# burchim/AVEC

Measured on AMD Instinct MI355X. Metric: AV utterances/sec fwd+bwd (audio T=400, video 100x88x88), higher is better.
Workload: dtype bf16

## Files before the change

avec_amd/csrc/conv3x3.hip:

```cpp
#include "wave_prims.h"
#include "vec.h"
#include "avec_hip.h"

#define C3_WPITCH 1280
#define C3_WBYTES (64 * C3_WPITCH)
#define C3_MAXPIX 576
#define C3_SBYTES (C3_MAXPIX * 128)

struct C3Args { const bf16* x; const bf16* w; bf16* y; const bf16* res; float* stats; int N, H, W, flip; const unsigned char* rmask; };

__device__ __forceinline__ int c3_wslot(int n, int c) { return (c & ~15) | ((c & 15) ^ (n & 15)); }
__device__ __forceinline__ int c3_saddr(int pix, int c) { const int pr = pix >> 1; return pr * 256 + (((((pix & 1) << 3) | c) ^ (pr & 7)) << 4); }
__device__ __forceinline__ int c3_lane_pixel(int l) { return l < 4 ? l : l < 12 ? l + 12 : l < 16 ? l - 8 : l < 20 ? l + 8 : l < 28 ? l - 12 : l; }

#ifndef C3S_ABL
#define C3S_ABL 0
#endif
template <bool STATS, bool RES>
__global__ __launch_bounds__(512) void conv3x3_c64_kernel(C3Args a) {
  extern __shared__ __attribute__((aligned(16))) char smem[];
  char* Ws = smem; char* Sl = smem + C3_WBYTES;
  const int tid = threadIdx.x, lane = tid & 63, wave = tid >> 6;
  const int H = a.H, W = a.W, PW = W + 1, HW = H * W, NPIX = (H + 2) * PW + 1;

  for (int q = tid; q < 64 * 72; q += 512) {
    const int n = q / 72, c = q - n * 72;
    *(chunk16*)(Ws + n * C3_WPITCH + c3_wslot(n, c) * 16) = ldg16(a.w + (long long)n * 576 + c * 8);
  }
  int soff[9];
#pragma unroll
  for (int i = 0; i < 9; ++i) {
    const int S = (wave + 8 * i) * 64 + lane, pr = S >> 4, c2 = (S & 15) ^ (pr & 7);
    const int pix = pr * 2 + (c2 >> 3), ch = c2 & 7;
    const int py = (pix - 1) / PW, px = (pix - 1) - py * PW;
    const bool in = pix >= 1 && pix < NPIX && py >= 1 && py <= H && px < W;
    soff[i] = in ? ((py - 1) * W + px) * 64 + ch * 8 : -1;
  }
  const int kh2 = lane >> 5;
  int p0[2]; bool pvalid[2]; int pm[2];
#pragma unroll
  for (int i = 0; i < 2; ++i) {
    int m = wave * 64 + i * 32 + c3_lane_pixel(lane & 31);
    pvalid[i] = m < HW; if (m >= HW) m = HW - 1;
    pm[i] = m;
    const int oy = m / W;
    p0[i] = oy * PW + (m - oy * W);
  }
  const int wrow[2] = {(lane & 31) * C3_WPITCH, (32 + (lane & 31)) * C3_WPITCH};
  const int wkey = lane & 15;

  float ssum[STATS ? 2 : 1][16], ssq[STATS ? 2 : 1][16];
  if (STATS) {
#pragma unroll
    for (int j = 0; j < 2; ++j)
#pragma unroll
      for (int r = 0; r < 16; ++r) { ssum[j][r] = 0.f; ssq[j][r] = 0.f; }
  }

  f32x16 acc[2][2];
  u32x4 outp[2][2][2], resp[RES ? 2 : 1][2][2];
  long long prev = -1;
  auto swap_pair = [&](uint2& x, uint2& y) {
    auto r0 = __builtin_amdgcn_permlane32_swap(x.x, y.x, false, false); x.x = r0[0]; y.x = r0[1];
    auto r1 = __builtin_amdgcn_permlane32_swap(x.y, y.y, false, false); x.y = r1[0]; y.y = r1[1];
  };
  const int chq = kh2 * 8;
  unsigned ldoff[9], zmask = 0u;
#pragma unroll
  for (int i = 0; i < 9; ++i) { ldoff[i] = soff[i] < 0 ? 0u : (unsigned)soff[i] * 2u; if (soff[i] < 0) zmask |= 1u << i; }
  const unsigned stoff[2] = {(unsigned)pm[0] * 128u + (unsigned)chq * 2u, (unsigned)pm[1] * 128u + (unsigned)chq * 2u};
#define C3_GLOAD(dst, voff, sbase, OFF) asm volatile("s_nop 4\n\tglobal_load_dwordx4 %0, %1, %2 offset:%3" : "+v"(dst) : "v"(voff), "s"(sbase), "n"(OFF))
#define C3_GSTORE(voff, data, sbase, OFF) asm volatile("s_nop 4\n\tglobal_store_dwordx4 %0, %1, %2 offset:%3\n\ts_nop 1" :: "v"(voff), "v"(data), "s"(sbase), "n"(OFF))
  auto issue_stores = [&]() {
    if (prev < 0 || (C3S_ABL & (8 | 16))) return;
    bf16* yo = a.y + prev * HW * 64;
#pragma unroll
    for (int i = 0; i < 2; ++i) {
      if (!pvalid[i]) continue;
#pragma unroll
      for (int j = 0; j < 2; ++j)
#pragma unroll
        for (int k = 0; k < 2; ++k) *(u32x4*)(yo + (long long)pm[i] * 64 + j * 32 + k * 16 + chq) = outp[j][i][k];
    }
  };

  u32x4 pf[9];
#pragma unroll
  for (int i = 0; i < 9; ++i) pf[i] = u32x4{0u, 0u, 0u, 0u};
  if (RES) {
#pragma unroll
    for (int i = 0; i < 2; ++i)
#pragma unroll
      for (int j = 0; j < 2; ++j)
#pragma unroll
        for (int k = 0; k < 2; ++k) resp[RES ? j : 0][i][k] = u32x4{0u, 0u, 0u, 0u};
  }
  if ((long long)blockIdx.x < a.N && !(C3S_ABL & 2)) {
    const bf16* x0 = a.x + (long long)blockIdx.x * HW * 64;
#pragma unroll
    for (int i = 0; i < 9; ++i) C3_GLOAD(pf[i], ldoff[i], x0, 0);
    asm volatile("s_waitcnt vmcnt(0)");
#pragma unroll
    for (int i = 0; i < 9; ++i) asm volatile("" : "+v"(pf[i]));
  }
#ifdef C3S_TRACE
  int tr_k = 0;
  float* const trbuf = STATS ? a.stats + 8192 : (float*)(a.y + (long long)a.N * HW * 64);
#define C3S_STAMP(slot) do { if (blockIdx.x == C3S_TRACE_WG && tid == 0 && tr_k < 16) { trbuf[8 * tr_k + (slot)] = (float)(clock64() & 0xffffff); if ((slot) == 0) trbuf[8 * tr_k + 6] = (float)(wall_clock64() & 0xffffff); } } while (0)
#else
#define C3S_STAMP(slot) do {} while (0)
#endif
  for (long long n = blockIdx.x; n < a.N; n += gridDim.x) {
    C3S_STAMP(0);
    asm volatile("s_waitcnt vmcnt(0)");
#pragma unroll
    for (int i = 0; i < 9; ++i) asm volatile("" : "+v"(pf[i]));
    __syncthreads();
#pragma unroll
    for (int i = 0; i < 9; ++i) {
      if (C3S_ABL & 2) break;
      u32x4 v = pf[i];
      if (zmask & (1u << i)) v = u32x4{0u, 0u, 0u, 0u};
      *(u32x4*)(Sl + ((wave + 8 * i) * 64 + lane) * 16) = v;
    }
    __syncthreads();
    C3S_STAMP(1);
#pragma unroll
    for (int j = 0; j < 2; ++j)
#pragma unroll
      for (int i = 0; i < 2; ++i)
#pragma unroll
        for (int r = 0; r < 16; ++r) acc[j][i][r] = 0.f;
    int p0o[2] = {p0[0], p0[1]}, wkeyo = wkey;
    asm volatile("" : "+v"(p0o[0]), "+v"(p0o[1]), "+v"(wkeyo));
    auto tap_addr = [&](int tap, int& ax0, int& ax1, int& aw0, int& aw1, bool& z0, bool& z1) {
      const int th = tap / 3, tw = tap - th * 3;
      const int dh = (a.flip & 1) ? 2 - th : th, dw = (a.flip & 1) ? 2 - tw : tw;
      const int d = dh * PW + dw;
      ax0 = c3_saddr(p0o[0] + d, kh2); ax1 = c3_saddr(p0o[1] + d, kh2);
      const int wt = (((tap >> 1) << 4) | ((((tap & 1) << 3) | kh2) ^ wkeyo)) << 4;
      aw0 = wrow[0] + wt; aw1 = wrow[1] + wt;
      z0 = z1 = false;
    };
    auto load4 = [&](int ax0, int ax1, int aw0, int aw1, bool z0, bool z1, int q, chunk16& fx0, chunk16& fx1, chunk16& fw0, chunk16& fw1) {
      if (C3S_ABL & 4) { fx0.w[0] = fx0.w[1] = fx0.w[2] = fx0.w[3] = ax0 + q; fx1 = fx0; fw0 = fx0; fw1 = fx0; return; }
      fx0 = *(const chunk16*)(Sl + (ax0 ^ (q << 5)));
      fx1 = *(const chunk16*)(Sl + (ax1 ^ (q << 5)));
      fw0 = *(const chunk16*)(Ws + (aw0 ^ (q << 5)));
      fw1 = *(const chunk16*)(Ws + (aw1 ^ (q << 5)));
    };
    const bool has_prev = prev >= 0 && !(C3S_ABL & (8 | 16)), has_next = n + gridDim.x < a.N;
    const bf16* const yprev = a.y + (has_prev ? prev : 0) * HW * 64;
    const bf16* const xnext = a.x + (has_next ? n + gridDim.x : n) * HW * 64;
    const bf16* const rcur = RES ? a.res + n * HW * 64 : a.x;
    auto one_tap = [&](int tap) {
      int ax0, ax1, aw0, aw1; bool z0, z1;
      tap_addr(tap, ax0, ax1, aw0, aw1, z0, z1);
#pragma unroll
      for (int q = 0; q < 4; ++q) {
        chunk16 cx0, cx1, cw0, cw1;
        load4(ax0, ax1, aw0, aw1, z0, z1, q, cx0, cx1, cw0, cw1);
        if (C3S_ABL & 1) { asm volatile("" :: "v"(cx0.w[0]), "v"(cx0.w[3]), "v"(cx1.w[0]), "v"(cx1.w[3]), "v"(cw0.w[0]), "v"(cw0.w[3]), "v"(cw1.w[0]), "v"(cw1.w[3])); continue; }
        acc[0][0] = __builtin_amdgcn_mfma_f32_32x32x16_bf16(__builtin_bit_cast(bf16x8_t, cw0), __builtin_bit_cast(bf16x8_t, cx0), acc[0][0], 0, 0, 0);
        acc[0][1] = __builtin_amdgcn_mfma_f32_32x32x16_bf16(__builtin_bit_cast(bf16x8_t, cw0), __builtin_bit_cast(bf16x8_t, cx1), acc[0][1], 0, 0, 0);
        acc[1][0] = __builtin_amdgcn_mfma_f32_32x32x16_bf16(__builtin_bit_cast(bf16x8_t, cw1), __builtin_bit_cast(bf16x8_t, cx0), acc[1][0], 0, 0, 0);
        acc[1][1] = __builtin_amdgcn_mfma_f32_32x32x16_bf16(__builtin_bit_cast(bf16x8_t, cw1), __builtin_bit_cast(bf16x8_t, cx1), acc[1][1], 0, 0, 0);
      }
    };
#define C3_RS(I, J, K) do { if (RES) C3_GLOAD(resp[RES ? (J) : 0][I][K], stoff[I], rcur, (J) * 64 + (K) * 32); } while (0)
#define C3_ST(I, J, K) do { if (has_prev) C3_GSTORE(stoff[I], outp[J][I][K], yprev, (J) * 64 + (K) * 32); } while (0)
#define C3_LD1(I) do { if (!(C3S_ABL & 2)) C3_GLOAD(pf[I], ldoff[I], xnext, 0); } while (0)
#pragma unroll
    for (int tap = 0; tap < 9; ++tap) {
      switch (tap) {
        case 0: C3_LD1(0); C3_ST(0, 0, 0); break;
        case 1: C3_LD1(1); C3_ST(0, 0, 1); break;
        case 2: C3_LD1(2); C3_ST(0, 1, 0); break;
        case 3: C3_LD1(3); C3_ST(0, 1, 1); break;
        case 4: C3_LD1(4); C3_ST(1, 0, 0); break;
        case 5: C3_RS(0, 0, 0); C3_RS(0, 0, 1); C3_RS(0, 1, 0); C3_RS(0, 1, 1); C3_RS(1, 0, 0); C3_RS(1, 0, 1); C3_RS(1, 1, 0); C3_RS(1, 1, 1); C3_LD1(5); C3_ST(1, 0, 1); break;
        case 6: C3_LD1(6); C3_ST(1, 1, 0); break;
        case 7: C3_LD1(7); C3_ST(1, 1, 1); break;
        default: C3_LD1(8); break;
      }
      one_tap(tap);
      if (tap == 4) C3S_STAMP(2);
    }
#undef C3_LD1
#undef C3_RS
#undef C3_ST
    if (RES) { if (C3S_ABL & 2) asm volatile("s_waitcnt vmcnt(0)"); else if (has_prev) asm volatile("s_waitcnt vmcnt(7)"); else asm volatile("s_waitcnt vmcnt(4)"); }
    if (RES) {
#pragma unroll
      for (int i = 0; i < 2; ++i)
#pragma unroll
        for (int j = 0; j < 2; ++j)
#pragma unroll
          for (int k = 0; k < 2; ++k) asm volatile("" : "+v"(resp[RES ? j : 0][i][k]));
    }
    C3S_STAMP(3);
    if (C3S_ABL & 8) {
      float t = 0.f;
      for (int i = 0; i < 2; ++i) for (int j = 0; j < 2; ++j) for (int r = 0; r < 16; ++r) t += acc[j][i][r];
      if (t == 1234.5f) outp[0][0][0][0] = 1u;
      asm volatile("" :: "v"(t));
      prev = n; continue;
    }
#pragma unroll
    for (int i = 0; i < 2; ++i)
#pragma unroll
      for (int j = 0; j < 2; ++j)
#pragma unroll
        for (int k = 0; k < 2; ++k) {
          uint2 rx = make_uint2(0u, 0u), ry = make_uint2(0u, 0u);
          if (RES) { const u32x4 rr = resp[RES ? j : 0][i][k]; rx = make_uint2(rr[0], rr[1]); ry = make_uint2(rr[2], rr[3]); swap_pair(rx, ry); }
          uint2 o[2];
#pragma unroll
          for (int e = 0; e < 2; ++e) {
            const int g = 2 * k + e;
            float v[4] = {acc[j][i][g * 4 + 0], acc[j][i][g * 4 + 1], acc[j][i][g * 4 + 2], acc[j][i][g * 4 + 3]};
            if (STATS && pvalid[i]) {
#pragma unroll
              for (int t = 0; t < 4; ++t) { ssum[j][g * 4 + t] += v[t]; ssq[j][g * 4 + t] += v[t] * v[t]; }
            }
            if (RES) {
              const uint2 r = e ? ry : rx;
              v[0] += __uint_as_float(r.x << 16); v[1] += __uint_as_float(r.x & 0xffff0000u); v[2] += __uint_as_float(r.y << 16); v[3] += __uint_as_float(r.y & 0xffff0000u);
            }
            o[e] = make_uint2(f32x2_to_bf16x2(v[0], v[1]), f32x2_to_bf16x2(v[2], v[3]));
          }
          swap_pair(o[0], o[1]);
          outp[j][i][k] = u32x4{o[0].x, o[0].y, o[1].x, o[1].y};
        }
    prev = n;
    C3S_STAMP(4);
#ifdef C3S_TRACE
    ++tr_k;
#endif
  }
  issue_stores();
  if (STATS) {
    __syncthreads();
    float* red = (float*)Sl;
#pragma unroll
    for (int j = 0; j < 2; ++j)
#pragma unroll
      for (int r = 0; r < 16; ++r) {
        float s = ssum[j][r], q = ssq[j][r];
#pragma unroll
        for (int o = 1; o < 32; o <<= 1) { s += __shfl_xor(s, o, 64); q += __shfl_xor(q, o, 64); }
        if ((lane & 31) == 0) {
          const int ch = j * 32 + (r >> 2) * 8 + kh2 * 4 + (r & 3);
          red[(wave * 2 + 0) * 64 + ch] = s; red[(wave * 2 + 1) * 64 + ch] = q;
        }
      }
    __syncthreads();
    if (tid < 128) {
      float t = 0.f;
      for (int w = 0; w < 8; ++w) t += red[w * 128 + tid];
      float* rep = a.stats + (long long)(blockIdx.x % AVEC_STAT_REPLICAS) * 128;
      atomicAdd(rep + tid, t);
    }
  }
}

__device__ __forceinline__ unsigned c3_mask2(unsigned b, int d) {
  return ((0u - ((b >> (2 * d)) & 1u)) & 0xffffu) | ((0u - ((b >> (2 * d + 1)) & 1u)) & 0xffff0000u);
}
__global__ __launch_bounds__(512) void conv3x3_c64_res_kernel(C3Args a) {
  extern __shared__ __attribute__((aligned(16))) char smem[];
  char* Ws = smem; char* Sl = smem + C3_WBYTES;
  const int tid = threadIdx.x, lane = tid & 63, wave = tid >> 6;
  const int H = a.H, W = a.W, PW = W + 1, HW = H * W, NPIX = (H + 2) * PW + 1;

  for (int q = tid; q < 64 * 72; q += 512) {
    const int n = q / 72, c = q - n * 72;
    *(chunk16*)(Ws + n * C3_WPITCH + c3_wslot(n, c) * 16) = ldg16(a.w + (long long)n * 576 + c * 8);
  }
  int soff[9];
#pragma unroll
  for (int i = 0; i < 9; ++i) {
    const int S = (wave + 8 * i) * 64 + lane, pr = S >> 4, c2 = (S & 15) ^ (pr & 7);
    const int pix = pr * 2 + (c2 >> 3), ch = c2 & 7;
    const int py = (pix - 1) / PW, px = (pix - 1) - py * PW;
    const bool in = pix >= 1 && pix < NPIX && py >= 1 && py <= H && px < W;
    soff[i] = in ? ((py - 1) * W + px) * 64 + ch * 8 : -1;
  }
  const int kh2 = lane >> 5;
  int p0[2]; bool pvalid[2]; int pm[2];
#pragma unroll
  for (int i = 0; i < 2; ++i) {
    int m = wave * 64 + i * 32 + c3_lane_pixel(lane & 31);
    pvalid[i] = m < HW; if (m >= HW) m = HW - 1;
    pm[i] = m;
    const int oy = m / W;
    p0[i] = oy * PW + (m - oy * W);
  }
  const int wrow[2] = {(lane & 31) * C3_WPITCH, (32 + (lane & 31)) * C3_WPITCH};
  const int wkey = lane & 15;


  f32x16 acc[2][2];
  uint4 outp[2][2][2], resp[2][2][2];
  long long prev = -1;
  auto swap_pair = [&](uint2& x, uint2& y) {
    auto r0 = __builtin_amdgcn_permlane32_swap(x.x, y.x, false, false); x.x = r0[0]; y.x = r0[1];
    auto r1 = __builtin_amdgcn_permlane32_swap(x.y, y.y, false, false); x.y = r1[0]; y.y = r1[1];
  };
  const int chq = kh2 * 8;
  auto issue_stores = [&]() {
    if (prev < 0) return;
    bf16* yo = a.y + prev * HW * 64;
#pragma unroll
    for (int i = 0; i < 2; ++i) {
      if (!pvalid[i]) continue;
#pragma unroll
      for (int j = 0; j < 2; ++j)
#pragma unroll
        for (int k = 0; k < 2; ++k) *(uint4*)(yo + (long long)pm[i] * 64 + j * 32 + k * 16 + chq) = outp[j][i][k];
    }
  };

  chunk16 pf[9];
  if ((long long)blockIdx.x < a.N) {
    const bf16* x0 = a.x + (long long)blockIdx.x * HW * 64;
#pragma unroll
    for (int i = 0; i < 9; ++i) pf[i] = ldg16(x0 + (soff[i] < 0 ? 0 : soff[i]));
  }
  for (long long n = blockIdx.x; n < a.N; n += gridDim.x) {
    __syncthreads();
#pragma unroll
    for (int i = 0; i < 9; ++i) {
      chunk16 v = pf[i];
      if (soff[i] < 0) v.w[0] = v.w[1] = v.w[2] = v.w[3] = 0u;
      *(chunk16*)(Sl + ((wave + 8 * i) * 64 + lane) * 16) = v;
    }
    __syncthreads();
    if (n + gridDim.x < a.N) {
      const bf16* xn = a.x + (n + gridDim.x) * HW * 64;
#pragma unroll
      for (int i = 0; i < 9; ++i) pf[i] = ldg16(xn + (soff[i] < 0 ? 0 : soff[i]));
    }
#pragma unroll
    for (int j = 0; j < 2; ++j)
#pragma unroll
      for (int i = 0; i < 2; ++i)
#pragma unroll
        for (int r = 0; r < 16; ++r) acc[j][i][r] = 0.f;
    auto tap_addr = [&](int tap, int& ax0, int& ax1, int& aw0, int& aw1, bool& z0, bool& z1) {
      const int th = tap / 3, tw = tap - th * 3;
      const int dh = (a.flip & 1) ? 2 - th : th, dw = (a.flip & 1) ? 2 - tw : tw;
      const int d = dh * PW + dw;
      ax0 = c3_saddr(p0[0] + d, kh2); ax1 = c3_saddr(p0[1] + d, kh2);
      const int wt = (((tap >> 1) << 4) | ((((tap & 1) << 3) | kh2) ^ wkey)) << 4;
      aw0 = wrow[0] + wt; aw1 = wrow[1] + wt;
      z0 = z1 = false;
    };
    auto load4 = [&](int ax0, int ax1, int aw0, int aw1, bool z0, bool z1, int q, chunk16& fx0, chunk16& fx1, chunk16& fw0, chunk16& fw1) {
      fx0 = *(const chunk16*)(Sl + (ax0 ^ (q << 5)));
      fx1 = *(const chunk16*)(Sl + (ax1 ^ (q << 5)));
      fw0 = *(const chunk16*)(Ws + (aw0 ^ (q << 5)));
      fw1 = *(const chunk16*)(Ws + (aw1 ^ (q << 5)));
    };
    bf16* yprev = prev >= 0 ? a.y + prev * HW * 64 : nullptr;
    auto one_tap = [&](int tap) {
      int ax0, ax1, aw0, aw1; bool z0, z1;
      tap_addr(tap, ax0, ax1, aw0, aw1, z0, z1);
#pragma unroll
      for (int q = 0; q < 4; ++q) {
        chunk16 cx0, cx1, cw0, cw1;
        load4(ax0, ax1, aw0, aw1, z0, z1, q, cx0, cx1, cw0, cw1);
        acc[0][0] = mma16(cw0, cx0, acc[0][0]);
        acc[0][1] = mma16(cw0, cx1, acc[0][1]);
        acc[1][0] = mma16(cw1, cx0, acc[1][0]);
        acc[1][1] = mma16(cw1, cx1, acc[1][1]);
      }
    };
#define C3_ST(I, J, K) if (pvalid[I]) *(uint4*)(yprev + (long long)pm[I] * 64 + J * 32 + K * 16 + chq) = outp[J][I][K]
#pragma unroll 1
    for (int tap = 0; tap < 5; ++tap) {
      if (yprev) {
        switch (tap) {
          case 1: C3_ST(0, 0, 0); C3_ST(0, 0, 1); break;
          case 2: C3_ST(0, 1, 0); C3_ST(0, 1, 1); break;
          case 3: C3_ST(1, 0, 0); C3_ST(1, 0, 1); break;
          case 4: C3_ST(1, 1, 0); C3_ST(1, 1, 1); break;
          default: break;
        }
      }
      one_tap(tap);
    }
#undef C3_ST
    if (a.res) {
      const bf16* ro = a.res + n * HW * 64;
#pragma unroll
      for (int i = 0; i < 2; ++i)
#pragma unroll
        for (int j = 0; j < 2; ++j)
#pragma unroll
          for (int k = 0; k < 2; ++k) resp[j][i][k] = *(const uint4*)(ro + (long long)pm[i] * 64 + j * 32 + k * 16 + chq);
      if (a.rmask) {
        const unsigned char* mo = a.rmask + n * HW * 8;
        unsigned mb[2][2][2];
#pragma unroll
        for (int i = 0; i < 2; ++i)
#pragma unroll
          for (int j = 0; j < 2; ++j)
#pragma unroll
            for (int k = 0; k < 2; ++k) mb[j][i][k] = mo[((long long)pm[i] * 64 + j * 32 + k * 16 + chq) >> 3];
#pragma unroll
        for (int i = 0; i < 2; ++i)
#pragma unroll
          for (int j = 0; j < 2; ++j)
#pragma unroll
            for (int k = 0; k < 2; ++k) {
              const unsigned b = mb[j][i][k];
              resp[j][i][k].x &= c3_mask2(b, 0); resp[j][i][k].y &= c3_mask2(b, 1); resp[j][i][k].z &= c3_mask2(b, 2); resp[j][i][k].w &= c3_mask2(b, 3);
            }
      }
    }
#pragma unroll 1
    for (int tap = 5; tap < 9; ++tap) one_tap(tap);
#pragma unroll
    for (int i = 0; i < 2; ++i)
#pragma unroll
      for (int j = 0; j < 2; ++j)
#pragma unroll
        for (int k = 0; k < 2; ++k) {
          uint2 rx = make_uint2(0u, 0u), ry = make_uint2(0u, 0u);
          if (a.res) { rx = make_uint2(resp[j][i][k].x, resp[j][i][k].y); ry = make_uint2(resp[j][i][k].z, resp[j][i][k].w); swap_pair(rx, ry); }
          uint2 o[2];
#pragma unroll
          for (int e = 0; e < 2; ++e) {
            const int g = 2 * k + e;
            float v[4] = {acc[j][i][g * 4 + 0], acc[j][i][g * 4 + 1], acc[j][i][g * 4 + 2], acc[j][i][g * 4 + 3]};
            if (a.res) {
              const uint2 r = e ? ry : rx;
              v[0] += __uint_as_float(r.x << 16); v[1] += __uint_as_float(r.x & 0xffff0000u); v[2] += __uint_as_float(r.y << 16); v[3] += __uint_as_float(r.y & 0xffff0000u);
            }
            o[e] = make_uint2(f32x2_to_bf16x2(v[0], v[1]), f32x2_to_bf16x2(v[2], v[3]));
          }
          swap_pair(o[0], o[1]);
          outp[j][i][k] = make_uint4(o[0].x, o[0].y, o[1].x, o[1].y);
        }
    prev = n;
  }
  issue_stores();
}

__device__ __forceinline__ uint2 c3_lds_tr(unsigned lds_addr) { uint2 v; asm volatile("ds_read_b64_tr_b16 %0, %1" : "=v"(v) : "v"(lds_addr) : "memory"); return v; }
#ifndef C3W_ABL
#define C3W_ABL 0
#endif
#define C3W_KROWS 512
#define C3W_DBYTES (C3W_KROWS * 128)

struct C3WArgs { const bf16* x; const bf16* dy; float* dw; int N, H, W; };
#if C3W_ABL & 64
__device__ float c3w_dbg[128];
extern "C" int avec_c3w_debug(float* out) { return (int)hipMemcpyFromSymbol(out, HIP_SYMBOL(c3w_dbg), sizeof(float) * 128); }
#endif

template <int V> struct C3I { static constexpr int value = V; };
__device__ __forceinline__ void c3w_roll_body(const C3WArgs& a, const int bid, const int nwg) {
  extern __shared__ __attribute__((aligned(16))) char smem[];
  char* Xs = smem; char* Ds = smem + C3_SBYTES;
  const int tid = threadIdx.x, lane = tid & 63, wave = __builtin_amdgcn_readfirstlane(tid >> 6);
  const int H = a.H, W = a.W, PW = W + 1, HW = H * W, NPIX = (H + 2) * PW + 1;
  int xoff[9], doff[8];
#pragma unroll
  for (int i = 0; i < 9; ++i) {
    const int S = (wave + 8 * i) * 64 + lane, row = S >> 3, c = (S & 7) ^ (4 * ((row >> 1) & 1));
    const int py = (row - 1) / PW, px = (row - 1) - py * PW;
    const bool in = row >= 1 && row < NPIX && py >= 1 && py <= H && px < W;
    xoff[i] = in ? ((py - 1) * W + px) * 64 + c * 8 : -1;
  }
#pragma unroll
  for (int i = 0; i < 8; ++i) {
    const int S = (wave + 8 * i) * 64 + lane, row = S >> 3, c = (S & 7) ^ (4 * ((row >> 1) & 1));
    const int oy = row / PW, ox = row - oy * PW;
    doff[i] = (oy < H && ox < W) ? (oy * W + ox) * 64 + c * 8 : -1;
  }
  const int cohalf = (wave >> 1) & 1, cihalf = wave & 1, tap0 = wave >> 2;
  const bool five = wave < 4;
  const int g4 = lane >> 4, t = lane & 15;
  int offa[2], offb[5][2];
#pragma unroll
  for (int h = 0; h < 2; ++h) {
    const int krow = 8 * (g4 >> 1) + 4 * h + (t >> 2);
    const int cbA = cohalf * 32 + 16 * (g4 & 1), cbB = cihalf * 32 + 16 * (g4 & 1);
    offa[h] = krow * 128 + ((((cbA >> 3) + ((t & 3) >> 1)) ^ (4 * ((krow >> 1) & 1))) << 4) + (t & 1) * 8;
#pragma unroll
    for (int j = 0; j < 5; ++j) {
      const int tap = j < 4 ? tap0 + 2 * j : 8;
      const int rowd = krow + (tap / 3) * PW + (tap % 3);
      offb[j][h] = rowd * 128 + ((((cbB >> 3) + ((t & 3) >> 1)) ^ (4 * ((rowd >> 1) & 1))) << 4) + (t & 1) * 8;
    }
  }
  f32x16 acc[5];
#pragma unroll
  for (int j = 0; j < 5; ++j)
#pragma unroll
    for (int r = 0; r < 16; ++r) acc[j][r] = 0.f;

  const unsigned xs0 = (unsigned)(uintptr_t)(lptr_t)Xs, ds0 = (unsigned)(uintptr_t)(lptr_t)Ds;
  auto batch = [&](auto gc, const long long n) {
    constexpr int G = decltype(gc)::value;
    const bf16* xi = a.x + n * HW * 64; const bf16* di = a.dy + n * HW * 64;
#pragma unroll
    for (int i = 2 * G; i < (G == 3 ? 9 : 2 * G + 2); ++i) glds16(xoff[i] >= 0 ? (const void*)(xi + xoff[i]) : (const void*)avec_zero16, xs0 + (wave + 8 * i) * 1024);
#pragma unroll
    for (int i = 2 * G; i < 2 * G + 2; ++i) glds16(doff[i] >= 0 ? (const void*)(di + doff[i]) : (const void*)avec_zero16, ds0 + (wave + 8 * i) * 1024);
  };
  auto group = [&](auto gc) {
    constexpr int G = decltype(gc)::value;
#pragma unroll 2
    for (int s = 8 * G; s < 8 * G + 8; ++s) {
      const int so = s * 2048;
      const chunk16 fa = lds_tr8(Ds + offa[0] + so, Ds + offa[1] + so);
      chunk16 fb[5];
#pragma unroll
      for (int j = 0; j < 4; ++j) fb[j] = lds_tr8(Xs + offb[j][0] + so, Xs + offb[j][1] + so);
      if (five) fb[4] = lds_tr8(Xs + offb[4][0] + so, Xs + offb[4][1] + so);
#pragma unroll
      for (int j = 0; j < 4; ++j)
        acc[j] = mma16(fa, fb[j], acc[j]);
      if (five) acc[4] = mma16(fa, fb[4], acc[4]);
    }
// ... 202 lines not shown
  int KP, RS, IT;
  AVEC_CHECK_ARG(wgrad3x3_pairs_supported(H, W, C) || c3_wide_geometry(H, W, C, KP, RS, IT), "wgrad3x3_c128: %d channels, %dx%d images do not fit the slabs", C, H, W);
  avec_wgrad3x3_item_t it; it.x = x; it.dy = dy; it.dw = dw; it.images = images; it.C = C; it.H = H; it.W = W; it.reserved = 0;
  return avec_wgrad3x3_c128_grouped(&it, 1, st);
}

extern "C" int avec_wgrad3x3_c64_grouped(const avec_wgrad3x3_item_t* items, int n, hipStream_t st) {
  AVEC_CHECK_ARG(items && n > 0 && n <= AVEC_WGRAD_GROUP_MAX, "wgrad3x3_c64_grouped: 1..%d items", AVEC_WGRAD_GROUP_MAX);
  C3WGroup g; g.n = n;
  long long total_images = 0;
  for (int i = 0; i < n; ++i) {
    const avec_wgrad3x3_item_t& t = items[i];
    AVEC_CHECK_ARG(t.x && t.dy && t.dw && t.images > 0 && t.C == 64, "wgrad3x3_c64_grouped: bad item %d", i);
    AVEC_CHECK_ARG(avec_conv3x3_c64_supported(t.H, t.W, 64, 64, 3, 3, 1) && t.H * (t.W + 1) <= C3W_KROWS, "wgrad3x3_c64_grouped: item %d: %dx%d images do not fit the slab", i, t.H, t.W);
    C3WArgs& a = g.it[i]; a.x = (const bf16*)t.x; a.dy = (const bf16*)t.dy; a.dw = t.dw; a.N = (int)t.images; a.H = t.H; a.W = t.W;
    total_images += t.images;
  }
  int used = 0; g.first[0] = 0;
  for (int i = 0; i < n; ++i) {
    long long w = (256 * items[i].images + total_images / 2) / total_images; if (w < 1) w = 1; if (w > items[i].images) w = items[i].images;
    if (used + w > 256 + n) w = 1;
    used += (int)w; g.first[i + 1] = used;
  }
  const size_t lds = C3_SBYTES + C3W_DBYTES;
  if (int r = avec_lds_optin(wgrad3x3_c64_grouped_kernel, lds)) return r;
  avec_note_kernel("wgrad3x3_c64_grouped_kernel");
  hipLaunchKernelGGL(wgrad3x3_c64_grouped_kernel, dim3((unsigned)used), dim3(512), lds, st, g);
  AVEC_LAUNCH_CHECK();
  return 0;
}

extern "C" int avec_wgrad3x3_c128_grouped(const avec_wgrad3x3_item_t* items, int n, hipStream_t st) {
  AVEC_CHECK_ARG(items && n > 0 && n <= AVEC_WGRAD_GROUP_MAX, "wgrad3x3_c128_grouped: 1..%d items", AVEC_WGRAD_GROUP_MAX);
  {
    avec_wgrad3x3_item_t fast[AVEC_WGRAD_GROUP_MAX], slow[AVEC_WGRAD_GROUP_MAX]; int nf = 0, ns = 0;
    for (int i = 0; i < n; ++i) {
      AVEC_CHECK_ARG(items[i].x && items[i].dy && items[i].dw && items[i].images > 0, "wgrad3x3_c128_grouped: null buffer in item %d", i);
      if (wgrad3x3_pairs_supported(items[i].H, items[i].W, items[i].C)) fast[nf++] = items[i]; else slow[ns++] = items[i];
    }
    if (nf) {
      if (int r = wgrad3x3_pairs_grouped(fast, nf, st)) return r;
      if (!ns) return 0;
      return avec_wgrad3x3_c128_grouped(slow, ns, st);
    }
  }
  C3WWGroup g; g.n = n;
  long long cost[AVEC_WGRAD_GROUP_MAX]; int kinds[AVEC_WGRAD_GROUP_MAX], nwg[AVEC_WGRAD_GROUP_MAX], total = 0;
  for (int i = 0; i < n; ++i) {
    const avec_wgrad3x3_item_t& t = items[i];
    AVEC_CHECK_ARG(t.x && t.dy && t.dw && t.images > 0, "wgrad3x3_c128_grouped: null buffer in item %d", i);
    C3WWArgs& a = g.it[i]; a.x = (const bf16*)t.x; a.dy = (const bf16*)t.dy; a.dw = t.dw; a.N = (int)t.images; a.H = t.H; a.W = t.W; a.C = t.C;
    AVEC_CHECK_ARG(c3_wide_geometry(t.H, t.W, t.C, a.KP, a.RS, a.IT), "wgrad3x3_c128_grouped: item %d: %d channels, %dx%d images do not fit the slabs", i, t.C, t.H, t.W);
    kinds[i] = (t.C / 64) * (t.C / 128);
    const long long halves = (t.images + a.IT - 1) / a.IT;
    cost[i] = halves * (long long)(a.IT * (a.KP >> 4) + 2);
    nwg[i] = kinds[i]; total += kinds[i];
  }
  AVEC_CHECK_ARG(total <= 4096, "wgrad3x3_c128_grouped: too many tiles");
  const int budget = 256;
  for (;;) {
    int best = -1; double worst = 0.0;
    for (int i = 0; i < n; ++i) {
      const long long halves = (g.it[i].N + g.it[i].IT - 1) / g.it[i].IT;
      if (total + kinds[i] > budget || nwg[i] / kinds[i] >= halves) continue;
      const double load = (double)cost[i] / (double)(nwg[i] / kinds[i]);
      if (load > worst) { worst = load; best = i; }
    }
    if (best < 0) break;
    nwg[best] += kinds[best]; total += kinds[best];
  }
  g.first[0] = 0; for (int i = 0; i < n; ++i) g.first[i + 1] = g.first[i] + nwg[i];
  const size_t lds = (size_t)C3X_ROWS * 256 + C3X_KROWS * 128;
  if (int r = avec_lds_optin(wgrad3x3_wide_grouped_kernel, lds)) return r;
  avec_note_kernel("wgrad3x3_wide_grouped_kernel");
  hipLaunchKernelGGL(wgrad3x3_wide_grouped_kernel, dim3((unsigned)total), dim3(512), lds, st, g);
  AVEC_LAUNCH_CHECK();
  return 0;
}

extern "C" int avec_conv3x3_c64_supported(int H, int W, int Cin, int Cout, int KH, int KW, int stride) {
  return Cin == 64 && Cout == 64 && KH == 3 && KW == 3 && stride == 1 && H * W <= 512 && (H + 2) * (W + 1) + 1 <= C3_MAXPIX && H >= 1 && W >= 2;
}

static int conv3x3_c64_impl(const void* x, const void* w, void* y, const void* res, const unsigned char* rmask, float* stats, long long images, int H, int W, int flip, hipStream_t st);
extern "C" int avec_conv3x3_c64(const void* x, const void* w, void* y, const void* res, float* stats, long long images, int H, int W, int flip, hipStream_t st) {
  return conv3x3_c64_impl(x, w, y, res, nullptr, stats, images, H, W, flip, st);
}
extern "C" int avec_conv3x3_c64_res_masked(const void* x, const void* w, void* y, const void* res, const unsigned char* res_mask, long long images, int H, int W, int flip, hipStream_t st) {
  AVEC_CHECK_ARG(res && res_mask, "conv3x3_c64_res_masked: null residual / mask");
  return conv3x3_c64_impl(x, w, y, res, res_mask, nullptr, images, H, W, flip, st);
}
static int conv3x3_c64_impl(const void* x, const void* w, void* y, const void* res, const unsigned char* rmask, float* stats, long long images, int H, int W, int flip, hipStream_t st) {
  AVEC_CHECK_ARG(x && w && y && images > 0, "conv3x3_c64: null buffer");
  AVEC_CHECK_ARG(avec_conv3x3_c64_supported(H, W, 64, 64, 3, 3, 1), "conv3x3_c64: %dx%d images do not fit the slab", H, W);
  AVEC_CHECK_ARG(!(stats && res), "conv3x3_c64: statistics and a residual in the same launch are not supported");
  const size_t lds = C3_WBYTES + C3_SBYTES;
  const void* kern = !stats && !res ? (const void*)conv3x3_c64_kernel<false, false> : stats ? (const void*)conv3x3_c64_kernel<true, false> : (const void*)conv3x3_c64_res_kernel;
  if (int r = avec_lds_optin(kern, lds)) return r;
  C3Args a; a.x = (const bf16*)x; a.w = (const bf16*)w; a.y = (bf16*)y; a.res = (const bf16*)res; a.stats = stats; a.N = (int)images; a.H = H; a.W = W; a.flip = flip; a.rmask = rmask;
  const int grid = (int)(images < 256 ? images : 256);
  avec_note_kernel(stats ? "conv3x3_c64_kernel<true,false>" : res ? "conv3x3_c64_res_kernel" : "conv3x3_c64_kernel<false,false>");
  if (stats) hipLaunchKernelGGL((conv3x3_c64_kernel<true, false>), dim3(grid), dim3(512), lds, st, a);
  else if (res) hipLaunchKernelGGL(conv3x3_c64_res_kernel, dim3(grid), dim3(512), lds, st, a);
  else hipLaunchKernelGGL((conv3x3_c64_kernel<false, false>), dim3(grid), dim3(512), lds, st, a);
  AVEC_LAUNCH_CHECK();
  return 0;
}

extern "C" int avec_wgrad3x3_c64(const void* x, const void* dy, float* dw, long long images, int H, int W, hipStream_t st) {
  AVEC_CHECK_ARG(x && dy && dw && images > 0, "wgrad3x3_c64: null buffer");
  AVEC_CHECK_ARG(avec_conv3x3_c64_supported(H, W, 64, 64, 3, 3, 1) && H * (W + 1) <= C3W_KROWS, "wgrad3x3_c64: %dx%d images do not fit the slab", H, W);
  avec_wgrad3x3_item_t it; it.x = x; it.dy = dy; it.dw = dw; it.images = images; it.C = 64; it.H = H; it.W = W; it.reserved = 0;
  return avec_wgrad3x3_c64_grouped(&it, 1, st);
}
```

avec_amd/csrc/norm.hip:

```cpp
#include "common.h"
#include "avec_hip.h"

#include "vec.h"
#include <type_traits>

__global__ __launch_bounds__(256) void col_finalize_kernel(ColFin f) {
  __shared__ float red[16][17];
  const int cw = threadIdx.x & 15, sl = threadIdx.x >> 4;
  const int ncols = f.NV * f.W;
  const int o = blockIdx.x * 16 + cw;
  const unsigned cb = blockIdx.y;
  const int s0 = blockIdx.z * 128;
  float s = 0.f;
  if (o < ncols) {
    const float* p = f.partial + ((size_t)cb * f.nslots) * ncols + o;
#pragma unroll
    for (int k = 0; k < 8; ++k) {
      const int si = s0 + sl + 16 * k; const int sc = si < f.nslots ? si : f.nslots - 1;
      const float v = p[(size_t)sc * ncols];
      s += si < f.nslots ? v : 0.f;
    }
  }
  red[sl][cw] = s;
  __syncthreads();
// ... 588 lines not shown
  ld8<float>(ss + 2 * C + c, k.mu); ld8<float>(ss + 3 * C + c, k.rs);
  if (recompute) { ld8<float>(ss + c, k.sc); ld8<float>(ss + C + c, k.sh); }
}
__device__ __forceinline__ void bn8_dy_coeffs(Bn8Dy& q, const Bn8Bwd& k, const float* __restrict__ gamma, const float* __restrict__ dstats, float inv_n, int C, int c) {
  float g[8], s1[8], s2[8]; ld8<float>(gamma + c, g); ld8<float>(dstats + c, s1); ld8<float>(dstats + C + c, s2);
#pragma unroll
  for (int e = 0; e < 8; ++e) { q.A[e] = g[e] * k.rs[e]; q.m1[e] = s1[e] * inv_n; q.m2[e] = s2[e] * inv_n; }
}
template <typename T>
__device__ __forceinline__ void bn8_bwd_d(const Raw8<T>& rd, const Raw8<T>& rv, const Raw8<T>& ro, const unsigned& mb, int src, int act, const Bn8Bwd& k, float (&d)[8], float (&v)[8]) {
  rd.get(d); rv.get(v);
  if (src == BN_SRC_BITS) {
#pragma unroll
    for (int e = 0; e < 8; ++e) d[e] = (mb >> e) & 1u ? d[e] : 0.f;
  } else if (src == BN_SRC_OUT) { float o[8]; ro.get(o);
#pragma unroll
    for (int e = 0; e < 8; ++e) d[e] = o[e] > 0.f ? d[e] : 0.f;
  } else if (act == 2) {
#pragma unroll
    for (int e = 0; e < 8; ++e) d[e] = __builtin_fmaf(v[e], k.sc[e], k.sh[e]) > 0.f ? d[e] : 0.f;
  } else if (act == 1) {
#pragma unroll
    for (int e = 0; e < 8; ++e) { const float x = __builtin_fmaf(v[e], k.sc[e], k.sh[e]), sg = sigmoidf_(x); d[e] *= sg * __builtin_fmaf(x, 1.f - sg, 1.f); }
  }
}
__device__ __forceinline__ void bn8_bwd_acc(float (&part)[2][8], const float (&d)[8], const float (&v)[8], const Bn8Bwd& k) {
#pragma unroll
  for (int e = 0; e < 8; ++e) { part[0][e] += d[e]; part[1][e] += d[e] * (v[e] - k.mu[e]) * k.rs[e]; }
}
__device__ __forceinline__ void bn8_dy(const float (&d)[8], const float (&v)[8], const Bn8Bwd& k, const Bn8Dy& q, float (&o)[8]) {
#pragma unroll
  for (int e = 0; e < 8; ++e) o[e] = q.A[e] * __builtin_fmaf(-((v[e] - k.mu[e]) * k.rs[e]), q.m2[e], d[e] - q.m1[e]);
}

constexpr int BNS_P = 4;
constexpr unsigned BNS_SLICE_FWD = 1024, BNS_SLICE_BWD = 1536;
constexpr unsigned BNS_GRID_RED = 2048, BNS_RED_MIN_UNITS = 4;
constexpr long long BNS_MIN_CHUNKS = 1ll << 20;
static int& bns_mode() { static int mode = getenv("AVEC_BN_SLICE") ? atoi(getenv("AVEC_BN_SLICE")) : 1; return mode; }
static inline bool bns_ok(int dtype, long long M, int C) {
  const int mode = bns_mode();
  if (mode == 0 || dtype != AVEC_BF16 || C % 8 != 0 || 256 % (C / 8) != 0) return false;
  const long long n8 = M * C / 8;
  return n8 < (1ll << 31) && (mode == 2 || n8 >= BNS_MIN_CHUNKS);
}
template <bool NT> __device__ __forceinline__ void bns_ld(Raw8<bf16>& r, const bf16* p) {
  if (NT) { typedef unsigned v4u __attribute__((ext_vector_type(4))); const v4u t = __builtin_nontemporal_load((const v4u*)p); r.t = make_uint4(t.x, t.y, t.z, t.w); }
  else r.load(p);
}
static inline unsigned bns_slice(long long n8, unsigned grid) { return (unsigned)(((n8 + grid - 1) / grid + 255) / 256 * 256); }
static inline unsigned bns_grid(long long n8, unsigned slice) { return (unsigned)((n8 + slice - 1) / slice); }
static inline unsigned bns_red_grid(long long n8) {
  long long g = n8 / (256ll * BNS_P * BNS_RED_MIN_UNITS) / 256 * 256; if (g > BNS_GRID_RED) g = BNS_GRID_RED; if (g < 256) g = 256;
  return (unsigned)g;
}
struct BnsPlan { unsigned grid, slice; ColPlan col; };
static BnsPlan bns_plan(int pass, long long n8, int C, hipStream_t st) {
  if (pass == 1) { const ColPlan col = ColPlan::flat<2>(bns_red_grid(n8), C, st).cap_without_ws(256); return BnsPlan{col.nslots, bns_slice(n8, col.nslots), col}; }
  const unsigned slice = pass == 0 ? BNS_SLICE_FWD : BNS_SLICE_BWD;
  return BnsPlan{bns_grid(n8, slice), slice, ColPlan{}};
}
template <int P, typename Set, typename Load, typename Use>
__device__ __forceinline__ void bns_walk(unsigned begin, unsigned end, Load load, Use use) {
  constexpr unsigned UNIT = 256 * P;
  constexpr std::true_type full{}; constexpr std::false_type ragged{};
  if (begin >= end) return;
  Set a, b;
  unsigned base = begin;
  load(a, base, ragged);
  while (end - base >= 3 * UNIT) {
    load(b, base + UNIT, full); use(a, base, full);
    load(a, base + 2 * UNIT, full); use(b, base + UNIT, full);
    base += 2 * UNIT;
  }
  if (end - base > UNIT) {
    load(b, base + UNIT, ragged); use(a, base, full);
    if (end - base > 2 * UNIT) { load(a, base + 2 * UNIT, ragged); use(b, base + UNIT, full); use(a, base + 2 * UNIT, ragged); }
    else use(b, base + UNIT, ragged);
  } else use(a, base, ragged);
}
template <bool FULL> __device__ __forceinline__ unsigned bns_chunk(unsigned base, int p, unsigned end) {
  const unsigned j = base + threadIdx.x + p * 256; return FULL || j < end ? j : end - 1;
}
__device__ __forceinline__ void bns_range(unsigned slice, unsigned n8, unsigned& begin, unsigned& end) {
  const unsigned long long b = (unsigned long long)blockIdx.x * slice;
  begin = b < n8 ? (unsigned)b : n8; end = n8 - begin > slice ? begin + slice : n8;
}

template <int P, bool RES> struct BnsFwdSet { Raw8<bf16> y[P], r[RES ? P : 1]; };
template <int P, bool RES, bool MASK>
__global__ __launch_bounds__(256) void bn_apply8s_kernel(const bf16* __restrict__ y, const float* __restrict__ ss, const bf16* __restrict__ res, int act,
                                                         bf16* __restrict__ out, unsigned n8, int C, unsigned slice, unsigned char* __restrict__ mask,
                                                         const float* __restrict__ res_ss) {
  unsigned begin, end; bns_range(slice, n8, begin, end);
  const int c = (int)(threadIdx.x % ((unsigned)C >> 3)) * 8;
  Bn8Fwd k; bn8_fwd_coeffs(k, ss, RES ? res_ss : nullptr, C, c);
  typedef BnsFwdSet<P, RES> Set;
  auto load = [&](Set& s, unsigned base, auto full) {
#pragma unroll
    for (int p = 0; p < P; ++p) { const long long off = (long long)bns_chunk<decltype(full)::value>(base, p, end) * 8; bns_ld<true>(s.y[p], y + off); if (RES) bns_ld<true>(s.r[p], res + off); }
  };
  auto use = [&](Set& s, unsigned base, auto full) {
#pragma unroll
    for (int p = 0; p < P; ++p) {
      const unsigned j = base + threadIdx.x + p * 256; if (!decltype(full)::value && j >= end) break;
      const Bn8Out o = bn8_fwd<bf16>(s.y[p], s.r[RES ? p : 0], RES, res_ss != nullptr, k, act, MASK ? mask : nullptr, j);
      st8<bf16>(out + (long long)j * 8, o.v);
    }
  };
  bns_walk<P, Set>(begin, end, load, use);
}

template <int P, int SRC> struct BnsBwdSet { Raw8<bf16> d[P], v[P], o[SRC == BN_SRC_OUT ? P : 1]; unsigned mb[SRC == BN_SRC_BITS ? P : 1]; };
template <bool FULL, bool NT, int P, int SRC>
__device__ __forceinline__ void bns_bwd_load(BnsBwdSet<P, SRC>& s, unsigned base, unsigned end, const bf16* __restrict__ dout, const bf16* __restrict__ y,
                                             const bf16* __restrict__ out, const unsigned char* __restrict__ mask) {
#pragma unroll
  for (int p = 0; p < P; ++p) { const unsigned j = bns_chunk<FULL>(base, p, end); const long long off = (long long)j * 8; bns_ld<NT>(s.d[p], dout + off); bns_ld<NT>(s.v[p], y + off);
    if (SRC == BN_SRC_BITS) s.mb[p] = mask[j]; else if (SRC == BN_SRC_OUT) bns_ld<NT>(s.o[p], out + off); }
}
template <int P, int SRC>
__device__ __forceinline__ void bns_bwd_d(const BnsBwdSet<P, SRC>& s, int p, int act, const Bn8Bwd& k, float (&d)[8], float (&v)[8]) {
  bn8_bwd_d<bf16>(s.d[p], s.v[p], s.o[SRC == BN_SRC_OUT ? p : 0], s.mb[SRC == BN_SRC_BITS ? p : 0], SRC, act, k, d, v);
}
template <int P, int SRC>
__global__ __launch_bounds__(256) void bn_bwd_reduce8s_kernel(const bf16* __restrict__ dout, const bf16* __restrict__ y, const bf16* __restrict__ out, const float* __restrict__ ss,
                                                              int act, float* dstats, unsigned n8, int C, unsigned slice, ColWs ws, const unsigned char* __restrict__ mask) {
  unsigned begin, end; bns_range(slice, n8, begin, end);
  const Col8 m = col8_map(C);
  const int c = m.l * 8;
  float part[2][8];
#pragma unroll
  for (int e = 0; e < 8; ++e) part[0][e] = part[1][e] = 0.f;
  Bn8Bwd k; bn8_bwd_coeffs(k, ss, SRC == BN_SRC_NONE && act != 0, C, c);
  typedef BnsBwdSet<P, SRC> Set;
  auto load = [&](Set& s, unsigned base, auto full) { bns_bwd_load<decltype(full)::value, false, P, SRC>(s, base, end, dout, y, out, mask); };
  auto use = [&](Set& s, unsigned base, auto full) {
#pragma unroll
    for (int p = 0; p < P; ++p) {
      if (!decltype(full)::value && base + threadIdx.x + p * 256 >= end) break;
      float d[8], v[8]; bns_bwd_d<P, SRC>(s, p, act, k, d, v);
      bn8_bwd_acc(part, d, v, k);
    }
  };
  bns_walk<P, Set>(begin, end, load, use);
  float* const dst[2] = {dstats, dstats + C};
  colreduce8_atomic<2>(part, dst, m, ws);
}
template <int P, int SRC>
__global__ __launch_bounds__(256) void bn_bwd_apply8s_kernel(const bf16* __restrict__ dout, const bf16* __restrict__ y, const bf16* __restrict__ out, const float* __restrict__ ss,
                                                             const float* __restrict__ gamma, const float* __restrict__ dstats, const float* count_ptr, float count, int act,
                                                             bf16* __restrict__ dy, bf16* __restrict__ dres, float* dgamma, float* dbeta, unsigned n8, int C, unsigned slice,
                                                             const unsigned char* __restrict__ mask) {
  const float inv_n = 1.f / (count_ptr ? *count_ptr : count);
  if (blockIdx.x == 0 && dgamma) for (int cc = threadIdx.x; cc < C; cc += 256) { atomicAdd(dgamma + cc, dstats[C + cc]); atomicAdd(dbeta + cc, dstats[cc]); }
  unsigned begin, end; bns_range(slice, n8, begin, end);
  const int c = (int)(threadIdx.x % ((unsigned)C >> 3)) * 8;
  Bn8Bwd k; bn8_bwd_coeffs(k, ss, SRC == BN_SRC_NONE && act != 0, C, c);
  Bn8Dy q; bn8_dy_coeffs(q, k, gamma, dstats, inv_n, C, c);
  typedef BnsBwdSet<P, SRC> Set;
  auto load = [&](Set& s, unsigned base, auto full) { bns_bwd_load<decltype(full)::value, true, P, SRC>(s, base, end, dout, y, out, mask); };
  auto use = [&](Set& s, unsigned base, auto full) {
#pragma unroll
    for (int p = 0; p < P; ++p) {
      const unsigned j = base + threadIdx.x + p * 256; if (!decltype(full)::value && j >= end) break;
      const long long off = (long long)j * 8;
      float d[8], v[8], o[8]; bns_bwd_d<P, SRC>(s, p, act, k, d, v);
      bn8_dy(d, v, k, q, o);
      st8<bf16>(dy + off, o);
      if (dres) st8<bf16>(dres + off, d);
    }
  };
  bns_walk<P, Set>(begin, end, load, use);
}

template <typename T>
__global__ __launch_bounds__(256) void bn_apply8_kernel(const T* __restrict__ y, const float* __restrict__ ss, const T* __restrict__ res, int act,
                                                        T* __restrict__ out, unsigned n8, int C, unsigned char* __restrict__ mask, const float* __restrict__ res_ss) {
  const unsigned C8 = (unsigned)C >> 3, stride = gridDim.x * 256, i0 = blockIdx.x * 256 + threadIdx.x;
  const int c = (int)(i0 % C8) * 8;
  Bn8Fwd k; bn8_fwd_coeffs(k, ss, res_ss, C, c);
  for (unsigned i = i0; i < n8; i += stride * BN8_U) {
    Raw8<T> ry[BN8_U], rr[BN8_U];
#pragma unroll
    for (int u = 0; u < BN8_U; ++u) { const unsigned j = i + u * stride; if (j < n8) { ry[u].load(y + (long long)j * 8); if (res) rr[u].load(res + (long long)j * 8); } }
#pragma unroll
    for (int u = 0; u < BN8_U; ++u) {
      const unsigned j = i + u * stride; if (j >= n8) break;
      const Bn8Out o = bn8_fwd<T>(ry[u], rr[u], res != nullptr, res_ss != nullptr, k, act, mask, j);
      st8<T>(out + (long long)j * 8, o.v);
    }
  }
}
static int bn_apply_fwd_impl(int dtype, const void* y, const float* ss, const void* res, const float* res_ss, int act, void* out, unsigned char* mask, long long M, int C,
                             hipStream_t st) {
  const long long n8 = M * C / 8;
  if (bns_ok(dtype, M, C)) {
    const BnsPlan p = bns_plan(0, n8, C, st);
#define BNS_FWD(RES, MASK) hipLaunchKernelGGL((bn_apply8s_kernel<BNS_P, RES, MASK>), dim3(p.grid), dim3(256), 0, st, (const bf16*)y, ss, (const bf16*)res, act, (bf16*)out, (unsigned)n8, C, p.slice, mask, res_ss)
    if (res) { if (mask) BNS_FWD(true, true); else BNS_FWD(true, false); } else { if (mask) BNS_FWD(false, true); else BNS_FWD(false, false); }
#undef BNS_FWD
  } else if (C % 8 == 0 && n8 < (1ll << 31)) {
    DISPATCH_T(dtype, hipLaunchKernelGGL(bn_apply8_kernel<T>, dim3(bn8_blocks(n8, C, BN8_CAP_FWD)), dim3(256), 0, st, (const T*)y, ss, (const T*)res, act, (T*)out, (unsigned)n8, C, mask, res_ss));
  } else {
    long long n4 = M * C / 4; long long nb = (n4 + 255) / 256; if (nb > 4096) nb = 4096;
    DISPATCH_T(dtype, hipLaunchKernelGGL(bn_apply_kernel<T>, dim3((unsigned)nb), dim3(256), 0, st, (const T*)y, ss, (const T*)res, act, (T*)out, n4, C));
  }
  AVEC_LAUNCH_CHECK(); return 0;
}
extern "C" int avec_bn_apply_fwd_mask(int dtype, const void* y, const float* ss, const void* residual, const float* residual_ss, void* out, unsigned char* mask, long long M, int C,
                                      hipStream_t st) {
  AVEC_CHECK_ARG(y && ss && out && mask && M > 0 && C > 0 && C % 8 == 0 && M * C / 8 < (1ll << 31) && (residual || !residual_ss), "bn_apply_fwd_mask: bad arguments (C %% 8 == 0, M*C < 2^34)");
  return bn_apply_fwd_impl(dtype, y, ss, residual, residual_ss, 2, out, mask, M, C, st);
}
extern "C" int avec_bn_apply_fwd(int dtype, const void* y, const float* ss, const void* residual, int act, void* out, long long M, int C, hipStream_t st) {
  AVEC_CHECK_ARG(y && ss && out && M > 0 && C > 0 && C % 4 == 0, "bn_apply_fwd: bad arguments");
  return bn_apply_fwd_impl(dtype, y, ss, residual, nullptr, act, out, nullptr, M, C, st);
}

template <typename T>
__device__ __forceinline__ void bn_dr(const T* dout, const T* y, const T* out, const float* ss, int act, long long off, int c, int C, float dr[4], float yh[4]) {
  float d[4], v[4], mu[4], rs[4]; ld4<T>(dout + off, d); ld4<T>(y + off, v); ld4<float>(ss + 2 * C + c, mu); ld4<float>(ss + 3 * C + c, rs);
  for (int e = 0; e < 4; ++e) yh[e] = (v[e] - mu[e]) * rs[e];
  if (act == 2) {
    if (out) { float o[4]; ld4<T>(out + off, o); for (int e = 0; e < 4; ++e) dr[e] = o[e] > 0.f ? d[e] : 0.f; }
    else { float sc[4], sh[4]; ld4<float>(ss + c, sc); ld4<float>(ss + C + c, sh); for (int e = 0; e < 4; ++e) dr[e] = (v[e] * sc[e] + sh[e]) > 0.f ? d[e] : 0.f; }
  }
  else if (act == 1) { float sc[4], sh[4]; ld4<float>(ss + c, sc); ld4<float>(ss + C + c, sh); for (int e = 0; e < 4; ++e) dr[e] = d[e] * dswishf_(v[e] * sc[e] + sh[e]); }
  else { for (int e = 0; e < 4; ++e) dr[e] = d[e]; }
}
template <typename T>
__global__ __launch_bounds__(256) void bn_bwd_reduce_kernel(const T* __restrict__ dout, const T* __restrict__ y, const T* __restrict__ out, const float* __restrict__ ss,
                                                            int act, float* dstats, long long M, int C, ColWs ws) {
  const int tx = threadIdx.x & 31, ty = threadIdx.x >> 5; const int col = (blockIdx.x * 32 + tx) * 4;
  float part[2][4] = {{0.f, 0.f, 0.f, 0.f}, {0.f, 0.f, 0.f, 0.f}};
  if (col < C) for (long long row = (long long)blockIdx.y * 8 + ty; row < M; row += (long long)gridDim.y * 8) {
    float dr[4], yh[4]; bn_dr<T>(dout, y, out, ss, act, row * C + col, col, C, dr, yh);
    for (int e = 0; e < 4; ++e) { part[0][e] += dr[e]; part[1][e] += dr[e] * yh[e]; }
  }
  float* const dst[2] = {dstats, dstats + C};
  colreduce_atomic<2>(part, dst, col, C, ws);
}
template <typename T>
__global__ __launch_bounds__(256) void bn_bwd_reduce8_kernel(const T* __restrict__ dout, const T* __restrict__ y, const T* __restrict__ out, const float* __restrict__ ss,
                                                             int act, float* dstats, long long M, int C, ColWs ws, const unsigned char* __restrict__ mask) {
  const Col8 m = col8_map(C);
  float part[2][8];
#pragma unroll
  for (int e = 0; e < 8; ++e) part[0][e] = part[1][e] = 0.f;
  if (m.active) {
    const int c = m.l * 8, src = bn8_src(act, out, mask);
    Bn8Bwd k; bn8_bwd_coeffs(k, ss, src == BN_SRC_NONE && act != 0, C, c);
    const long long rstride = (long long)gridDim.x * m.R;
    for (long long row = (long long)blockIdx.x * m.R + m.r; row < M; row += rstride * BN8_UR) {
      Raw8<T> rd[BN8_UR], rv[BN8_UR], ro[BN8_UR]; unsigned mb[BN8_UR];
#pragma unroll
      for (int u = 0; u < BN8_UR; ++u) { const long long r = row + u * rstride; if (r < M) { const long long off = r * C + c; rd[u].load(dout + off); rv[u].load(y + off);
        if (src == BN_SRC_BITS) mb[u] = mask[off >> 3]; else if (src == BN_SRC_OUT) ro[u].load(out + off); } }
#pragma unroll
      for (int u = 0; u < BN8_UR; ++u) {
        if (row + u * rstride >= M) break;
        float d[8], v[8]; bn8_bwd_d<T>(rd[u], rv[u], ro[u], mb[u], src, act, k, d, v);
        bn8_bwd_acc(part, d, v, k);
      }
    }
  }
  float* const dst[2] = {dstats, dstats + C};
  colreduce8_atomic<2>(part, dst, m, ws);
}
static int bn_bwd_reduce_impl(int dtype, const void* dout, const void* y, const void* out, const unsigned char* mask, const float* ss, int act, float* dstats, long long M, int C,
                              hipStream_t st) {
  ColPlan plan;
  if (mask && bns_ok(dtype, M, C)) {
    const long long n8 = M * C / 8; const BnsPlan p = bns_plan(1, n8, C, st); plan = p.col;
    hipLaunchKernelGGL((bn_bwd_reduce8s_kernel<BNS_P, BN_SRC_BITS>), dim3(p.grid), dim3(256), 0, st, (const bf16*)dout, (const bf16*)y, (const bf16*)out, ss, act, dstats, (unsigned)n8, C, p.slice, plan.ws, mask);
  } else if (col8_ok(C)) {
    plan = ColPlan::flat8<2>(M, C, st);
    DISPATCH_T(dtype, hipLaunchKernelGGL(bn_bwd_reduce8_kernel<T>, dim3(plan.nslots), dim3(256), 0, st, (const T*)dout, (const T*)y, (const T*)out, ss, act, dstats, M, C, plan.ws, mask));
  } else {
    const dim3 grid = col_grid(M, C); plan = ColPlan::grid<2>(grid, C, st);
    DISPATCH_T(dtype, hipLaunchKernelGGL(bn_bwd_reduce_kernel<T>, grid, dim3(256), 0, st, (const T*)dout, (const T*)y, (const T*)out, ss, act, dstats, M, C, plan.ws));
  }
  AVEC_LAUNCH_CHECK();
  return plan.finish({dstats, dstats + C}, C, st);
}
extern "C" int avec_bn_bwd_reduce_mask(int dtype, const void* dout, const void* y, const unsigned char* mask, const float* ss, float* dstats, long long M, int C, hipStream_t st) {
  AVEC_CHECK_ARG(dout && y && mask && ss && dstats && M > 0 && col8_ok(C), "bn_bwd_reduce_mask: bad arguments");
  return bn_bwd_reduce_impl(dtype, dout, y, nullptr, mask, ss, 2, dstats, M, C, st);
}
extern "C" int avec_bn_bwd_reduce(int dtype, const void* dout, const void* y, const void* out, const float* ss, int act, float* dstats, long long M, int C, hipStream_t st) {
  AVEC_CHECK_ARG(dout && y && ss && dstats && M > 0 && C % 4 == 0, "bn_bwd_reduce: bad arguments");
  return bn_bwd_reduce_impl(dtype, dout, y, out, nullptr, ss, act, dstats, M, C, st);
}
template <typename T>
__global__ __launch_bounds__(256) void bn_bwd_apply_kernel(const T* __restrict__ dout, const T* __restrict__ y, const T* __restrict__ out, const float* __restrict__ ss,
                                                           const float* __restrict__ gamma, const float* __restrict__ dstats, const float* count_ptr, float count, int act,
                                                           T* __restrict__ dy, T* __restrict__ dres, float* dgamma, float* dbeta, long long n4, int C) {
  const float inv_n = 1.f / (count_ptr ? *count_ptr : count);
  if (blockIdx.x == 0 && dgamma) for (int c = threadIdx.x; c < C; c += 256) { atomicAdd(dgamma + c, dstats[C + c]); atomicAdd(dbeta + c, dstats[c]); }
  for (long long i = (long long)blockIdx.x * 256 + threadIdx.x; i < n4; i += (long long)gridDim.x * 256) {
    const long long off = i * 4; const int c = (int)(off % C);
    float dr[4], yh[4], g[4], rs[4], s1[4], s2[4], o[4];
    bn_dr<T>(dout, y, out, ss, act, off, c, C, dr, yh);
    ld4<float>(gamma + c, g); ld4<float>(ss + 3 * C + c, rs); ld4<float>(dstats + c, s1); ld4<float>(dstats + C + c, s2);
    for (int e = 0; e < 4; ++e) o[e] = g[e] * rs[e] * (dr[e] - s1[e] * inv_n - yh[e] * s2[e] * inv_n);
    st4<T>(dy + off, o);
    if (dres) st4<T>(dres + off, dr);
  }
}
template <typename T>
__global__ __launch_bounds__(256) void bn_bwd_apply8_kernel(const T* __restrict__ dout, const T* __restrict__ y, const T* __restrict__ out, const float* __restrict__ ss,
                                                            const float* __restrict__ gamma, const float* __restrict__ dstats, const float* count_ptr, float count, int act,
                                                            T* __restrict__ dy, T* __restrict__ dres, float* dgamma, float* dbeta, unsigned n8, int C,
                                                            const unsigned char* __restrict__ mask) {
  const float inv_n = 1.f / (count_ptr ? *count_ptr : count);
  if (blockIdx.x == 0 && dgamma) for (int c = threadIdx.x; c < C; c += 256) { atomicAdd(dgamma + c, dstats[C + c]); atomicAdd(dbeta + c, dstats[c]); }
  const unsigned C8 = (unsigned)C >> 3, stride = gridDim.x * 256, i0 = blockIdx.x * 256 + threadIdx.x;
  const int c = (int)(i0 % C8) * 8, src = bn8_src(act, out, mask);
  Bn8Bwd k; bn8_bwd_coeffs(k, ss, src == BN_SRC_NONE && act != 0, C, c);
  Bn8Dy q; bn8_dy_coeffs(q, k, gamma, dstats, inv_n, C, c);
  for (unsigned i = i0; i < n8; i += stride * BN8_U) {
    Raw8<T> rd[BN8_U], rv[BN8_U], ro[BN8_U]; unsigned mb[BN8_U];
#pragma unroll
    for (int u = 0; u < BN8_U; ++u) { const unsigned j = i + u * stride; if (j < n8) { const long long off = (long long)j * 8; rd[u].load(dout + off); rv[u].load(y + off);
      if (src == BN_SRC_BITS) mb[u] = mask[j]; else if (src == BN_SRC_OUT) ro[u].load(out + off); } }
#pragma unroll
    for (int u = 0; u < BN8_U; ++u) {
      const unsigned j = i + u * stride; if (j >= n8) break;
      const long long off = (long long)j * 8;
      float d[8], v[8], o[8]; bn8_bwd_d<T>(rd[u], rv[u], ro[u], mb[u], src, act, k, d, v);
      bn8_dy(d, v, k, q, o);
      st8<T>(dy + off, o);
      if (dres) st8<T>(dres + off, d);
    }
  }
}
static int bn_bwd_apply_impl(int dtype, const void* dout, const void* y, const void* out, const unsigned char* mask, const float* ss, const float* gamma, const float* dstats,
                             const float* count_ptr, float count, int act, void* dy, void* dres, float* dgamma, float* dbeta, long long M, int C, hipStream_t st) {
  const long long n8 = M * C / 8;
  if (bns_ok(dtype, M, C)) {
    const BnsPlan p = bns_plan(2, n8, C, st);
#define BNS_BWD(SRC) hipLaunchKernelGGL((bn_bwd_apply8s_kernel<BNS_P, SRC>), dim3(p.grid), dim3(256), 0, st, (const bf16*)dout, (const bf16*)y, (const bf16*)out, ss, gamma, dstats, \
                                        count_ptr, count, act, (bf16*)dy, (bf16*)dres, dgamma, dbeta, (unsigned)n8, C, p.slice, mask)
    if (mask) BNS_BWD(BN_SRC_BITS); else if (act == 2 && out) BNS_BWD(BN_SRC_OUT); else BNS_BWD(BN_SRC_NONE);
#undef BNS_BWD
  } else if (C % 8 == 0 && n8 < (1ll << 31)) {
    DISPATCH_T(dtype, hipLaunchKernelGGL(bn_bwd_apply8_kernel<T>, dim3(bn8_blocks(n8, C, BN8_CAP_BWD)), dim3(256), 0, st, (const T*)dout, (const T*)y, (const T*)out, ss, gamma, dstats,
                                         count_ptr, count, act, (T*)dy, (T*)dres, dgamma, dbeta, (unsigned)n8, C, mask));
  } else {
    long long n4 = M * C / 4; long long nb = (n4 + 255) / 256; if (nb > 4096) nb = 4096;
    DISPATCH_T(dtype, hipLaunchKernelGGL(bn_bwd_apply_kernel<T>, dim3((unsigned)nb), dim3(256), 0, st, (const T*)dout, (const T*)y, (const T*)out, ss, gamma, dstats,
                                         count_ptr, count, act, (T*)dy, (T*)dres, dgamma, dbeta, n4, C));
  }
  AVEC_LAUNCH_CHECK(); return 0;
}
extern "C" int avec_bn_bwd_apply_mask(int dtype, const void* dout, const void* y, const unsigned char* mask, const float* ss, const float* gamma, const float* dstats,
                                      const float* count_ptr, float count, void* dy, void* dres, float* dgamma, float* dbeta, long long M, int C, hipStream_t st) {
  AVEC_CHECK_ARG(dout && y && mask && ss && gamma && dstats && dy && M > 0 && C % 8 == 0 && M * C / 8 < (1ll << 31), "bn_bwd_apply_mask: bad arguments");
  return bn_bwd_apply_impl(dtype, dout, y, nullptr, mask, ss, gamma, dstats, count_ptr, count, 2, dy, dres, dgamma, dbeta, M, C, st);
}
extern "C" int avec_bn_bwd_apply(int dtype, const void* dout, const void* y, const void* out, const float* ss, const float* gamma, const float* dstats,
                                 const float* count_ptr, float count, int act, void* dy, void* dres, float* dgamma, float* dbeta, long long M, int C, hipStream_t st) {
  AVEC_CHECK_ARG(dout && y && ss && gamma && dstats && dy && M > 0 && C % 4 == 0, "bn_bwd_apply: bad arguments");
  return bn_bwd_apply_impl(dtype, dout, y, out, nullptr, ss, gamma, dstats, count_ptr, count, act, dy, dres, dgamma, dbeta, M, C, st);
}
extern "C" int avec_bn_slice_mode(int mode) { const int old = bns_mode(); if (mode >= 0 && mode <= 2) bns_mode() = mode; return old; }
extern "C" int avec_bn_slice_plan(int pass, long long M, int C, int* P, unsigned* grid, unsigned* slice, hipStream_t st) {
  if (P) *P = BNS_P;
  if (M <= 0 || C <= 0 || C % 8 != 0 || pass < 0 || pass > 2 || !bns_ok(AVEC_BF16, M, C)) return 0;
  const BnsPlan p = bns_plan(pass, M * C / 8, C, st);
  if (grid) *grid = p.grid;
  if (slice) *slice = p.slice;
  return 1;
}

template <typename T>
__global__ __launch_bounds__(256) void softmax_fwd_kernel(const float* __restrict__ x, T* __restrict__ p, long long M, int V) {
  const int lane = threadIdx.x & 63; const long long row = (long long)blockIdx.x * 4 + (threadIdx.x >> 6);
  if (row >= M) return;
  float mx = -INFINITY;
  for (int c = lane; c < V; c += 64) mx = fmaxf(mx, x[row * V + c]);
  mx = wave_max(mx);
  float s = 0.f;
  for (int c = lane; c < V; c += 64) s += __expf(x[row * V + c] - mx);
  s = 1.f / wave_sum(s);
  for (int c = lane; c < V; c += 64) stf(p + row * V + c, __expf(x[row * V + c] - mx) * s);
}
template <typename T>
__global__ __launch_bounds__(256) void softmax_bwd_kernel(const T* __restrict__ dp, const float* __restrict__ x, float* dx, const float* dadd, long long M, int V) {
  const int lane = threadIdx.x & 63; const long long row = (long long)blockIdx.x * 4 + (threadIdx.x >> 6);
  if (row >= M) return;
  float mx = -INFINITY;
  for (int c = lane; c < V; c += 64) mx = fmaxf(mx, x[row * V + c]);
  mx = wave_max(mx);
  float s = 0.f, dot = 0.f;
  for (int c = lane; c < V; c += 64) { float e = __expf(x[row * V + c] - mx); s += e; dot += e * ldf(dp + row * V + c); }
  s = wave_sum(s); dot = wave_sum(dot) / s;
  for (int c = lane; c < V; c += 64) {
    float pr = __expf(x[row * V + c] - mx) / s; float g = pr * (ldf(dp + row * V + c) - dot);
    dx[row * V + c] = dadd ? dadd[row * V + c] + g : g;
  }
}
extern "C" int avec_softmax_fwd(int dtype, const float* logits, void* probs, long long M, int V, hipStream_t st) {
  AVEC_CHECK_ARG(logits && probs && M > 0 && V > 0, "softmax_fwd: bad arguments");
  DISPATCH_T(dtype, hipLaunchKernelGGL(softmax_fwd_kernel<T>, dim3((unsigned)((M + 3) / 4)), dim3(256), 0, st, logits, (T*)probs, M, V));
  AVEC_LAUNCH_CHECK(); return 0;
}
extern "C" int avec_softmax_bwd(int dtype, const void* dprobs, const float* logits, float* dlogits, const float* dadd, long long M, int V, hipStream_t st) {
  AVEC_CHECK_ARG(dprobs && logits && dlogits && M > 0 && V > 0, "softmax_bwd: bad arguments");
  DISPATCH_T(dtype, hipLaunchKernelGGL(softmax_bwd_kernel<T>, dim3((unsigned)((M + 3) / 4)), dim3(256), 0, st, (const T*)dprobs, logits, dlogits, dadd, M, V));
  AVEC_LAUNCH_CHECK(); return 0;
}

template <typename T>
__global__ __launch_bounds__(256) void cast_rows_kernel(const float* __restrict__ src, long long lds_, T* __restrict__ dst, long long ldd, long long M, int N) {
  const long long n4 = M * (N / 4);
  for (long long i = (long long)blockIdx.x * 256 + threadIdx.x; i < n4; i += (long long)gridDim.x * 256) {
    const long long row = i / (N / 4); const int c = (int)(i % (N / 4)) * 4;
    float v[4]; ld4<float>(src + row * lds_ + c, v); st4<T>(dst + row * ldd + c, v);
  }
}
extern "C" int avec_cast_rows(int dtype, const float* src, long long ld_src, void* dst, long long ld_dst, long long M, int N, hipStream_t st) {
  AVEC_CHECK_ARG(src && dst && M > 0 && N > 0 && N % 4 == 0 && ld_src % 4 == 0 && ld_dst % 4 == 0, "cast_rows: bad arguments");
  long long nb = (M * (N / 4) + 255) / 256; if (nb > 4096) nb = 4096;
  DISPATCH_T(dtype, hipLaunchKernelGGL(cast_rows_kernel<T>, dim3((unsigned)nb), dim3(256), 0, st, src, ld_src, (T*)dst, ld_dst, M, N));
  AVEC_LAUNCH_CHECK(); return 0;
}
template <typename T>
__global__ __launch_bounds__(256) void to_f32_rows_kernel(const T* __restrict__ src, long long lds_, float* __restrict__ dst, long long ldd, long long M, int N, int accum) {
  const long long n4 = M * (N / 4);
  for (long long i = (long long)blockIdx.x * 256 + threadIdx.x; i < n4; i += (long long)gridDim.x * 256) {
    const long long row = i / (N / 4); const int c = (int)(i % (N / 4)) * 4;
    float v[4]; ld4<T>(src + row * lds_ + c, v);
    if (accum) { float o[4]; ld4<float>(dst + row * ldd + c, o); for (int e = 0; e < 4; ++e) v[e] += o[e]; }
    st4<float>(dst + row * ldd + c, v);
  }
}
extern "C" int avec_to_f32_rows(int dtype, const void* src, long long ld_src, float* dst, long long ld_dst, long long M, int N, int accum, hipStream_t st) {
  AVEC_CHECK_ARG(src && dst && M > 0 && N > 0 && N % 4 == 0 && ld_src % 4 == 0 && ld_dst % 4 == 0, "to_f32_rows: bad arguments");
  long long nb = (M * (N / 4) + 255) / 256; if (nb > 4096) nb = 4096;
  DISPATCH_T(dtype, hipLaunchKernelGGL(to_f32_rows_kernel<T>, dim3((unsigned)nb), dim3(256), 0, st, (const T*)src, ld_src, dst, ld_dst, M, N, accum));
  AVEC_LAUNCH_CHECK(); return 0;
}

__global__ __launch_bounds__(256) void dropout_f32_kernel(const float* __restrict__ x, float* __restrict__ y, float p, const unsigned long long* rng, unsigned stream, long long n) {
  const DropKey dk = drop_key(rng, stream, p);
  for (long long i = (long long)blockIdx.x * 256 + threadIdx.x; i < n; i += (long long)gridDim.x * 256) y[i] = x[i] * drop_one(dk, (unsigned long long)i);
// ... 146 lines not shown
```

avec_amd/csrc/vec.h:

```cpp
#pragma once
#include "common.h"
#include <cstdlib>
#include <initializer_list>

template <typename T> __device__ __forceinline__ void ld4(const T* p, float v[4]);
template <> __device__ __forceinline__ void ld4<float>(const float* p, float v[4]) { float4 t = *(const float4*)p; v[0] = t.x; v[1] = t.y; v[2] = t.z; v[3] = t.w; }
template <> __device__ __forceinline__ void ld4<bf16>(const bf16* p, float v[4]) {
  uint2 t = *(const uint2*)p;
  v[0] = __uint_as_float(t.x << 16); v[1] = __uint_as_float(t.x & 0xffff0000u);
  v[2] = __uint_as_float(t.y << 16); v[3] = __uint_as_float(t.y & 0xffff0000u);
}
template <typename T> __device__ __forceinline__ void st4(T* p, const float v[4]);
template <> __device__ __forceinline__ void st4<float>(float* p, const float v[4]) { *(float4*)p = make_float4(v[0], v[1], v[2], v[3]); }
template <> __device__ __forceinline__ void st4<bf16>(bf16* p, const float v[4]) {
  uint2 t; t.x = f32x2_to_bf16x2(v[0], v[1]);
  t.y = f32x2_to_bf16x2(v[2], v[3]);
  *(uint2*)p = t;
}

template <typename T> __device__ __forceinline__ void ld8(const T* p, float v[8]);
template <> __device__ __forceinline__ void ld8<float>(const float* p, float v[8]) { ld4<float>(p, v); ld4<float>(p + 4, v + 4); }
template <> __device__ __forceinline__ void ld8<bf16>(const bf16* p, float v[8]) {
  uint4 t = *(const uint4*)p; const uint32_t w[4] = {t.x, t.y, t.z, t.w};
#pragma unroll
  for (int k = 0; k < 4; ++k) { v[2 * k] = __uint_as_float(w[k] << 16); v[2 * k + 1] = __uint_as_float(w[k] & 0xffff0000u); }
}
template <typename T> __device__ __forceinline__ void st8(T* p, const float v[8]);
template <> __device__ __forceinline__ void st8<float>(float* p, const float v[8]) { st4<float>(p, v); st4<float>(p + 4, v + 4); }
template <> __device__ __forceinline__ void st8<bf16>(bf16* p, const float v[8]) {
  uint4 t;
  t.x = f32x2_to_bf16x2(v[0], v[1]); t.y = f32x2_to_bf16x2(v[2], v[3]);
  t.z = f32x2_to_bf16x2(v[4], v[5]); t.w = f32x2_to_bf16x2(v[6], v[7]);
  *(uint4*)p = t;
}

__device__ __forceinline__ void bf8_to_f32(const uint4& t, float v[8]) {
  const uint32_t w[4] = {t.x, t.y, t.z, t.w};
#pragma unroll
  for (int k = 0; k < 4; ++k) { v[2 * k] = __uint_as_float(w[k] << 16); v[2 * k + 1] = __uint_as_float(w[k] & 0xffff0000u); }
}
template <typename T> struct Raw8;
template <> struct Raw8<bf16> { uint4 t; __device__ __forceinline__ void load(const bf16* p) { t = *(const uint4*)p; } __device__ __forceinline__ void get(float v[8]) const { bf8_to_f32(t, v); } };
template <> struct Raw8<float> { float4 a, b; __device__ __forceinline__ void load(const float* p) { a = *(const float4*)p; b = *(const float4*)(p + 4); }
  __device__ __forceinline__ void get(float v[8]) const { v[0] = a.x; v[1] = a.y; v[2] = a.z; v[3] = a.w; v[4] = b.x; v[5] = b.y; v[6] = b.z; v[7] = b.w; } };
#define DISPATCH_T(dtype, ...) do { if ((dtype) == AVEC_BF16) { typedef bf16 T; __VA_ARGS__; } else { typedef float T; __VA_ARGS__; } } while (0)


struct ColWs { float* partial; };
ColWs avec_reduce_ws(size_t partial_floats, hipStream_t st);

__device__ __forceinline__ float* ws_slot(const ColWs& ws, unsigned colblock, unsigned slot, unsigned nslots, int ncols) {
  return ws.partial + ((size_t)colblock * nslots + slot) * ncols;
}
static constexpr int FIN_MAXNV = 20;
struct ColFin { const float* partial; float* dst[FIN_MAXNV]; int NV, W, C, nslots, dstride; };
__global__ __launch_bounds__(256) void col_finalize_kernel(ColFin f);
int colsum_launch(int dtype, const void* x, long long ld, float* out, long long M, int N, bool use_ws, hipStream_t st);
int col_finalize(const ColWs& ws, unsigned colblocks, unsigned nslots, int NV, int W, float* const* dst, int C, hipStream_t st, int dstride = 1);

template <int NV>
__device__ __forceinline__ void colreduce_atomic(float (&part)[NV][4], float* const (&dst)[NV], int col, int C, const ColWs& ws = ColWs{nullptr}) {
  __shared__ float red[8][32][4];
  const int tx = threadIdx.x & 31, ty = threadIdx.x >> 5;
  float* mine = ws.partial ? ws_slot(ws, blockIdx.x, blockIdx.y, gridDim.y, NV * 128) : nullptr;
#pragma unroll
  for (int n = 0; n < NV; ++n) {
    for (int e = 0; e < 4; ++e) red[ty][tx][e] = part[n][e];
    __syncthreads();
    if (ty == 0) {
      for (int e = 0; e < 4; ++e) {
        float s = 0.f;
        for (int y = 0; y < 8; ++y) s += red[y][tx][e];
        if (mine) mine[n * 128 + tx * 4 + e] = s;
        else if (col + e < C && dst[n]) atomicAdd(dst[n] + col + e, s);
      }
    }
    __syncthreads();
  }
}
static inline long long col_ws_min_atomics() { return 16384; }

static inline dim3 col_grid(long long M, int C) {
  unsigned gx = (unsigned)((C / 4 + 31) / 32);
  long long gy = (M + 63) / 64; long long cap = 2048 / gx; if (cap < 1) cap = 1; if (gy > cap) gy = cap; if (gy < 1) gy = 1;
  return dim3(gx, (unsigned)gy);
}

struct Col8 { int L, R, r, l; bool active; };
__device__ __forceinline__ Col8 col8_map(int C) {
  Col8 m; m.L = C >> 3; m.R = 256 / m.L; m.r = threadIdx.x / m.L; m.l = threadIdx.x - m.r * m.L; m.active = m.r < m.R; return m;
}
template <int NV>
__device__ __forceinline__ void colreduce8_atomic(float (&part)[NV][8], float* const (&dst)[NV], const Col8& m, const ColWs& ws = ColWs{nullptr}) {
  __shared__ float red8[NV * 8][256];
#pragma unroll
  for (int n = 0; n < NV; ++n)
#pragma unroll
    for (int e = 0; e < 8; ++e) red8[n * 8 + e][threadIdx.x] = m.active ? part[n][e] : 0.f;
  __syncthreads();
  const int C = m.L * 8;
  float* mine = ws.partial ? ws_slot(ws, 0, blockIdx.x, gridDim.x, NV * C) : nullptr;
  for (int o = threadIdx.x; o < NV * 8 * m.L; o += 256) {
    const int q = o / m.L, l = o - q * m.L; float s = 0.f;
    for (int rr = 0; rr < m.R; ++rr) s += red8[q][rr * m.L + l];
    if (mine) mine[(q >> 3) * C + l * 8 + (q & 7)] = s;
    else {
      float* d = nullptr;
#pragma unroll
      for (int n = 0; n < NV; ++n) if ((q >> 3) == n) d = dst[n];
      if (d) atomicAdd(d + l * 8 + (q & 7), s);
    }
  }
}
static inline bool col8_ok(int C) { return C % 8 == 0 && C <= 2048; }
#ifndef AVEC_COL8_CAP
#define AVEC_COL8_CAP 1024
#endif
static inline long long col8_cap() { return AVEC_COL8_CAP; }
static inline unsigned col8_blocks(long long M, int C) { const int R = 256 / (C / 8); long long nb = (M + R - 1) / R; if (nb > col8_cap()) nb = col8_cap(); return (unsigned)nb; }

struct __attribute__((visibility("hidden"))) ColPlan {
  ColWs ws; unsigned colblocks, nslots; int NV, W;
  template <int NV_> static ColPlan grid(dim3 g, int C, hipStream_t st, bool want_ws = true) {
    static_assert(NV_ <= FIN_MAXNV, "col_finalize_kernel carries FIN_MAXNV destinations");
    const bool two = want_ws && (long long)g.y * NV_ * C > col_ws_min_atomics();
    return ColPlan{two ? avec_reduce_ws((size_t)g.x * g.y * NV_ * 128, st) : ColWs{nullptr}, g.x, g.y, NV_, 128};
  }
  template <int NV_> static ColPlan flat(unsigned nb, int W, hipStream_t st, bool want_ws = true) {
    static_assert(NV_ <= FIN_MAXNV, "col_finalize_kernel carries FIN_MAXNV destinations");
    return ColPlan{want_ws ? avec_reduce_ws((size_t)nb * NV_ * W, st) : ColWs{nullptr}, 1, nb, NV_, W};
  }
  template <int NV_> static ColPlan flat8(long long M, int C, hipStream_t st) {
    const unsigned nb = col8_blocks(M, C);
    if ((long long)nb * NV_ * C <= col_ws_min_atomics()) return flat<NV_>(nb, C, st, false);
    return flat<NV_>(nb, C, st).cap_without_ws(256);
  }
  ColPlan cap_without_ws(unsigned cap) const { ColPlan p = *this; if (!p.ws.partial && p.nslots > cap) p.nslots = cap; return p; }
  int finish(float* const* dst, int C, hipStream_t st, int dstride = 1) const {
    return ws.partial ? col_finalize(ws, colblocks, nslots, NV, W, dst, C, st, dstride) : 0;
  }
  int finish(std::initializer_list<float*> dst, int C, hipStream_t st, int dstride = 1) const {
    AVEC_CHECK_ARG((int)dst.size() == NV, "column reduction: %d destinations for %d quantities", (int)dst.size(), NV);
    return finish(dst.begin(), C, st, dstride);
  }
};
```

avec_amd/nnet/networks.py:

```python
import os

import torch
import torch.nn as nn

from .. import ops
from .. import runtime as rt
from . import attentions, blocks, layers, modules, preprocessing, transforms
from .streaming import AudioFrontStreamSession, AudioStreamSession, AudioVisualStreamSession, ConformerLookaheadStreamSession, ConformerStreamSession, VisualFrontStreamSession, VisualStreamSession


class ResNet(nn.Module):

    def __init__(self, dim_input=3, dim_output=1000, model="ResNet50", include_stem=True, include_head=True):
        super().__init__()
        assert model in ("ResNet18", "ResNet34") and not include_stem, "hot path: basic-block ResNet fed by the Conv3d stem (nnet/networks.py:472)"
        dim_stem, dim_blocks = 64, [64, 128, 256, 512]
        num_blocks = [2, 2, 2, 2] if model == "ResNet18" else [3, 4, 6, 3]
        self.stem = nn.Identity()
        self.blocks = nn.ModuleList()
        for stage in range(4):
            for b in range(num_blocks[stage]):
                first = b == 0
                cin = (dim_stem if stage == 0 else dim_blocks[stage - 1]) if first else dim_blocks[stage]
                stride = (2, 2) if (first and stage > 0) else (1, 1)
                self.blocks.append(blocks.ResNetBlock(in_features=cin, out_features=dim_blocks[stage], kernel_size=(3, 3), stride=stride,
                                                      act_fun="ReLU", joined_post_act=True))
        self.head = nn.Sequential(layers.GlobalAvgPool2d(),
                                  layers.Linear(dim_blocks[-1], dim_output, weight_init="he_normal", bias_init="zeros")) if include_head else nn.Identity()

    def forward_nhwc(self, x):
        for i, blk in enumerate(self.blocks):
            x = blk.forward_nhwc(x, chain=i + 1 < len(self.blocks))
        if isinstance(self.head, nn.Identity):
            return x
        x = ops.AvgPoolFn.apply(x)
        lin = self.head[1]
        return ops.linear(x, lin.weight, lin.bias)

    def forward(self, x):
        return self.forward_nhwc(x.permute(0, 2, 3, 1).to(rt.act_dtype()).contiguous())


class Transformer(nn.Module):

    def __init__(self, dim_model, num_blocks, att_params={"class": "MultiHeadAttention", "params": {"num_heads": 4, "weight_init": "normal_02", "bias_init": "zeros"}},
                 ff_ratio=4, emb_drop_rate=0.1, drop_rate=0.1, act_fun="GELU", pos_embedding=None, mask=None, inner_dropout=False, weight_init="normal_02",
                 bias_init="zeros", post_norm=False):
        super().__init__()
        assert not post_norm, "post-norm Transformers are not on this path"
        if not (isinstance(mask, attentions.Mask) and mask.right_context == 0 and mask.left_context is None and not mask.mask_start):
            raise NotImplementedError("networks.Transformer on the HIP path is the causal LM stack: mask=attentions.Mask(right_context=0)")
        self.pos_embedding = pos_embedding
        self.dropout = nn.Dropout(p=emb_drop_rate)
        self.mask = mask
        self.blocks = nn.ModuleList([blocks.TransformerBlock(dim_model=dim_model, ff_ratio=ff_ratio, att_params=att_params, drop_rate=drop_rate, inner_dropout=inner_dropout,
                                                             act_fun=act_fun, weight_init=weight_init, bias_init=bias_init, post_norm=post_norm) for _ in range(num_blocks)])
        self.layernorm = nn.LayerNorm(normalized_shape=dim_model)

    def forward_rows(self, x, lengths=None, embedded=False):
        if self.training:
            raise RuntimeError("networks.Transformer is an inference path: call .eval() first (training the LM is out of scope)")
        ops._inference_only("networks.Transformer", x)
        if self.pos_embedding is not None and not embedded:
            x = self.pos_embedding(x)
        B, T, D = x.shape
        mask = attentions.CausalMask(lengths)
        for block in self.blocks:
            x = block(x, mask=mask)
        ln = self.layernorm
        return ops.layernorm_fwd(x.reshape(B * T, D), ln.weight, ln.bias, B * T, D, False, ln.eps)[0]

    def forward(self, x, lengths=None):
        B, T, D = x.shape
        return self.forward_rows(x, lengths).float().view(B, T, D)


class ConformerInterCTC(nn.Module):

    def __init__(self, dim_model, num_blocks, interctc_blocks, vocab_size, loss_prefix="ctc", att_params={"class": "MultiHeadAttention", "num_heads": 4},
                 conv_params={"class": "Conv1d", "params": {"padding": "same", "kernel_size": 31}}, ff_ratio=4, drop_rate=0.1, pos_embedding=None,
                 mask=None, conv_stride=1, batch_norm=True):
        super().__init__()
        assert pos_embedding is None
        self.interctc_blocks, self.loss_prefix = interctc_blocks, loss_prefix
        dim_model = [dim_model] if isinstance(dim_model, int) else dim_model
        num_blocks = [num_blocks] if isinstance(num_blocks, int) else num_blocks
        self.pos_embedding = None
        self.dropout = layers.Dropout(p=drop_rate)
        self.mask = mask
        self.conformer_blocks = nn.ModuleList()
        self.interctc_modules = nn.ModuleList()
        i = 1
        for stage, nb in enumerate(num_blocks):
            for b in range(nb):
                down = (b == nb - 1) and (stage < len(num_blocks) - 1)
                d_out = dim_model[stage + 1] if down else dim_model[stage]
                stride = (conv_stride[stage] if isinstance(conv_stride, list) else conv_stride) if down else 1
                self.conformer_blocks.append(blocks.ConformerBlock(
                    dim_model=dim_model[stage], dim_expand=d_out, ff_ratio=ff_ratio, drop_rate=drop_rate,
                    att_params=att_params[stage] if isinstance(att_params, list) else att_params, conv_stride=stride,
                    conv_params=conv_params[stage] if isinstance(conv_params, list) else conv_params, batch_norm=batch_norm))
                if i in interctc_blocks:
                    self.interctc_modules.append(modules.InterCTCResModule(dim_model=d_out, vocab_size=vocab_size))
                i += 1

        for i in range(len(self.conformer_blocks) - 1):
            b0, b1 = self.conformer_blocks[i], self.conformer_blocks[i + 1]
            if (i + 1) not in interctc_blocks and isinstance(b0.norm, nn.LayerNorm) and b0.norm.normalized_shape == b1.ff_module1.layers[0].normalized_shape:
                object.__setattr__(b0, "_next_ln", b1.ff_module1.layers[0])
        i0 = 0
        for nb in num_blocks:
            atts = [getattr(b.self_att_module, "attention", None) for b in self.conformer_blocks[i0:i0 + nb]]
            i0 += nb
# ... 212 lines not shown
```

avec_amd/ops.py:

```python
import collections
import ctypes
import os

import torch

from . import fp8
from . import runtime as rt
from .lib import (ACT_GELU, ACT_NONE, ACT_RELU, ACT_SWISH, BF16, LN_GROUP_MAX, ROWS_CONV_BWD, ROWS_CONV_FWD, ROWS_PLAIN, ROWS_STEM3D, TN_GROUP_MAX, WGRAD_GROUP_MAX, Attn, Epilogue, LnItem, Rows, TnBatched, TnItem,
                  WgradItem, lib)

_byref = ctypes.byref


class KernelTimer:
    NAMES = {(0, ROWS_CONV_FWD): "gemm_nt<conv_fwd>", (0, ROWS_CONV_BWD): "gemm_nt<conv_bwd_data>", (0, ROWS_STEM3D): "gemm_nt<stem3d>",
             (0, ROWS_PLAIN): "gemm_nt<plain>", (1, ROWS_CONV_FWD): "gemm_tn<conv_wgrad>", (1, ROWS_STEM3D): "gemm_tn<stem3d_wgrad>",
             (1, ROWS_PLAIN): "gemm_tn<plain>", (2, 0): "conv3x3_slab<fwd>", (2, 1): "conv3x3_slab<bwd_data>", (2, 2): "conv3x3_slab<wgrad>"}

    def __init__(self):
        self.enabled = False
        self.records = []

    def reset(self, enabled):
        self.enabled, self.records = enabled, []
# ... 162 lines not shown
    if drop_p > 0.0:
        ep.drop_p, ep.rng, ep.rng_stream = drop_p, _rng(out.device, drop_p), sid
    if res is not None:
        ep.res, ep.ldres, ep.res_act, ep.res_cls0 = res.data_ptr(), (N if ldres is None else ldres), int(res_act), int(res_cls0)
        if res_mask is not None:
            ep.res_mask = res_mask.data_ptr()
    ep.alpha = alpha
    if dact_z is not None:
        ep.dact_z, ep.ldz, ep.dact = dact_z.data_ptr(), N, dact
    ep.colsum, ep.stats = _p(colsum), _p(stats)
    if bnb is not None:
        ep.bnb_y, ep.ldby, ep.stats = bnb.y.data_ptr(), N, bnb.stats.data_ptr()
        if bnb.mask_z is not None:
            ep.dact_z, ep.ldz, ep.dact, ep.bnb_mask = bnb.mask_z.data_ptr(), N, 2, 0
        else:
            ep.bnb_ss, ep.bnb_mask = bnb.ss.data_ptr(), 1
    if rows is None:
        rows = rows_plain(K)
    ev = KERNEL_TIMER.start()
    lib.gemm_nt(rt.dt() if dtype is None else dtype, A.data_ptr(), _byref(rows), mode, int(a_f32), W.data_ptr(),
                K if ldw is None else ldw, M, N, K, _byref(ep), rt.stream())
    esz = A.element_size()
    KERNEL_TIMER.stop(ev, (0, mode), 2.0 * M * N * K if flops is None else flops,
                      ((M * K + N * K) * esz + M * N * (4 if out_f32 else esz)) if abytes is None else abytes)
    return out


DEFER_WGRAD = os.environ.get("AVEC_DEFER_WGRAD", "1") != "0"


_QueueKind = collections.namedtuple("_QueueKind", "item group_max launcher dtype timer_key abytes flush_when_full")


def _wgrad3x3_bytes(it):
    return 2.0 * 2 * it.images * it.H * it.W * it.C + 4.0 * 9 * it.C * it.C


_QUEUE_KINDS = {
    "tn": _QueueKind(TnItem, TN_GROUP_MAX, "gemm_tn_grouped", lambda: BF16, (1, ROWS_PLAIN), lambda it: 2.0 * it.M * (it.I + it.J) + 4.0 * it.I * it.J, True),
    "ln": _QueueKind(LnItem, LN_GROUP_MAX, "layernorm_param_grads_grouped", rt.dt, None, None, True),
    "cw": _QueueKind(WgradItem, WGRAD_GROUP_MAX, "wgrad3x3_c128_grouped", None, (2, 2), _wgrad3x3_bytes, False),
    "cw64": _QueueKind(WgradItem, WGRAD_GROUP_MAX, "wgrad3x3_c64_grouped", None, (2, 2), _wgrad3x3_bytes, False),
}


class _PendingGrads:
    __slots__ = ("stream", "items", "flops", "keep")

    def __init__(self, stream):
        self.stream = stream
        self.clear()

    def clear(self):
        self.items, self.flops, self.keep = {k: [] for k in _QUEUE_KINDS}, dict.fromkeys(_QUEUE_KINDS, 0.0), []

    def push(self, kind, item, keep, flops=0.0):
        self.items[kind].append(item)
        self.keep += keep
        self.flops[kind] += flops
        if _QUEUE_KINDS[kind].flush_when_full and len(self.items[kind]) >= _QUEUE_KINDS[kind].group_max:
            self.flush((kind,))

    def flush(self, kinds=None):
        cur = torch.cuda.current_stream()
        if cur.cuda_stream != self.stream.cuda_stream:
            for t in self.keep:
                t.record_stream(cur)
        for kind in (_QUEUE_KINDS if kinds is None else kinds):
            k, items = _QUEUE_KINDS[kind], self.items[kind]
            if not items:
                continue
            ev = KERNEL_TIMER.start() if k.timer_key is not None else None
            for i in range(0, len(items), k.group_max):
                chunk = items[i:i + k.group_max]
                getattr(lib, k.launcher)(*(() if k.dtype is None else (k.dtype(),)), (k.item * len(chunk))(*chunk), len(chunk), rt.stream())
            if ev is not None:
                KERNEL_TIMER.stop(ev, k.timer_key, self.flops[kind], sum(k.abytes(it) for it in items))
            self.items[kind], self.flops[kind] = [], 0.0
        if not any(self.items.values()):
            self.keep = []


class _BackwardPass:
    __slots__ = ("task", "queues", "prep", "ln2", "pos", "bn_ready")

    def __init__(self, task):
        self.task = task
        self.queues = {}
        self.prep = {}
        self.ln2 = {}
        self.pos = {}
        self.bn_ready = {}

    def pending(self):
        st = torch.cuda.current_stream()
        q = self.queues.get(st.cuda_stream)
        if q is None:
            q = self.queues[st.cuda_stream] = _PendingGrads(st)
        return q


_PASS = None


def _pass():
    global _PASS
    task = torch._C._current_graph_task_id()
    if task == -1:
        return None
    if _PASS is None or _PASS.task != task:
        _PASS = _BackwardPass(task)
        torch.autograd.Variable._execution_engine.queue_callback(_flush_at_end)
    return _PASS


def _in_backward():
    return DEFER_WGRAD and torch._C._current_graph_task_id() != -1


def reset_backward_state():
    global _PASS
    _PASS = None


def flush_param_grads(all_streams=False):
    if _PASS is None:
        return
    if all_streams:
        for q in list(_PASS.queues.values()):
            q.flush()
        return
    q = _PASS.queues.get(torch.cuda.current_stream().cuda_stream)
    if q is not None:
        q.flush()


def _flush_at_end():
    global _PASS
    flush_param_grads(all_streams=True)
    _PASS = None


def gemm_tn(P, Q, O, M, I, J, *, ldp=None, q_rows=None, q_mode=ROWS_PLAIN, q_f32=False, ldo=None, dtype=None, p_colsum=None, side=False):
    if q_rows is None:
        q_rows = rows_plain(J)
    if side and q_mode == ROWS_PLAIN and q_f32 and dtype is None and rt.compute_dtype() == "bf16" and _in_backward() and Q.dim() == 2 and Q.dtype == torch.float32:
        Qb = empty((Q.shape[0], J), rt.act_dtype(), Q)
        lib.cast_rows(rt.dt(), Q.data_ptr(), q_rows.ld, Qb.data_ptr(), J, Q.shape[0], J, rt.stream())
        Q, q_f32, q_rows = Qb, False, rows_plain(J, q_rows.rows_out, q_rows.rows_in, q_rows.step)
    if side and q_mode == ROWS_PLAIN and not q_f32 and dtype is None and rt.compute_dtype() == "bf16" and _in_backward():
        it = TnItem()
        it.P, it.Q, it.O, it.p_colsum = P.data_ptr(), Q.data_ptr(), O.data_ptr(), _p(p_colsum)
        it.ldp, it.ldq, it.ldo, it.M, it.I, it.J = (I if ldp is None else ldp), q_rows.ld, (J if ldo is None else ldo), M, I, J
        it.q_rows_out, it.q_rows_in, it.q_step = q_rows.rows_out, q_rows.rows_in, q_rows.step
        if lib.raw("avec_gemm_tn_grouped_ok")(BF16, _byref(it)) and _chunk_readable(P, it.ldp, I, M) and _chunk_readable(Q, it.ldq, J, M):
            _pass().pending().push("tn", it, [P, Q], 2.0 * M * I * J)
            return
    ev = KERNEL_TIMER.start()
    st = rt.stream()
    if side and not KERNEL_TIMER.enabled:
        sd = rt.wgrad_fork(P, Q)
        st = st if sd is None else sd.cuda_stream
    lib.gemm_tn_bias(rt.dt() if dtype is None else dtype, P.data_ptr(), I if ldp is None else ldp, Q.data_ptr(), _byref(q_rows), q_mode,
                     int(q_f32), O.data_ptr(), J if ldo is None else ldo, _p(p_colsum), M, I, J, st)
    KERNEL_TIMER.stop(ev, (1, q_mode), 2.0 * M * I * J, (M * I + M * J) * 2.0 + I * J * 4.0)


def layernorm_fwd(x, w, b, M, D, out_f32, eps):
    y = empty((M, D), torch.float32 if out_f32 else rt.act_dtype(), x)
    mean = empty((M,), torch.float32, x)
    rstd = empty((M,), torch.float32, x)
    lib.layernorm_fwd(rt.dt(), x.data_ptr(), w.data_ptr(), b.data_ptr(), y.data_ptr(), int(out_f32), mean.data_ptr(), rstd.data_ptr(), M, D, eps,
                      rt.stream())
    return y, mean, rstd


def _tag_prep(out, alpha, drop_p, sid):
    out._avec_prep = (float(alpha), float(drop_p), int(sid))
    return out


def _prep_request(x):
    return getattr(x, "_avec_prep", None)


def _take_prep(dy, M, N, alpha, drop_p, sid):
    p = _pass()
    r = None if p is None else p.prep.pop(dy.data_ptr(), None)
    if r is not None and r[1:] == (M, N, float(alpha), float(drop_p), int(sid)) and r[0].dtype == rt.act_dtype():
        return r[0]
    return None


def layernorm_bwd(dy, dy_f32, x, mean, rstd, w, b, M, D, dres=None, prep=None):
    dx = empty((M, D), torch.float32, x)
    gw, gb = grad_of(w), grad_of(b)
# ... 513 lines not shown
        lib.relpos_attention_fwd(rt.dt(), _byref(a), rt.stream())
        ctx.saved = (qkv, e, o, lse, lens, len_div, mask, B, H, T, d, scale)
        return o

    @staticmethod
    def backward(ctx, do):
        qkv, e, o, lse, lens, len_div, mask, B, H, T, d, scale = ctx.saved
        D, adt = H * d, rt.act_dtype()
        do = do.to(adt).contiguous()
        dqkv = empty((B * T, 3 * D), adt, do)
        de = torch.zeros((2 * T - 1, D), dtype=torch.float32, device=do.device)
        a = _attn_args(qkv, e, lens, len_div, mask, o, lse, B, H, T, d, D, scale=scale)
        dsrel = torch.zeros((H, B * T, _pad8(2 * T - 1)), dtype=adt, device=do.device)
        _attn_backward(a, do, dqkv, dsrel, de, products=True)
        return dqkv, de.to(adt), None, None, None, None, None, None, None, None


def relpos_core_infer(q, k, v, e, lens, mask, B, H, T, Tk, d, scale, want_probs=False):
    rt.require_gpu(q)
    D, adt = H * d, rt.act_dtype()
    for t in (q, k, v, e):
        assert t.dtype == adt and t.is_contiguous()
    assert q.shape == (B * T, D) and k.shape == (B * Tk, D) and v.shape == (B * Tk, D) and e.shape == (Tk + T - 1, D)
    if mask is not None:
        mask = mask.reshape(mask.shape[0], T, Tk).float().contiguous()
    o = empty((B * T, D), adt, q)
    lse = empty((B * H, T, 2), torch.float32, q)
    a = _attn_args(q, e, lens, 1, mask, o, lse, B, H, T, d, D, kv=(k, v, D), Tk=Tk, scale=scale)
    lib.relpos_attention_fwd(rt.dt(), _byref(a), rt.stream())
    if not want_probs:
        return o, None
    dq = empty((B * T, D), adt, q)
    zero = torch.zeros((B * T, D), dtype=adt, device=q.device)
    dsrel = torch.zeros((H, B * T, _pad8(Tk + T - 1)), dtype=adt, device=q.device)
    scratch = _attn_backward(a, zero, dq, dsrel)
    return o, scratch[0].view(B, H, T, -1)[..., :Tk].float()


def _pool_mask(mask, T, P):
    pad = (P - T % P) % P
    m = torch.nn.functional.pad(mask.reshape(mask.shape[0], 1, T, T).float(), (0, pad, 0, pad), value=0.0)
    Tp = (T + pad) // P
    return m.reshape(m.shape[0], Tp, P, Tp, P).amin(dim=(2, 4))


class BNState:

    NREP = 64

    def __init__(self, C, ref):
        self.stats = rt.zeros_scratch(self.NREP * 2 * C, ref.device)
        self.red = None
        self.ss = torch.empty(4 * C, dtype=torch.float32, device=ref.device)
        self.C = C


RELU_BITMASK = True
def bn_finalize(bn, st, count, training):
    C = st.C
    cptr = None
    sptr, nrep = st.stats.data_ptr(), st.NREP
    if training and rt.sync_batchnorm():
        st.red = rt.sync_bn_stats(st.stats, st.NREP, C, count, key=(id(bn), "f"))
        sptr, nrep, cptr = st.red.data_ptr(), 1, st.red.data_ptr() + 2 * C * 4
    lib.bn_finalize(sptr, nrep, cptr, float(count), bn.weight.data_ptr(), bn.bias.data_ptr(), *_bn_running(bn, training), bn.eps, st.ss.data_ptr(), C, int(training),
                    rt.stream())
    return cptr


def _bn_running(bn, training):
    track = bn.track_running_stats and bn.running_mean is not None
    return (bn.running_mean.data_ptr() if track else None, bn.running_var.data_ptr() if track else None,
            bn.num_batches_tracked.data_ptr() if (track and training) else None, bn.momentum if bn.momentum is not None else 0.1)


def bn_backward(bn, st, cptr, count, dout, y, out, act, M, want_dres=False, pre=None, mask=None):
    C = st.C
    adt = rt.act_dtype()
    dstats = rt.zeros_scratch(2 * C, dout.device)
    if pre is not None:
        lib.bn_bwd_finalize(pre.stats.data_ptr(), BNState.NREP, st.ss.data_ptr(), dstats.data_ptr(), C, rt.stream())
        act, out, want_dres, mask = ACT_NONE, None, False, None
    elif mask is not None:
        lib.bn_bwd_reduce_mask(rt.dt(), dout.data_ptr(), y.data_ptr(), mask.data_ptr(), st.ss.data_ptr(), dstats.data_ptr(), M, C, rt.stream())
    else:
        lib.bn_bwd_reduce(rt.dt(), dout.data_ptr(), y.data_ptr(), _p(out), st.ss.data_ptr(), act, dstats.data_ptr(), M, C, rt.stream())
    dstats, gw, gb = _bn_sync_grads(bn, dstats, C)
    dy = empty((M, C), adt, dout)
    dres = empty((M, C), adt, dout) if want_dres else None
    if mask is not None:
        lib.bn_bwd_apply_mask(rt.dt(), dout.data_ptr(), y.data_ptr(), mask.data_ptr(), st.ss.data_ptr(), bn.weight.data_ptr(), dstats.data_ptr(), cptr, float(count),
                              dy.data_ptr(), _p(dres), _p(gw), _p(gb), M, C, rt.stream())
    else:
        lib.bn_bwd_apply(rt.dt(), dout.data_ptr(), y.data_ptr(), _p(out), st.ss.data_ptr(), bn.weight.data_ptr(), dstats.data_ptr(), cptr, float(count), act,
                         dy.data_ptr(), _p(dres), _p(gw), _p(gb), M, C, rt.stream())
    return dy, (dout if pre is not None else dres)


def _add_local_affine_grads(dstats, gw, gb, C, key):
    if not rt.sync_batchnorm():
        return dstats, False
    from . import peer
    px = peer.active()
    if px is not None and dstats.is_cuda and dstats.is_contiguous() :
        return px.all_reduce_sum_fused(dstats, 1, 2 * C, None, key, dgamma=gw, dbeta=gb, C=C), True
    lib.bn_affine_grads(dstats.data_ptr(), gw.data_ptr(), gb.data_ptr(), C, rt.stream())
    return rt.all_reduce_small(dstats, key), True


def _bn_sync_grads(bn, dstats, C):
    gw, gb = grad_of(bn.weight), grad_of(bn.bias)
    dstats, synced = _add_local_affine_grads(dstats, gw, gb, C, (id(bn), "b"))
    return (dstats, None, None) if synced else (dstats, gw, gb)


def dw_pad_left(conv):
    K = conv.kernel_size[0]
    kind = getattr(conv, "padding_type", "same")
    if kind == "causal":
        return K - 1
    assert kind == "same", "the fused convolution module supports 'same' and 'causal' padding, got %r" % (kind,)
    return K // 2

CONVMOD_BN_FUSE = True


class ConvModuleFn(torch.autograd.Function):
    @staticmethod
    def forward(ctx, x, _anchor, mod, res_conv, drop_p, sid, training):
        rt.require_gpu(x)
        B, T, D = x.shape
        ln, pw1, dw, bn, pw2 = mod.layers[0], mod.layers[1], mod.layers[3], mod.layers[4], mod.layers[6]
        Dp, K, stride = dw.weight.shape[0], dw.weight.shape[2], dw.stride[0]
        To = (T - 1) // stride + 1
        M, Mo, adt = B * T, B * To, rt.act_dtype()
        x2 = _f32c(x.reshape(M, D))
        h, mean, rstd = layernorm_fwd(x2, ln.weight, ln.bias, M, D, False, ln.eps)
        u = linear_fwd(h, pw1.weight, pw1.bias, M, in_f32=False, out_f32=False)
        c = empty((Mo, Dp), adt, x2)
        st = BNState(Dp, x2)
        use_batch = training and not getattr(bn, "frozen", False)
        if use_batch and not rt.sync_batchnorm() and CONVMOD_BN_FUSE:
            lib.glu_dwconv_fwd_bn(rt.dt(), u.data_ptr(), dw.weight.data_ptr(), _p(dw.bias), c.data_ptr(), st.stats.data_ptr(), B, T, Dp, K, stride, dw_pad_left(dw),
                                  bn.weight.data_ptr(), bn.bias.data_ptr(), *_bn_running(bn, use_batch), bn.eps, st.ss.data_ptr(), rt.stream())
            cptr = None
        else:
            lib.glu_dwconv_fwd(rt.dt(), u.data_ptr(), dw.weight.data_ptr(), _p(dw.bias), c.data_ptr(), st.stats.data_ptr() if use_batch else None,
                               B, T, Dp, K, stride, dw_pad_left(dw), rt.stream())
            cptr = bn_finalize(bn, st, Mo, use_batch)
        a = empty((Mo, Dp), adt, x2)
        lib.bn_apply_fwd(rt.dt(), c.data_ptr(), st.ss.data_ptr(), None, ACT_SWISH, a.data_ptr(), Mo, Dp, rt.stream())
        if res_conv is not None:
            rs = res_conv.stride[0]
            R = linear_fwd(x2, res_conv.weight, res_conv.bias, Mo, in_f32=(adt != torch.float32), out_f32=True,
                           rows=rows_plain(D, To, T, rs) if rs > 1 else None)
        else:
            R = x2
        y = linear_fwd(a, pw2.weight, pw2.bias, Mo, in_f32=False, out_f32=True, drop_p=drop_p, sid=sid, res=R, alpha=1.0)
        ctx.saved = (x2, mean, rstd, h, u, c, a, st, cptr, use_batch, mod, res_conv, drop_p, sid, B, T, To, D, Dp, K, stride)
        ctx.prep_req = _prep_request(x)
        return _tag_prep(y.view(B, To, Dp), 1.0, drop_p, sid)

    @staticmethod
    def backward(ctx, dy):
        x2, mean, rstd, h, u, c, a, st, cptr, use_batch, mod, res_conv, drop_p, sid, B, T, To, D, Dp, K, stride = ctx.saved
        ln, pw1, dw, bn, pw2 = mod.layers[0], mod.layers[1], mod.layers[3], mod.layers[4], mod.layers[6]
        M, Mo, adt = B * T, B * To, rt.act_dtype()
        dy = _f32c(dy.reshape(Mo, Dp))
        dacc = _take_prep(dy, Mo, Dp, 1.0, drop_p, sid)
        if dacc is None:
            dacc = grad_prep(dy, Mo, Dp, drop_p=drop_p, sid=sid)
        linear_bwd_weight(dacc, a, pw2.weight, Mo, bias=pw2.bias)
        da = linear_bwd_input(dacc, pw2.weight, Mo, out_f32=False)
        du = empty((M, 2 * Dp), adt, dy)
        if use_batch and CONVMOD_BN_FUSE and stride == 1 and not rt.sync_batchnorm():
            dstats = rt.zeros_scratch(2 * Dp, da.device)
            lib.bn_bwd_reduce(rt.dt(), da.data_ptr(), c.data_ptr(), None, st.ss.data_ptr(), ACT_SWISH, dstats.data_ptr(), Mo, Dp, rt.stream())
            lib.dwconv_glu_bwd_bn(rt.dt(), da.data_ptr(), c.data_ptr(), st.ss.data_ptr(), bn.weight.data_ptr(), dstats.data_ptr(), float(Mo), u.data_ptr(), dw.weight.data_ptr(),
# ... 162 lines not shown
        ctx.mark_non_differentiable(*outs)
        return (total,) + outs

    @staticmethod
    def backward(ctx, dtotal, *_unused):
        grads, B, n, weights = ctx.saved
        out = [None, None, None, None, None]
        if dtotal is None:
            return tuple(out + [None, None] * n)
        dt = dtotal.float().contiguous()
        live = [i for i in range(n) if grads[i] is not None]
        outs = {i: torch.empty_like(grads[i]) for i in live}
        if live:
            k = len(live)
            lib.scale_by_scalar_multi(k, (ctypes.c_void_p * k)(*[grads[i].data_ptr() for i in live]), (ctypes.c_void_p * k)(*[outs[i].data_ptr() for i in live]),
                                      (ctypes.c_longlong * k)(*[grads[i].numel() for i in live]), (ctypes.c_float * k)(*[weights[i] / B for i in live]), dt.data_ptr(), rt.stream())
        for i in range(n):
            out += [outs.get(i), None]
        return tuple(out)


_WCACHE = {}


def ctc_multi_fits(T, V, Lmax):
    return bool(lib.raw("avec_ctc_loss_multi_fits")(int(T), int(V), int(Lmax)))


class TimeMeanFn(torch.autograd.Function):

    @staticmethod
    def forward(ctx, x):
        from .lib import F32
        rt.require_gpu(x)
        B, T, V = x.shape
        x = _f32c(x)
        y = empty((B, V), torch.float32, x)
        lib.avgpool_fwd(F32, x.data_ptr(), y.data_ptr(), B, T, V, rt.stream())
        ctx.saved = (B, T, V)
        return y

    @staticmethod
    def backward(ctx, dy):
        from .lib import F32
        B, T, V = ctx.saved
        dy = _f32c(dy)
        dx = empty((B, T, V), torch.float32, dy)
        lib.avgpool_bwd(F32, dy.data_ptr(), dx.data_ptr(), B, T, V, rt.stream())
        return dx


class SoftmaxCEFn(torch.autograd.Function):

    @staticmethod
    def forward(ctx, logits, targets, ignore_index):
        rt.require_gpu(logits)
        M, V = logits.shape
        lg = _f32c(logits)
        tg = targets.to(device=lg.device, dtype=torch.int64).contiguous()
        loss = empty((M,), torch.float32, lg)
        mean = torch.zeros((), dtype=torch.float32, device=lg.device)
        grad = empty((M, V), torch.float32, lg) if ctx.needs_input_grad[0] else None
        lib.softmax_ce(lg.data_ptr(), tg.data_ptr(), int(ignore_index), loss.data_ptr(), mean.data_ptr(), _p(grad), M, V, rt.stream())
        ctx.saved = (grad, M)
        return mean

    @staticmethod
    def backward(ctx, dloss):
        grad, M = ctx.saved
        out = torch.empty_like(grad)
        lib.scale_by_scalar(grad.data_ptr(), dloss.float().contiguous().data_ptr(), 1.0 / M, out.data_ptr(), grad.numel(), rt.stream())
        return out, None, None


def conv2d_fwd(x, weight, N, H, W, Cin, stride, stats=None):
    Cout, KH, KW = weight.shape[0], weight.shape[2], weight.shape[3]
    pad = (KH - 1) // 2
    OH, OW = (H - 1) // stride + 1, (W - 1) // stride + 1
    M = N * OH * OW
    sh = rt.shadow(weight)
    y = empty((M, Cout), rt.act_dtype(), x)
    if _slab_conv(H, W, Cin, Cout, KH, KW, stride):
        ev = KERNEL_TIMER.start()
        lib.conv3x3_c64(x.data_ptr(), sh.fwd.data_ptr(), y.data_ptr(), None, _p(stats), N, H, W, 0, rt.stream())
        KERNEL_TIMER.stop(ev, (2, 0), 2.0 * M * Cout * KH * KW * Cin, 2.0 * (N * H * W * Cin + Cout * KH * KW * Cin + M * Cout))
        return y, OH, OW
    gemm_nt(x, sh.fwd, y, M, Cout, KH * KW * Cin, rows=rows_conv(H, W, Cin, KH, KW, stride, pad, OH, OW), mode=ROWS_CONV_FWD, stats=stats,
            abytes=2.0 * (N * H * W * Cin + Cout * KH * KW * Cin + M * Cout))
    return y, OH, OW


SHORTCUT_SUBGRID = True
GROUP_WGRAD128 = True


def _slab_conv(H, W, Cin, Cout, KH, KW, stride):
    return rt.act_dtype() == torch.bfloat16 and bool(lib.raw("avec_conv3x3_c64_supported")(H, W, Cin, Cout, KH, KW, stride))


class BnbFuse:
    __slots__ = ("y", "ss", "mask_z", "stats", "done")

    def __init__(self, y, ss, mask_z, C):
        self.y, self.ss, self.mask_z, self.done = y, ss, mask_z, False
        self.stats = rt.zeros_scratch(BNState.NREP * 2 * C, y.device)


BNB_FUSE = False


def conv2d_bwd(dy, x, weight, N, H, W, Cin, stride, OH, OW, need_dx=True, dx_res=None, bnb=None, dx_res_cls0=False, dx_res_mask=None):
    Cout, KH, KW = weight.shape[0], weight.shape[2], weight.shape[3]
    pad = (KH - 1) // 2
    M = N * OH * OW
    sh = rt.shadow(weight)
    slab64 = _slab_conv(H, W, Cin, Cout, KH, KW, stride) and H * (W + 1) <= 512
    wide = not slab64 and rt.act_dtype() == torch.bfloat16 and bool(lib.raw("avec_wgrad3x3_c128_supported")(H, W, Cin, Cout, KH, KW, stride))
    if slab64 or wide:
        if GROUP_WGRAD128 and _in_backward():
            it = WgradItem()
            it.x, it.dy, it.dw, it.images, it.C, it.H, it.W = x.data_ptr(), dy.data_ptr(), grad_of(weight).data_ptr(), N, Cin, H, W
            _pass().pending().push("cw64" if slab64 else "cw", it, [x, dy], 2.0 * M * Cout * KH * KW * Cin)
        else:
            ev = KERNEL_TIMER.start()
            if slab64:
                lib.wgrad3x3_c64(x.data_ptr(), dy.data_ptr(), grad_of(weight).data_ptr(), N, H, W, rt.stream())
            else:
                lib.wgrad3x3_c128(x.data_ptr(), dy.data_ptr(), grad_of(weight).data_ptr(), N, Cin, H, W, rt.stream())
            KERNEL_TIMER.stop(ev, (2, 2), 2.0 * M * Cout * KH * KW * Cin)
    else:
        gemm_tn(dy, x, grad_of(weight), M, Cout, KH * KW * Cin, q_rows=rows_conv(H, W, Cin, KH, KW, stride, pad, OH, OW), q_mode=ROWS_CONV_FWD, side=True)
    if not need_dx:
        return None
    dx = empty((N * H * W, Cin), rt.act_dtype(), dy)
    if _slab_conv(H, W, Cin, Cout, KH, KW, stride):
        ev = KERNEL_TIMER.start()
        if dx_res_mask is not None:
            lib.conv3x3_c64_res_masked(dy.data_ptr(), sh.bwd.data_ptr(), dx.data_ptr(), dx_res.data_ptr(), dx_res_mask.data_ptr(), N, H, W, 1, rt.stream())
        else:
            lib.conv3x3_c64(dy.data_ptr(), sh.bwd.data_ptr(), dx.data_ptr(), _p(dx_res), None, N, H, W, 1, rt.stream())
        KERNEL_TIMER.stop(ev, (2, 1), 2.0 * N * H * W * Cin * KH * KW * Cout, 2.0 * (2 * N * H * W * Cin + Cout * KH * KW * Cin + M * Cout))
        return dx
    fuse = bnb if (bnb is not None and BNB_FUSE and rt.act_dtype() == torch.bfloat16 and Cin % 4 == 0) else None
    gemm_nt(dy, sh.bwd, dx, N * H * W, Cin, KH * KW * Cout, rows=rows_conv(H, W, Cout, KH, KW, stride, pad, OH, OW), mode=ROWS_CONV_BWD,
            res=dx_res, res_act=True, flops=2.0 * N * OH * OW * Cout * KH * KW * Cin, bnb=fuse, res_cls0=dx_res_cls0, res_mask=dx_res_mask,
            abytes=2.0 * (N * H * W * Cin * (2 if dx_res is not None else 1) + Cout * KH * KW * Cin + M * Cout))
    if fuse is not None:
        fuse.done = True
    return dx


def res_mask_ok(H, W, Cin, Cout, stride):
    if rt.act_dtype() != torch.bfloat16 or stride != 1 or Cin != Cout:
        return False
    return _slab_conv(H, W, Cin, Cout, 3, 3, 1) or (Cin >= 128 and Cin % 32 == 0 and W <= 31)


class ResNetBlockFn(torch.autograd.Function):

    _CHAIN = {}

    @staticmethod
    def forward(ctx, x, _anchor, blk, training, chain=False):
        rt.require_gpu(x)
        N, H, W, Cin = x.shape
        conv1, bn1, conv2, bn2 = blk.layers[0], blk.layers[1], blk.layers[3], blk.layers[4]
        stride = conv1.stride[0]
        Cout = conv1.weight.shape[0]
        adt = rt.act_dtype()
        x = x.contiguous()
        st1, st2 = BNState(Cout, x), BNState(Cout, x)
        y1, OH, OW = conv2d_fwd(x, conv1.weight, N, H, W, Cin, stride, stats=st1.stats if training else None)
        Mo = N * OH * OW
        c1 = bn_finalize(bn1, st1, Mo, training)
        a1 = empty((Mo, Cout), adt, x)
        lib.bn_apply_fwd(rt.dt(), y1.data_ptr(), st1.ss.data_ptr(), None, ACT_RELU, a1.data_ptr(), Mo, Cout, rt.stream())
        y2, _, _ = conv2d_fwd(a1, conv2.weight, N, OH, OW, Cout, 1, stats=st2.stats if training else None)
        c2 = bn_finalize(bn2, st2, Mo, training)
        has_proj = not isinstance(blk.residual, torch.nn.Identity)
        yr = str_ = cr = None
        if has_proj:
            convr, bnr = blk.residual[0], blk.residual[1]
            str_ = BNState(Cout, x)
            yr, _, _ = conv2d_fwd(x, convr.weight, N, H, W, Cin, stride, stats=str_.stats if training else None)
            cr = bn_finalize(bnr, str_, Mo, training)
        use_mask = RELU_BITMASK and training and Cout % 8 == 0 and Cout <= 2048 and Mo * Cout // 8 < (1 << 31)
        if has_proj and not use_mask:
            r = empty((Mo, Cout), adt, x)
            lib.bn_apply_fwd(rt.dt(), yr.data_ptr(), str_.ss.data_ptr(), None, ACT_NONE, r.data_ptr(), Mo, Cout, rt.stream())
        elif not has_proj:
            r = x
        out = empty((Mo, Cout), adt, x)
        ctx.relu_mask = None
        if use_mask:
            ctx.relu_mask = torch.empty(Mo * Cout // 8, dtype=torch.uint8, device=x.device)
            lib.bn_apply_fwd_mask(rt.dt(), y2.data_ptr(), st2.ss.data_ptr(), (yr if has_proj else r).data_ptr(), str_.ss.data_ptr() if has_proj else None, out.data_ptr(),
                                  ctx.relu_mask.data_ptr(), Mo, Cout, rt.stream())
        else:
            lib.bn_apply_fwd(rt.dt(), y2.data_ptr(), st2.ss.data_ptr(), r.data_ptr(), ACT_RELU, out.data_ptr(), Mo, Cout, rt.stream())
        ctx.saved = (x, y1, a1, y2, yr, out, st1, st2, str_, c1, c2, cr, blk, training, N, H, W, Cin, Cout, OH, OW, stride, has_proj)
        ctx.chain = bool(chain and training and BNB_FUSE and rt.act_dtype() == torch.bfloat16)
        if ctx.chain:
            if len(ResNetBlockFn._CHAIN) > 64:
                ResNetBlockFn._CHAIN.clear()
            ResNetBlockFn._CHAIN[out.data_ptr()] = (y2, out, st2, Cout)
        return out.view(N, OH, OW, Cout)

    @staticmethod
    def backward(ctx, dout):
        x, y1, a1, y2, yr, out, st1, st2, str_, c1, c2, cr, blk, training, N, H, W, Cin, Cout, OH, OW, stride, has_proj = ctx.saved
        conv1, bn1, conv2, bn2 = blk.layers[0], blk.layers[1], blk.layers[3], blk.layers[4]
        Mo = N * OH * OW
        dout = dout.reshape(Mo, Cout).to(rt.act_dtype()).contiguous()
        assert training, "ResNetBlock backward is implemented for training-mode BatchNorm"
        ResNetBlockFn._CHAIN.pop(out.data_ptr(), None)
        pre2 = _pass().bn_ready.pop(dout.data_ptr(), None) if ctx.chain else None
        if pre2 is not None and pre2.y is not y2:
            raise RuntimeError("ResNetBlock backward: a fused BatchNorm-backward request does not belong to this block (the block output has another consumer?)")
        lazy_dres = (not BNB_FUSE and ctx.relu_mask is not None and pre2 is None and
                     (has_proj or (conv1.weight.shape[2] == 3 and res_mask_ok(H, W, Cin, Cout, stride) and not KERNEL_TIMER.enabled)))
        dy2, dres = bn_backward(bn2, st2, c2, Mo, dout, y2, out, ACT_RELU, Mo, want_dres=not lazy_dres, pre=pre2, mask=ctx.relu_mask)
        f1 = BnbFuse(y1, st1.ss, None, Cout)
        da1 = conv2d_bwd(dy2, a1, conv2.weight, N, OH, OW, Cout, 1, OH, OW, bnb=f1)
        dy1, _ = bn_backward(bn1, st1, c1, Mo, da1, y1, None, ACT_RELU, Mo, pre=f1 if f1.done else None)
        need_dx = ctx.needs_input_grad[0]
        prev = ResNetBlockFn._CHAIN.get(x.data_ptr()) if need_dx else None
        fx = BnbFuse(prev[0], prev[2].ss, prev[1], prev[3]) if prev is not None else None
        if has_proj:
            convr, bnr = blk.residual[0], blk.residual[1]
            if lazy_dres:
                dyr, _ = bn_backward(bnr, str_, cr, Mo, dout, yr, None, ACT_NONE, Mo, mask=ctx.relu_mask)
            else:
                dyr, _ = bn_backward(bnr, str_, cr, Mo, dres, yr, None, ACT_NONE, Mo)
            kr = convr.weight.shape[2]
            if (SHORTCUT_SUBGRID and need_dx and stride == 2 and kr == 1 and rt.act_dtype() == torch.bfloat16 and Cin % 64 == 0 and Cout % 64 == 0
                    and conv1.weight.shape[2] == 3 and not _slab_conv(H, W, Cin, Cout, 3, 3, stride)):
                conv2d_bwd(dyr, x, convr.weight, N, H, W, Cin, stride, OH, OW, need_dx=False)
                dxs = empty((Mo, Cin), rt.act_dtype(), dyr)
                gemm_nt(dyr, rt.shadow(convr.weight).bwd, dxs, Mo, Cin, Cout)
                dx = conv2d_bwd(dy1, x, conv1.weight, N, H, W, Cin, stride, OH, OW, need_dx=True, dx_res=dxs, bnb=fx, dx_res_cls0=True)
            else:
                dx = conv2d_bwd(dyr, x, convr.weight, N, H, W, Cin, stride, OH, OW, need_dx=need_dx)
                dx = conv2d_bwd(dy1, x, conv1.weight, N, H, W, Cin, stride, OH, OW, need_dx=need_dx, dx_res=dx, bnb=fx)
        else:
            if lazy_dres:
                dx = conv2d_bwd(dy1, x, conv1.weight, N, H, W, Cin, stride, OH, OW, need_dx=need_dx, dx_res=dout, dx_res_mask=ctx.relu_mask, bnb=fx)
            else:
                dx = conv2d_bwd(dy1, x, conv1.weight, N, H, W, Cin, stride, OH, OW, need_dx=need_dx, dx_res=dres, bnb=fx)
        if fx is not None and fx.done:
            _pass().bn_ready[dx.data_ptr()] = fx
        return (dx.view(N, H, W, Cin) if dx is not None else None), None, None, None, None


STEM3D_DIRECT = True
STEM3P_FUSED_WGRAD = True
STEM3P = True


class VideoStemFn(torch.autograd.Function):

    @staticmethod
    def forward(ctx, video, _anchor, conv, bn, training):
        rt.require_gpu(video)
        B, T, H, W = video.shape
        C = conv.weight.shape[0]
        v = _f32c(video)
        OH, OW = (H - 1) // 2 + 1, (W - 1) // 2 + 1
        M = B * T * OH * OW
        sh = rt.shadow(conv.weight)
        st = BNState(C, v)
        K, Kp = sh.Tm * sh.C, sh.Cp
        y = empty((M, C), rt.act_dtype(), v)
        if (STEM3P and STEM3D_DIRECT and rt.compute_dtype() == "bf16" and C == 64 and K == 245 and lib.raw("avec_stem3p_supported")(B, T, H, W)
                and lib.raw("avec_stem3d_supported")(B, T, H, W)):
            w8 = torch.zeros((C, 36, 8), dtype=sh.fwd.dtype, device=v.device)
            w8[:, :35, 1:] = sh.fwd.view(C, Kp)[:, :K].view(C, 35, 7)
            vb = v.to(torch.bfloat16)
            PH, PW = (OH - 1) // 2 + 1, (OW - 1) // 2 + 1
            zp = torch.empty((B * T, PH, PW, C), dtype=torch.bfloat16, device=v.device)
            idx = torch.empty((B * T, PH, PW, C), dtype=torch.uint8, device=v.device)
            lib.stem3p_fwd(vb.data_ptr(), w8.data_ptr(), _p(conv.bias), bn.weight.data_ptr(), zp.data_ptr(), idx.data_ptr(), st.stats.data_ptr() if training else None,
                           B, T, H, W, rt.stream())
            cp = bn_finalize(bn, st, M, training)
            out = torch.empty_like(zp)
            lib.bn_apply_fwd(rt.dt(), zp.data_ptr(), st.ss.data_ptr(), None, ACT_RELU, out.data_ptr(), B * T * PH * PW, C, rt.stream())
            ctx.saved = (v, None, idx, st, cp, conv, bn, ("p", vb, w8, zp, PH, PW), B, T, OH, OW, C, M, K, training, None)
            return out
        if STEM3D_DIRECT and rt.compute_dtype() == "bf16" and C == 64 and K == 245 and lib.raw("avec_stem3d_supported")(B, T, H, W):
            w8 = torch.zeros((C, 36, 8), dtype=sh.fwd.dtype, device=v.device)
            w8[:, :35, :7] = sh.fwd.view(C, Kp)[:, :K].view(C, 35, 7)
            lib.stem3d_fwd(v.data_ptr(), w8.data_ptr(), 288, _p(conv.bias), y.data_ptr(), st.stats.data_ptr() if training else None, B, T, H, W, rt.stream())
            r = None
        else:
            A = empty((M, Kp), rt.act_dtype(), v)
            lib.stem_im2col(rt.dt(), v.data_ptr(), A.data_ptr(), B, T, H, W, Kp, rt.stream())
            gemm_nt(A, sh.fwd, y, M, C, Kp, bias=conv.bias, stats=st.stats if training else None)
            r = A
        cp = bn_finalize(bn, st, M, training)
        PH, PW = (OH - 1) // 2 + 1, (OW - 1) // 2 + 1
        out = empty((B * T, PH, PW, C), rt.act_dtype(), v)
        idx = torch.empty((B * T, PH, PW, C), dtype=torch.uint8, device=v.device)
        ymax = torch.empty_like(out) if (training and C % 8 == 0) else None
        lib.stem_pool_fwd(rt.dt(), y.data_ptr(), st.ss.data_ptr(), out.data_ptr(), idx.data_ptr(), _p(ymax), B * T, OH, OW, C, rt.stream())
        ctx.saved = (v, y, idx, st, cp, conv, bn, r, B, T, OH, OW, C, M, K, training, ymax)
        return out

    @staticmethod
    def backward(ctx, dpool):
        v, y, idx, st, cp, conv, bn, r, B, T, OH, OW, C, M, K, training, ymax = ctx.saved
        assert training, "VideoStem backward is implemented for training-mode BatchNorm"
        dpool = dpool.to(rt.act_dtype()).contiguous()
        if isinstance(r, tuple):
            _, vb, w8, zp, PH, PW = r
            H, W = v.shape[2], v.shape[3]
            dstats = torch.zeros(2 * C, dtype=torch.float32, device=v.device)
            lib.stem3p_reduce(dpool.data_ptr(), zp.data_ptr(), st.ss.data_ptr(), dstats.data_ptr(), B * T, PH, PW, rt.stream())
            dstats, gw, gb = _bn_sync_grads(bn, dstats, C)
            if STEM3P_FUSED_WGRAD and lib.raw("avec_stem3p_wgrad_supported")(B, T, H, W):
                lib.stem3p_wgrad(vb.data_ptr(), w8.data_ptr(), _p(conv.bias), dpool.data_ptr(), idx.data_ptr(), st.ss.data_ptr(), bn.weight.data_ptr(), dstats.data_ptr(), cp, float(M),
                                 grad_of(conv.weight).data_ptr(), _p(gw), _p(gb), B, T, H, W, rt.stream())
            else:
                dy = empty((M, C), rt.act_dtype(), v)
                lib.stem3p_dz(vb.data_ptr(), w8.data_ptr(), _p(conv.bias), dpool.data_ptr(), idx.data_ptr(), st.ss.data_ptr(), bn.weight.data_ptr(), dstats.data_ptr(), cp, float(M),
                              dy.data_ptr(), _p(gw), _p(gb), B, T, H, W, rt.stream())
                lib.stem3d_wgrad(v.data_ptr(), dy.data_ptr(), grad_of(conv.weight).data_ptr(), B, T, H, W, rt.stream())
            if conv.bias is not None:
                grad_of(conv.bias)
            stamp("v_stem_end:b")
            return None, None, None, None, None
        dstats = torch.zeros(2 * C, dtype=torch.float32, device=v.device)

        def common(ds):
            return dpool.data_ptr(), idx.data_ptr(), y.data_ptr(), st.ss.data_ptr(), bn.weight.data_ptr(), ds.data_ptr(), cp, float(M)
        if ymax is not None:
            lib.stem_pool_bwd_reduce_pooled(rt.dt(), dpool.data_ptr(), idx.data_ptr(), ymax.data_ptr(), st.ss.data_ptr(), dstats.data_ptr(), B * T, OH, OW, C, rt.stream())
        else:
            lib.stem_pool_bwd(rt.dt(), *common(dstats), 0, None, None, None, B * T, OH, OW, C, rt.stream())
        dstats, gw, gb = _bn_sync_grads(bn, dstats, C)
        dy = empty((M, C), rt.act_dtype(), v)
        lib.stem_pool_bwd(rt.dt(), *common(dstats), 1, dy.data_ptr(), _p(gw), _p(gb), B * T, OH, OW, C, rt.stream())
        if r is None:
            H, W = v.shape[2], v.shape[3]
            lib.stem3d_wgrad(v.data_ptr(), dy.data_ptr(), grad_of(conv.weight).data_ptr(), B, T, H, W, rt.stream())
        else:
            gemm_tn(dy, r, grad_of(conv.weight), M, C, K, q_rows=rows_plain(r.shape[1]), side=True)
        if conv.bias is not None:
            grad_of(conv.bias)
        return None, None, None, None, None


class AvgPoolFn(torch.autograd.Function):

    @staticmethod
    def forward(ctx, x):
        N, H, W, C = x.shape
        x = x.contiguous()
        y = empty((N, C), x.dtype, x)
        lib.avgpool_fwd(rt.dt(), x.data_ptr(), y.data_ptr(), N, H * W, C, rt.stream())
        ctx.saved = (N, H, W, C)
        return y

    @staticmethod
    def backward(ctx, dy):
        N, H, W, C = ctx.saved
        dy = dy.to(rt.act_dtype()).contiguous()
        dx = empty((N, H, W, C), dy.dtype, dy)
        lib.avgpool_bwd(rt.dt(), dy.data_ptr(), dx.data_ptr(), N, H * W, C, rt.stream())
        return dx
# ... 656 lines not shown
```

include/avec_hip.h:

```cpp
#ifndef AVEC_HIP_H
#define AVEC_HIP_H
#include <stdint.h>
#ifdef __HIPCC__
#include <hip/hip_runtime.h>
#else
typedef struct ihipStream_t* hipStream_t;
#endif
#ifdef __cplusplus
extern "C" {
#endif

#define AVEC_F32 0
#define AVEC_BF16 1
#define AVEC_ABI_VERSION 4
#define AVEC_STAT_REPLICAS 64

int avec_version(void);
int avec_struct_size(int which);
const char* avec_last_error(void);
const char* avec_last_kernel(void);
int avec_set_reduce_workspace(void* base, long long bytes);
int avec_set_reduce_workspace_stream(void* base, long long bytes, hipStream_t stream);

enum { AVEC_ROWS_PLAIN = 0, AVEC_ROWS_CONV_FWD = 1, AVEC_ROWS_CONV_BWD = 2 };
// ... 27 lines not shown
int avec_fp8_quantize(int src_dtype, const void* x, long long ldx, void* q, long long ldq, long long M, int K, float* amax, int compute_amax, hipStream_t stream);
int avec_fp8_weights_refresh(const avec_fp8_item_t* table, int n_items, int blocks_per_item, float* amax, hipStream_t stream);
int avec_gemm_nt_fp8(const void* A, long long lda, const void* W, long long ldw, long long M, int N, int K,
                     const float* amax_a, const float* amax_w, const avec_epilogue_t* ep, hipStream_t stream);


int avec_gemm_tn(int dtype, const void* P, long long ldp, const void* Q, const avec_rows_t* q_rows, int q_mode, int q_f32,
                 float* O, long long ldo, long long M, int I, int J, hipStream_t stream);
int avec_gemm_tn_bias(int dtype, const void* P, long long ldp, const void* Q, const avec_rows_t* q_rows, int q_mode, int q_f32,
                      float* O, long long ldo, float* p_colsum, long long M, int I, int J, hipStream_t stream);
#define AVEC_TN_GROUP_MAX 32
typedef struct avec_tn_item {
  const void* P; const void* Q; float* O; float* p_colsum;
  long long ldp, ldq, ldo, M;
  int I, J;
  int q_rows_out, q_rows_in, q_step;
  int reserved;
} avec_tn_item_t;
int avec_gemm_tn_grouped_ok(int dtype, const avec_tn_item_t* item);
int avec_gemm_tn_grouped(int dtype, const avec_tn_item_t* items, int n, hipStream_t stream);
int avec_gemm_tn_batched(int dtype, const void* P, long long ldp, const void* Q, long long ldq, float* O, long long ldo, long long M, int I, int J,
                         int nb_outer, int nb_inner, const long long* strides6, hipStream_t stream);
int avec_gemm_tn_batched_store(int dtype, const void* P, long long ldp, const void* Q, long long ldq, void* O_act, long long ldo, long long M, int I, int J,
                               int nb_outer, int nb_inner, const long long* strides6, hipStream_t stream);

typedef struct {
  const void* P; long long ldp; const void* Q; long long ldq;
  float* O; void* O_act; long long ldo;
  long long M; int I, J, nb_outer, nb_inner;
  const long long* strides6;
} avec_tn_batched_t;
int avec_gemm_tn_batched_multi(int dtype, const avec_tn_batched_t* items, int n, hipStream_t stream);

#define AVEC_PEER_MAX_WORLD 8
int avec_peer_exchange_sum(const float* in, float* out, int n, void* const* pages, long long page_stride_granules, int rank, int world,
                           unsigned* epoch, int* err_flag, int timeout_ms, hipStream_t stream);
int avec_peer_exchange_sum_fused(const float* in, int n_replicas, int n_in, int has_tail, float tail, float* dgamma, float* dbeta, int C, float* out,
                                 void* const* pages, long long page_stride_granules, int rank, int world, unsigned* epoch, int* err_flag, int timeout_ms,
                                 hipStream_t stream);
int avec_enable_peer_access(int peer_device);
int avec_peer_buffer_alloc(void** ptr, long long bytes, void* ipc_handle_64b);
int avec_peer_buffer_open(const void* ipc_handle_64b, void** ptr);
int avec_peer_buffer_close(void* ptr);
int avec_peer_buffer_free(void* ptr);

int avec_layernorm_fwd(int dtype, const float* x, const float* gamma, const float* beta, void* y, int y_f32,
                       float* mean, float* rstd, long long M, int D, float eps, hipStream_t stream);
int avec_layernorm_bwd(int dtype, const void* dy, int dy_f32, const float* x, const float* mean, const float* rstd, const float* gamma,
                       float* dx, const float* dres, float* dgamma, float* dbeta, long long M, int D, hipStream_t stream);
int avec_layernorm_bwd_prep(int dtype, const void* dy, int dy_f32, const float* x, const float* mean, const float* rstd, const float* gamma,
                            float* dx, const float* dres, void* prep, float prep_alpha, float prep_drop_p, const unsigned long long* rng, unsigned rng_stream,
                            long long M, int D, hipStream_t stream);
int avec_layernorm_fwd2(int dtype, const float* x, const float* gamma1, const float* beta1, float eps1, float* y1, float* mean1, float* rstd1,
                        const float* gamma2, const float* beta2, float eps2, void* h2, float* mean2, float* rstd2, long long M, int D, hipStream_t stream);
int avec_layernorm_bwd2(int dtype, const void* dy2, const float* x2, const float* mean2, const float* rstd2, const float* gamma2, const float* dres2, float* dx2,
                        const float* x1, const float* mean1, const float* rstd1, const float* gamma1, float* dx1,
                        void* prep, float prep_alpha, float prep_drop_p, const unsigned long long* rng, unsigned rng_stream, long long M, int D, hipStream_t stream);
#define AVEC_LN_GROUP_MAX 40
typedef struct avec_ln_item {
  const void* dy; const float* x; const float* mean; const float* rstd; float* dgamma; float* dbeta;
  long long M; int D; int dy_f32;
} avec_ln_item_t;
int avec_layernorm_param_grads_grouped(int dtype, const avec_ln_item_t* items, int n, hipStream_t stream);
int avec_grad_prep(int dtype, const float* dout, long long ld, void* dacc, float alpha, float drop_p, const unsigned long long* rng,
                   unsigned rng_stream, float* dbias, long long M, int N, hipStream_t stream);
int avec_colsum(int dtype, const void* x, long long ld, float* out, long long M, int N, hipStream_t stream);
int avec_strided_rows_add(float* dx, const float* src, int B, int T, int To, int D, int step, hipStream_t stream);
int avec_bn_stats(int dtype, const void* y, float* stats, long long M, int C, hipStream_t stream);
int avec_bn_collapse(const float* stats, int n_replicas, float count, float* out, int C, hipStream_t stream);
int avec_bn_affine_grads(const float* dstats, float* dgamma, float* dbeta, int C, hipStream_t stream);
int avec_bn_finalize(const float* stats, int n_replicas, const float* count_ptr, float count, const float* gamma, const float* beta, float* running_mean,
                     float* running_var, long long* num_batches_tracked, float momentum, float eps, float* ss, int C, int training, hipStream_t stream);
int avec_stamp(unsigned long long* out, int slot, hipStream_t stream);
int avec_bn_bwd_finalize(const float* stats, int n_replicas, const float* ss, float* dstats, int C, hipStream_t stream);
int avec_bn_apply_fwd(int dtype, const void* y, const float* ss, const void* residual, int act, void* out, long long M, int C, hipStream_t stream);
int avec_bn_bwd_reduce(int dtype, const void* dout, const void* y, const void* out, const float* ss, int act, float* dstats, long long M, int C, hipStream_t stream);
int avec_bn_bwd_apply(int dtype, const void* dout, const void* y, const void* out, const float* ss, const float* gamma, const float* dstats,
                      const float* count_ptr, float count, int act, void* dy, void* dres, float* dgamma, float* dbeta, long long M, int C, hipStream_t stream);
int avec_bn_apply_fwd_mask(int dtype, const void* y, const float* ss, const void* residual, const float* residual_ss, void* out, unsigned char* mask, long long M, int C,
                           hipStream_t stream);
int avec_bn_bwd_reduce_mask(int dtype, const void* dout, const void* y, const unsigned char* mask, const float* ss, float* dstats, long long M, int C, hipStream_t stream);
int avec_bn_bwd_apply_mask(int dtype, const void* dout, const void* y, const unsigned char* mask, const float* ss, const float* gamma, const float* dstats,
                           const float* count_ptr, float count, void* dy, void* dres, float* dgamma, float* dbeta, long long M, int C, hipStream_t stream);
int avec_softmax_fwd(int dtype, const float* logits, void* probs, long long M, int V, hipStream_t stream);
int avec_softmax_bwd(int dtype, const void* dprobs, const float* logits, float* dlogits, const float* dadd, long long M, int V, hipStream_t stream);
int avec_cast_rows(int dtype, const float* src, long long ld_src, void* dst, long long ld_dst, long long M, int N, hipStream_t stream);
int avec_to_f32_rows(int dtype, const void* src, long long ld_src, float* dst, long long ld_dst, long long M, int N, int accum, hipStream_t stream);
int avec_act_f32(int act, const float* x, const float* dy, float* out, long long rows, int C, int backward, hipStream_t stream);
int avec_dropout_f32(const float* x, float* y, float p, const unsigned long long* rng, unsigned rng_stream, long long n, hipStream_t stream);
int avec_maxpool_hw_fwd(int dtype, const void* x, void* out, unsigned char* idx, long long frames, int H, int W, int C, int KH, int KW, int SH, int SW,
                        int pad0_h, int pad0_w, int pad1_h, int pad1_w, hipStream_t stream);
int avec_maxpool_hw_bwd(int dtype, const void* dy, const unsigned char* idx, void* dx, long long frames, int H, int W, int C, int KH, int KW, int SH, int SW,
                        int pad0_h, int pad0_w, int pad1_h, int pad1_w, hipStream_t stream);
int avec_upsample_rows(int dtype, const void* src, void* dst, long long B, int T, int D, int P, int backward, hipStream_t stream);
int avec_patch_pool_fwd(int dtype, const void* x, void* y, int B, int T, int D, int P, hipStream_t stream);
int avec_patch_pool_bwd(int dtype, const void* dy, void* dx, int B, int T, int D, int P, hipStream_t stream);
int avec_patch_unpool_add(int dtype, const void* o, const float* res, float* out, float drop_p, const unsigned long long* rng, unsigned rng_stream,
                          int B, int T, int D, int P, hipStream_t stream);
int avec_patch_unpool_bwd(int dtype, const float* dout, void* dob, float drop_p, const unsigned long long* rng, unsigned rng_stream,
                          int B, int T, int D, int P, hipStream_t stream);
int avec_avgpool_fwd(int dtype, const void* x, void* y, long long N, int HW, int C, hipStream_t stream);
int avec_avgpool_bwd(int dtype, const void* dy, void* dx, long long N, int HW, int C, hipStream_t stream);

int avec_glu_dwconv_fwd(int dtype, const void* u, const float* w, const float* bias, void* out, float* stats,
                        int B, int T, int C, int K, int stride, int pad_left, hipStream_t stream);
int avec_glu_dwconv_fwd_bn(int dtype, const void* u, const float* w, const float* bias, void* out, float* stats, int B, int T, int C, int K, int stride, int pad_left,
                           const float* gamma, const float* beta, float* running_mean, float* running_var, long long* num_batches_tracked, float momentum, float eps,
                           float* ss, hipStream_t stream);
int avec_dwconv_glu_bwd(int dtype, const void* dc, const void* u, const float* w, void* du, float* dw, float* dbias,
                        int B, int T, int C, int K, int stride, int pad_left, hipStream_t stream);
int avec_dwconv_glu_bwd_bn(int dtype, const void* da, const void* c, const float* ss, const float* gamma, const float* dstats, float count, const void* u, const float* w,
                           void* du, float* dw, float* dbias, float* dgamma, float* dbeta, int B, int T, int C, int K, int pad_left, hipStream_t stream);

typedef struct avec_attn {
  const void *q, *k, *v; long long ld;
  const void* e; long long lde;
  const long long* lens; int len_div;
  int q_full;
  const float* mask; long long mask_bstride;
  void* o; long long ldo; float* lse;
  const void* dout;
  void *dq, *dk, *dv; long long lddq, ldd;
  float* de; long long ldde;
  void *pbuf, *dsbuf; long long ldt;
  void* dsrel; long long ldr;
  int B, H, T, d; float scale;
  int Tk;
} avec_attn_t;
int avec_relpos_attention_fwd(int dtype, const avec_attn_t* args, hipStream_t stream);
int avec_relpos_attention_bwd(int dtype, const avec_attn_t* args, hipStream_t stream);

long long avec_glu_dwconv_stream_state_bytes(int dtype, int B, int C, int K);
int avec_glu_dwconv_stream(int dtype, const void* u, const float* w, const float* bias, const float* ss, void* out, void* state, long long state_bytes,
                           const long long* pos, const unsigned char* reset, const long long* chunk_len, int div, int B, int Tq, int C, int K, int stride, hipStream_t stream);
long long avec_relpos_attention_stream_state_bytes(int dtype, int B, int H, int d, int L, int Tq);
int avec_relpos_attention_stream(int dtype, const void* q, const void* k, const void* v, long long ld, const void* e, long long lde, void* kcache, void* vcache,
                                 long long cache_bytes, const long long* pos, const unsigned char* reset, const long long* chunk_len, int div, void* o, long long ldo,
                                 int B, int H, int Tq, int d, int L, float scale, hipStream_t stream);
int avec_stream_advance(long long* pos, unsigned char* reset, const long long* chunk_len, long long full, int B, hipStream_t stream);

int avec_stream_window(const float* x_new, const float* tail, float* X, const long long* pend, const long long* n_new, const unsigned char* last, const unsigned char* reset,
                       const unsigned char* ended, long long* nvalid, long long* ncommit, long long* emit, int B, int Tc, int LAe, int D, int S, hipStream_t stream);
int avec_stream_window_advance(const float* X, float* tail, long long* pend, long long* pos, const long long* nvalid, const long long* ncommit, unsigned char* last,
                               unsigned char* reset, unsigned char* ended, int B, int W, int LAe, int D, hipStream_t stream);
int avec_glu_dwconv_stream_la(int dtype, const void* u, const float* w, const float* bias, const float* ss, void* out, void* state, long long state_bytes,
                              const long long* pos, const unsigned char* reset, const long long* ncommit, int div, int B, int Wq, int C, int K, int stride, hipStream_t stream);
int avec_relpos_attention_stream_la(int dtype, const void* q, const void* k, const void* v, long long ld, const void* e, long long lde, void* kcache, void* vcache,
                                    long long cache_bytes, const long long* pos, const unsigned char* reset, const long long* nvalid, const long long* ncommit, int div,
                                    void* o, long long ldo, int B, int H, int Wq, int Tq, int d, int L, int R, float scale, hipStream_t stream);

long long avec_audio_stream_state_bytes(int B);
int avec_mel_frames_stream(const float* wave, long long ldw, const float* window, float* frames, const void* state, long long state_bytes,
                           const long long* n_samples, const unsigned char* reset, const unsigned char* last, long long* out_len, long long* meta,
                           int B, int W, int Tmax, int n_fft, int win, int hop, hipStream_t stream);
int avec_audio_stem_stream(int dtype, const float* mel, const float* w, const float* bias, const float* ss, void* out, const long long* out_len,
                           const long long* meta, int B, int n_mels, int Tmax, int C, hipStream_t stream);
int avec_audio_stream_advance(const float* wave, long long ldw, void* state, long long state_bytes, const long long* n_samples, unsigned char* reset,
                              unsigned char* last, int B, int W, int n_fft, int win, int hop, hipStream_t stream);

long long avec_video_stream_state_bytes(int dtype, int B, int H, int W);
int avec_video_stem_stream(int dtype, const float* chunk, long long ldc, const void* state, long long state_bytes, const long long* n_frames,
                           const unsigned char* reset, const unsigned char* last, const void* w8, const float* bias, const float* ss, void* out,
                           long long* out_len, int B, int Tin, int Tmax, int H, int W, hipStream_t stream);
int avec_video_stream_advance(int dtype, const float* chunk, long long ldc, void* state, long long state_bytes, const long long* n_frames, unsigned char* reset,
                              unsigned char* last, int B, int Tin, int H, int W, hipStream_t stream);

long long avec_av_fuse_stream_state_bytes(int dtype, int B, int Da, int Dv, int cap);
int avec_av_fuse_stream(int dtype, const float* a, const long long* a_len, const float* v, const long long* v_len, void* state, long long state_bytes,
                        unsigned char* reset, void* xc, long long* pair_len, int B, int Ra, int Rv, int Da, int Dv, int cap, int max_emit, hipStream_t stream);

int avec_mel_frames(const float* audio, const float* window, float* frames, int B, long long L, int n_fft, int win, int hop, hipStream_t stream);
int avec_mel_power_log(const float* spec, const float* fb, float* out, int B, int F, int n_bins, int n_mels, hipStream_t stream);
int avec_specaugment(float* mel, const long long* lens, int B, int n_mels, int F, int mF, int Fparam, int mT, float pS,
                     const unsigned long long* rng, unsigned rng_stream, hipStream_t stream);
int avec_debug_rng_uniform(const unsigned long long* rng, unsigned rng_stream, const long long* ids, int n, float* out, hipStream_t stream);
int avec_audio_stem_conv_fwd(int dtype, const float* mel, const float* w, const float* bias, void* y, float* stats, int B, int n_mels, int F, int C, hipStream_t stream);
int avec_audio_stem_act_fwd(int dtype, const void* y, const float* ss, void* a, int B, int n_mels, int F, int C, hipStream_t stream);
int avec_audio_stem_bwd(int dtype, const void* da, const void* y, const float* mel, const float* ss, const float* gamma, float* dstats,
                        const float* count_ptr, float count, int phase, float* dw, float* dbias, float* dgamma, float* dbeta,
                        int B, int n_mels, int F, int C, hipStream_t stream);
int avec_stem_im2col(int dtype, const float* video, void* A, long long clips, int T, int H, int W, int ldk, hipStream_t stream);
int avec_stem3d_supported(long long clips, int T, int H, int W);
int avec_stem3d_fwd(const float* video, const void* w_shadow, int ldw, const float* bias, void* y, float* stats, long long clips, int T, int H, int W, hipStream_t stream);
int avec_stem3d_wgrad(const float* video, const void* dy, float* dw, long long clips, int T, int H, int W, hipStream_t stream);
int avec_stem3p_supported(long long clips, int T, int H, int W);
int avec_stem3p_fwd(const void* video_bf16, const void* w_shadow, const float* bias, const float* gamma, void* zp, unsigned char* idx, float* stats,
                    long long clips, int T, int H, int W, hipStream_t stream);
int avec_stem3p_reduce(void* dpool, const void* zp, const float* ss, float* dstats, long long frames, int PH, int PW, hipStream_t stream);
int avec_stem3p_wgrad_supported(long long clips, int T, int H, int W);
int avec_stem3p_geom(long long clips, int T, int H, int W, int* out);
int avec_stem3p_wgrad(const void* video_bf16, const void* w_shadow, const float* bias, const void* dpool_masked, const unsigned char* idx, const float* ss,
                      const float* gamma, const float* dstats, const float* count_ptr, float count, float* dw, float* dgamma, float* dbeta,
                      long long clips, int T, int H, int W, hipStream_t stream);
int avec_stem3p_dz(const void* video_bf16, const void* w_shadow, const float* bias, const void* dpool_masked, const unsigned char* idx, const float* ss,
                   const float* gamma, const float* dstats, const float* count_ptr, float count, void* dz, float* dgamma, float* dbeta,
                   long long clips, int T, int H, int W, hipStream_t stream);
int avec_stem_pool_fwd(int dtype, const void* y, const float* ss, void* out, unsigned char* idx, void* ymax, long long frames, int H, int W, int C, hipStream_t stream);
int avec_stem_pool_bwd_reduce_pooled(int dtype, const void* dpool, const unsigned char* idx, const void* ymax, const float* ss, float* dstats,
                                     long long frames, int H, int W, int C, hipStream_t stream);
int avec_stem_pool_bwd(int dtype, const void* dpool, const unsigned char* idx, const void* y, const float* ss, const float* gamma, float* dstats,
                       const float* count_ptr, float count, int phase, void* dy, float* dgamma, float* dbeta, long long frames, int H, int W, int C, hipStream_t stream);

int avec_conv3x3_c64_supported(int H, int W, int Cin, int Cout, int KH, int KW, int stride);
int avec_conv3x3_c64(const void* x, const void* w, void* y, const void* res, float* stats, long long images, int H, int W, int flip, hipStream_t stream);
int avec_conv3x3_c64_res_masked(const void* x, const void* w, void* y, const void* res, const unsigned char* res_mask, long long images, int H, int W, int flip, hipStream_t stream);
int avec_wgrad3x3_c64(const void* x, const void* dy, float* dw, long long images, int H, int W, hipStream_t stream);
int avec_wgrad3x3_c128_supported(int H, int W, int Cin, int Cout, int KH, int KW, int stride);
int avec_wgrad3x3_c128(const void* x, const void* dy, float* dw, long long images, int C, int H, int W, hipStream_t stream);
#define AVEC_WGRAD_GROUP_MAX 16
typedef struct { const void* x; const void* dy; float* dw; long long images; int C, H, W, reserved; } avec_wgrad3x3_item_t;
int avec_wgrad3x3_c128_grouped(const avec_wgrad3x3_item_t* items, int n, hipStream_t stream);
int avec_wgrad3x3_c64_grouped(const avec_wgrad3x3_item_t* items, int n, hipStream_t stream);

int avec_video_input(const unsigned char* clips, const long long* clip_off, const int* geom, const int* masks, int max_masks, int channels, const float* lut, float mean, float stdv,
                     int mean_frame, float* out, float* frame_ws, int B, int Tout, int OH, int OW, hipStream_t stream);
int avec_video_tta_batch(const float* x, float* y, int B, long long rows, int W, int n, unsigned flip_mask, hipStream_t stream);

long long avec_ctc_workspace_floats(int B, int T, int Lmax);
int avec_ctc_loss(const float* logits, const long long* in_lens, const long long* targets, const long long* tgt_lens, float* nll, float* mean_out,
                  float* grad, float* workspace, int B, int T, int V, int Lmax, int blank, int zero_infinity, hipStream_t stream);
int avec_ctc_loss_multi_fits(int T, int V, int Lmax);
int avec_ctc_loss_multi(int n_heads, const float* const* logits, const long long* const* in_lens, const int* T, float* const* nll, float* const* mean_out, float* const* grad,
                        const long long* targets, const long long* tgt_lens, const float* weights, float* total, int B, int V, int Lmax, int blank, int zero_infinity, hipStream_t stream);
int avec_scale_by_scalar(const float* g, const float* scalar_dev, float mul, float* out, long long n, hipStream_t stream);
int avec_scale_by_scalar_multi(int n_tensors, const float* const* g, float* const* out, const long long* numel, const float* mul, const float* scalar_dev, hipStream_t stream);
int avec_softmax_ce(const float* logits, const long long* targets, long long ignore_index, float* loss, float* mean_out, float* grad, long long M, int V, hipStream_t stream);
int avec_len_affine(const long long* in, long long* out, int n, long long sub, long long div, long long add, hipStream_t stream);
int avec_argmax_rows(const float* x, long long* out, long long M, int V, hipStream_t stream);

typedef struct avec_ngram {
  int order;
  int V;
  const float* unigram;
  long long ctx_cap;
  const unsigned long long* ctx_key;
  const float* ctx_bo;
  const int* ctx_off;
  const int* ctx_cnt;
  const int* cont_tok;
  const float* cont_lp;
} avec_ngram_t;
long long avec_ctc_beam_workspace_bytes(int B, int T, int W);
int avec_ctc_beam_search(const float* logits, const long long* lengths, int B, int T, int V, int W, float inv_tmp, const avec_ngram_t* lm, float alpha, float beta,
                         float oov_logprob, void* workspace, long long workspace_bytes, int* tokens, int* out_len, float* score, float* ctc_logp, hipStream_t stream);
long long avec_ctc_beam_state_bytes(int B, int W);
int avec_ctc_beam_stream(const float* logits, const long long* chunk_len, const unsigned char* reset, int B, int Tc, int V, int W, int Tcap, float inv_tmp,
                         const avec_ngram_t* lm, float alpha, float beta, float oov_logprob, void* state, long long state_bytes, void* backptr, long long backptr_bytes,
                         int* tokens, int* out_len, float* score, float* ctc_logp, int* stable_len, int emit, hipStream_t stream);
long long avec_ctc_beam_ring_state_bytes(int B, int W);
long long avec_ctc_beam_ring_workspace_bytes(int B, int window, int W);
int avec_ctc_beam_stream_ring(const float* logits, const long long* chunk_len, const unsigned char* reset, int B, int Tc, int V, int W, int window, int log_frames,
                              float inv_tmp, const avec_ngram_t* lm, float alpha, float beta, float oov_logprob, void* state, long long state_bytes, void* backptr,
                              long long backptr_bytes, void* log, long long log_bytes, int* tokens, int* frames, int* out_len, float* score, float* ctc_logp,
                              int* stable_len, int* info, int emit, hipStream_t stream);
int avec_ngram_rows(const avec_ngram_t* lm, const int* ctx, const int* ctx_len, int n, int max_len, float oov_logprob, float* rows, hipStream_t stream);
long long avec_ctc_align_workspace_bytes(int B, int T, int Lmax);
int avec_ctc_align_fits_lds(int T, int Lmax);
int avec_ctc_align(const float* logits, const long long* in_lens, const long long* targets, const long long* tgt_lens,
                   int B, int T, int V, int Lmax, int blank, int tier ,
                   void* workspace, long long workspace_bytes,
                   int* path, int* spans, float* score, float* token_logp, hipStream_t stream);
int avec_embed_pos(int dtype, const long long* ids, const float* E, const float* P, void* out, int out_f32, long long N, int L, int V, int D, hipStream_t stream);
int avec_causal_attention_supported(int d);
int avec_causal_attention(int dtype, const void* qkv, long long ld, const long long* lens, void* o, long long ldo, int N, int H, int L, int d, float scale, hipStream_t stream);
long long avec_lm_head_nll_workspace_bytes(long long R, int V, int D);
int avec_lm_head_nll(int dtype, const void* h, long long ldh, const void* W, long long ldw, const float* bias, const long long* tgt, float* nll, long long R, int V, int D,
                     void* workspace, long long workspace_bytes, hipStream_t stream);
int avec_lm_segment_sum(const float* nll, const long long* lens, long long S, int L, float* out, hipStream_t stream);
int avec_lm_rescore_select(const float* neural, const long long* lens, const float* beam_score, float alpha, float beta, int B, int K, float* total, long long* best,
                           hipStream_t stream);
int avec_ctc_tta_pick(const int* tokens, const int* out_len, const float* score, const long long* best_slot, int B, int n, int W, int T, long long* best_aug,
                      long long* best_beam, long long* ids, long long* ids_len, float* best_score, hipStream_t stream);
int avec_adam_step(float* params, float* grads, float* exp_avg, float* exp_avg_sq, const float* state_dev, float beta1, float beta2, float eps,
                   float weight_decay, float grad_scale, int zero_grad, long long n, hipStream_t stream);
int avec_adam_step_guarded(float* params, float* grads, float* exp_avg, float* exp_avg_sq, const float* state_dev, float beta1, float beta2, float eps,
                           float weight_decay, float grad_scale, int zero_grad, long long n, const int* skip_flag, hipStream_t stream);
long long avec_grad_norm_workspace_bytes(long long n);
int avec_grad_norm_blocks(long long n);
int avec_grad_norm(const float* g, long long n, float grad_scale, float max_norm, int skip_nonfinite, const int* skip_in, void* workspace, long long workspace_bytes,
                   float* stats, int* flag, hipStream_t stream);
int avec_adam_step_clipped(float* params, float* grads, float* exp_avg, float* exp_avg_sq, const float* state_dev, float beta1, float beta2, float eps,
                           float weight_decay, float grad_scale, int zero_grad, long long n, const int* skip_flag, const float* clip_dev, hipStream_t stream);
int avec_weight_average(float* avg, const float* p, int mode, float wa, float wp, long long n, hipStream_t stream);
int avec_shadow_refresh(int dtype, const float* master, void* shadow, const long long* table_dev, int n_entries, long long total_blocks, hipStream_t stream);
int avec_shadow_refresh_range(int dtype, const float* master, void* shadow, const long long* table_dev, int n_entries, long long first_block, long long n_blocks, hipStream_t stream);

#ifdef __cplusplus
}
// ... 3 lines not shown
```

Baseline: 1943.

## Alternate traversal order of consecutive streaming kernels to reuse cache-resident data

Adds an order flag to the slab conv3x3 kernels and the sliced batch-norm apply/reduce kernels so they can walk images or slices in reverse. The Python side alternates the order between consecutive launches, so each kernel starts on the data the previous one touched last and is more likely to find it still in L2/MALL. The bwd-reduce path now also takes the sliced kernel for the unmasked case when reversed. This adds a per-launch order state machine and changes the atomic accumulation order, which can alter floating-point rounding.

```diff
diff --git a/avec_amd/csrc/conv3x3.hip b/avec_amd/csrc/conv3x3.hip
--- a/avec_amd/csrc/conv3x3.hip
+++ b/avec_amd/csrc/conv3x3.hip
@@ -7,7 +7,8 @@
 #define C3_MAXPIX 576
 #define C3_SBYTES (C3_MAXPIX * 128)
 
-struct C3Args { const bf16* x; const bf16* w; bf16* y; const bf16* res; float* stats; int N, H, W, flip; const unsigned char* rmask; };
+struct C3Args { const bf16* x; const bf16* w; bf16* y; const bf16* res; float* stats; int N, H, W, flip; const unsigned char* rmask; int rev; };
+__device__ __forceinline__ long long c3_img(const C3Args& a, long long n) { return a.rev ? a.N - 1 - n : n; }
 
 __device__ __forceinline__ int c3_wslot(int n, int c) { return (c & ~15) | ((c & 15) ^ (n & 15)); }
 __device__ __forceinline__ int c3_saddr(int pix, int c) { const int pr = pix >> 1; return pr * 256 + (((((pix & 1) << 3) | c) ^ (pr & 7)) << 4); }
@@ -96,7 +97,7 @@
         for (int k = 0; k < 2; ++k) resp[RES ? j : 0][i][k] = u32x4{0u, 0u, 0u, 0u};
   }
   if ((long long)blockIdx.x < a.N && !(C3S_ABL & 2)) {
-    const bf16* x0 = a.x + (long long)blockIdx.x * HW * 64;
+    const bf16* x0 = a.x + c3_img(a, blockIdx.x) * HW * 64;
 #pragma unroll
     for (int i = 0; i < 9; ++i) C3_GLOAD(pf[i], ldoff[i], x0, 0);
     asm volatile("s_waitcnt vmcnt(0)");
@@ -151,8 +152,8 @@
     };
     const bool has_prev = prev >= 0 && !(C3S_ABL & (8 | 16)), has_next = n + gridDim.x < a.N;
     const bf16* const yprev = a.y + (has_prev ? prev : 0) * HW * 64;
-    const bf16* const xnext = a.x + (has_next ? n + gridDim.x : n) * HW * 64;
-    const bf16* const rcur = RES ? a.res + n * HW * 64 : a.x;
+    const bf16* const xnext = a.x + c3_img(a, has_next ? n + gridDim.x : n) * HW * 64;
+    const bf16* const rcur = RES ? a.res + c3_img(a, n) * HW * 64 : a.x;
     auto one_tap = [&](int tap) {
       int ax0, ax1, aw0, aw1; bool z0, z1;
       tap_addr(tap, ax0, ax1, aw0, aw1, z0, z1);
@@ -204,7 +205,7 @@
       for (int i = 0; i < 2; ++i) for (int j = 0; j < 2; ++j) for (int r = 0; r < 16; ++r) t += acc[j][i][r];
       if (t == 1234.5f) outp[0][0][0][0] = 1u;
       asm volatile("" :: "v"(t));
-      prev = n; continue;
+      prev = c3_img(a, n); continue;
     }
 #pragma unroll
     for (int i = 0; i < 2; ++i)
@@ -232,7 +233,7 @@
           swap_pair(o[0], o[1]);
           outp[j][i][k] = u32x4{o[0].x, o[0].y, o[1].x, o[1].y};
         }
-    prev = n;
+    prev = c3_img(a, n);
     C3S_STAMP(4);
 #ifdef C3S_TRACE
     ++tr_k;
@@ -323,7 +324,7 @@
 
   chunk16 pf[9];
   if ((long long)blockIdx.x < a.N) {
-    const bf16* x0 = a.x + (long long)blockIdx.x * HW * 64;
+    const bf16* x0 = a.x + c3_img(a, blockIdx.x) * HW * 64;
 #pragma unroll
     for (int i = 0; i < 9; ++i) pf[i] = ldg16(x0 + (soff[i] < 0 ? 0 : soff[i]));
   }
@@ -337,7 +338,7 @@
     }
     __syncthreads();
     if (n + gridDim.x < a.N) {
-      const bf16* xn = a.x + (n + gridDim.x) * HW * 64;
+      const bf16* xn = a.x + c3_img(a, n + gridDim.x) * HW * 64;
 #pragma unroll
       for (int i = 0; i < 9; ++i) pf[i] = ldg16(xn + (soff[i] < 0 ? 0 : soff[i]));
     }
@@ -392,7 +393,8 @@
     }
 #undef C3_ST
     if (a.res) {
-      const bf16* ro = a.res + n * HW * 64;
+      const long long ni = c3_img(a, n);
+      const bf16* ro = a.res + ni * HW * 64;
 #pragma unroll
       for (int i = 0; i < 2; ++i)
 #pragma unroll
@@ -400,7 +402,7 @@
 #pragma unroll
           for (int k = 0; k < 2; ++k) resp[j][i][k] = *(const uint4*)(ro + (long long)pm[i] * 64 + j * 32 + k * 16 + chq);
       if (a.rmask) {
-        const unsigned char* mo = a.rmask + n * HW * 8;
+        const unsigned char* mo = a.rmask + ni * HW * 8;
         unsigned mb[2][2][2];
 #pragma unroll
         for (int i = 0; i < 2; ++i)
@@ -443,7 +445,7 @@
           swap_pair(o[0], o[1]);
           outp[j][i][k] = make_uint4(o[0].x, o[0].y, o[1].x, o[1].y);
         }
-    prev = n;
+    prev = c3_img(a, n);
   }
   issue_stores();
 }
@@ -812,22 +814,31 @@
   return Cin == 64 && Cout == 64 && KH == 3 && KW == 3 && stride == 1 && H * W <= 512 && (H + 2) * (W + 1) + 1 <= C3_MAXPIX && H >= 1 && W >= 2;
 }
 
-static int conv3x3_c64_impl(const void* x, const void* w, void* y, const void* res, const unsigned char* rmask, float* stats, long long images, int H, int W, int flip, hipStream_t st);
+static int conv3x3_c64_impl(const void* x, const void* w, void* y, const void* res, const unsigned char* rmask, float* stats, long long images, int H, int W, int flip, int order,
+                            hipStream_t st);
+extern "C" int avec_conv3x3_c64_ord(const void* x, const void* w, void* y, const void* res, float* stats, long long images, int H, int W, int flip, int order, hipStream_t st) {
+  return conv3x3_c64_impl(x, w, y, res, nullptr, stats, images, H, W, flip, order, st);
+}
 extern "C" int avec_conv3x3_c64(const void* x, const void* w, void* y, const void* res, float* stats, long long images, int H, int W, int flip, hipStream_t st) {
-  return conv3x3_c64_impl(x, w, y, res, nullptr, stats, images, H, W, flip, st);
+  return conv3x3_c64_impl(x, w, y, res, nullptr, stats, images, H, W, flip, 0, st);
+}
+extern "C" int avec_conv3x3_c64_res_masked_ord(const void* x, const void* w, void* y, const void* res, const unsigned char* res_mask, long long images, int H, int W, int flip, int order,
+                                               hipStream_t st) {
+  AVEC_CHECK_ARG(res && res_mask, "conv3x3_c64_res_masked: null residual / mask");
+  return conv3x3_c64_impl(x, w, y, res, res_mask, nullptr, images, H, W, flip, order, st);
 }
 extern "C" int avec_conv3x3_c64_res_masked(const void* x, const void* w, void* y, const void* res, const unsigned char* res_mask, long long images, int H, int W, int flip, hipStream_t st) {
-  AVEC_CHECK_ARG(res && res_mask, "conv3x3_c64_res_masked: null residual / mask");
-  return conv3x3_c64_impl(x, w, y, res, res_mask, nullptr, images, H, W, flip, st);
-}
-static int conv3x3_c64_impl(const void* x, const void* w, void* y, const void* res, const unsigned char* rmask, float* stats, long long images, int H, int W, int flip, hipStream_t st) {
-  AVEC_CHECK_ARG(x && w && y && images > 0, "conv3x3_c64: null buffer");
+  return avec_conv3x3_c64_res_masked_ord(x, w, y, res, res_mask, images, H, W, flip, 0, st);
+}
+static int conv3x3_c64_impl(const void* x, const void* w, void* y, const void* res, const unsigned char* rmask, float* stats, long long images, int H, int W, int flip, int order,
+                            hipStream_t st) {
+  AVEC_CHECK_ARG(x && w && y && images > 0 && (order == 0 || order == 1), "conv3x3_c64: null buffer or an order other than 0 / 1");
   AVEC_CHECK_ARG(avec_conv3x3_c64_supported(H, W, 64, 64, 3, 3, 1), "conv3x3_c64: %dx%d images do not fit the slab", H, W);
   AVEC_CHECK_ARG(!(stats && res), "conv3x3_c64: statistics and a residual in the same launch are not supported");
   const size_t lds = C3_WBYTES + C3_SBYTES;
   const void* kern = !stats && !res ? (const void*)conv3x3_c64_kernel<false, false> : stats ? (const void*)conv3x3_c64_kernel<true, false> : (const void*)conv3x3_c64_res_kernel;
   if (int r = avec_lds_optin(kern, lds)) return r;
-  C3Args a; a.x = (const bf16*)x; a.w = (const bf16*)w; a.y = (bf16*)y; a.res = (const bf16*)res; a.stats = stats; a.N = (int)images; a.H = H; a.W = W; a.flip = flip; a.rmask = rmask;
+  C3Args a; a.x = (const bf16*)x; a.w = (const bf16*)w; a.y = (bf16*)y; a.res = (const bf16*)res; a.stats = stats; a.N = (int)images; a.H = H; a.W = W; a.flip = flip; a.rmask = rmask; a.rev = order;
   const int grid = (int)(images < 256 ? images : 256);
   avec_note_kernel(stats ? "conv3x3_c64_kernel<true,false>" : res ? "conv3x3_c64_res_kernel" : "conv3x3_c64_kernel<false,false>");
   if (stats) hipLaunchKernelGGL((conv3x3_c64_kernel<true, false>), dim3(grid), dim3(512), lds, st, a);
diff --git a/avec_amd/csrc/norm.hip b/avec_amd/csrc/norm.hip
--- a/avec_amd/csrc/norm.hip
+++ b/avec_amd/csrc/norm.hip
@@ -694,17 +694,19 @@
 template <bool FULL> __device__ __forceinline__ unsigned bns_chunk(unsigned base, int p, unsigned end) {
   const unsigned j = base + threadIdx.x + p * 256; return FULL || j < end ? j : end - 1;
 }
-__device__ __forceinline__ void bns_range(unsigned slice, unsigned n8, unsigned& begin, unsigned& end) {
-  const unsigned long long b = (unsigned long long)blockIdx.x * slice;
+__device__ __forceinline__ unsigned bns_range(unsigned slice, unsigned n8, int rev, unsigned& begin, unsigned& end) {
+  const unsigned s = rev ? gridDim.x - 1 - blockIdx.x : blockIdx.x;
+  const unsigned long long b = (unsigned long long)s * slice;
   begin = b < n8 ? (unsigned)b : n8; end = n8 - begin > slice ? begin + slice : n8;
+  return s;
 }
 
 template <int P, bool RES> struct BnsFwdSet { Raw8<bf16> y[P], r[RES ? P : 1]; };
 template <int P, bool RES, bool MASK>
 __global__ __launch_bounds__(256) void bn_apply8s_kernel(const bf16* __restrict__ y, const float* __restrict__ ss, const bf16* __restrict__ res, int act,
                                                          bf16* __restrict__ out, unsigned n8, int C, unsigned slice, unsigned char* __restrict__ mask,
-                                                         const float* __restrict__ res_ss) {
-  unsigned begin, end; bns_range(slice, n8, begin, end);
+                                                         const float* __restrict__ res_ss, int rev) {
+  unsigned begin, end; bns_range(slice, n8, rev, begin, end);
   const int c = (int)(threadIdx.x % ((unsigned)C >> 3)) * 8;
   Bn8Fwd k; bn8_fwd_coeffs(k, ss, RES ? res_ss : nullptr, C, c);
   typedef BnsFwdSet<P, RES> Set;
@@ -737,8 +739,8 @@
 }
 template <int P, int SRC>
 __global__ __launch_bounds__(256) void bn_bwd_reduce8s_kernel(const bf16* __restrict__ dout, const bf16* __restrict__ y, const bf16* __restrict__ out, const float* __restrict__ ss,
-                                                              int act, float* dstats, unsigned n8, int C, unsigned slice, ColWs ws, const unsigned char* __restrict__ mask) {
-  unsigned begin, end; bns_range(slice, n8, begin, end);
+                                                              int act, float* dstats, unsigned n8, int C, unsigned slice, ColWs ws, const unsigned char* __restrict__ mask, int rev) {
+  unsigned begin, end; const unsigned sl = bns_range(slice, n8, rev, begin, end);
   const Col8 m = col8_map(C);
   const int c = m.l * 8;
   float part[2][8];
@@ -757,16 +759,16 @@
   };
   bns_walk<P, Set>(begin, end, load, use);
   float* const dst[2] = {dstats, dstats + C};
-  colreduce8_atomic<2>(part, dst, m, ws);
+  colreduce8_atomic<2>(part, dst, m, ws, (int)sl);
 }
 template <int P, int SRC>
 __global__ __launch_bounds__(256) void bn_bwd_apply8s_kernel(const bf16* __restrict__ dout, const bf16* __restrict__ y, const bf16* __restrict__ out, const float* __restrict__ ss,
                                                              const float* __restrict__ gamma, const float* __restrict__ dstats, const float* count_ptr, float count, int act,
                                                              bf16* __restrict__ dy, bf16* __restrict__ dres, float* dgamma, float* dbeta, unsigned n8, int C, unsigned slice,
-                                                             const unsigned char* __restrict__ mask) {
+                                                             const unsigned char* __restrict__ mask, int rev) {
   const float inv_n = 1.f / (count_ptr ? *count_ptr : count);
   if (blockIdx.x == 0 && dgamma) for (int cc = threadIdx.x; cc < C; cc += 256) { atomicAdd(dgamma + cc, dstats[C + cc]); atomicAdd(dbeta + cc, dstats[cc]); }
-  unsigned begin, end; bns_range(slice, n8, begin, end);
+  unsigned begin, end; bns_range(slice, n8, rev, begin, end);
   const int c = (int)(threadIdx.x % ((unsigned)C >> 3)) * 8;
   Bn8Bwd k; bn8_bwd_coeffs(k, ss, SRC == BN_SRC_NONE && act != 0, C, c);
   Bn8Dy q; bn8_dy_coeffs(q, k, gamma, dstats, inv_n, C, c);
@@ -805,11 +807,11 @@
   }
 }
 static int bn_apply_fwd_impl(int dtype, const void* y, const float* ss, const void* res, const float* res_ss, int act, void* out, unsigned char* mask, long long M, int C,
-                             hipStream_t st) {
+                             int order, hipStream_t st) {
   const long long n8 = M * C / 8;
   if (bns_ok(dtype, M, C)) {
     const BnsPlan p = bns_plan(0, n8, C, st);
-#define BNS_FWD(RES, MASK) hipLaunchKernelGGL((bn_apply8s_kernel<BNS_P, RES, MASK>), dim3(p.grid), dim3(256), 0, st, (const bf16*)y, ss, (const bf16*)res, act, (bf16*)out, (unsigned)n8, C, p.slice, mask, res_ss)
+#define BNS_FWD(RES, MASK) hipLaunchKernelGGL((bn_apply8s_kernel<BNS_P, RES, MASK>), dim3(p.grid), dim3(256), 0, st, (const bf16*)y, ss, (const bf16*)res, act, (bf16*)out, (unsigned)n8, C, p.slice, mask, res_ss, order)
     if (res) { if (mask) BNS_FWD(true, true); else BNS_FWD(true, false); } else { if (mask) BNS_FWD(false, true); else BNS_FWD(false, false); }
 #undef BNS_FWD
   } else if (C % 8 == 0 && n8 < (1ll << 31)) {
@@ -820,14 +822,21 @@
   }
   AVEC_LAUNCH_CHECK(); return 0;
 }
+extern "C" int avec_bn_apply_fwd_mask_ord(int dtype, const void* y, const float* ss, const void* residual, const float* residual_ss, void* out, unsigned char* mask, long long M, int C,
+                                          int order, hipStream_t st) {
+  AVEC_CHECK_ARG((order == 0 || order == 1) && y && ss && out && mask && M > 0 && C > 0 && C % 8 == 0 && M * C / 8 < (1ll << 31) && (residual || !residual_ss), "bn_apply_fwd_mask: bad arguments (C %% 8 == 0, M*C < 2^34)");
+  return bn_apply_fwd_impl(dtype, y, ss, residual, residual_ss, 2, out, mask, M, C, order, st);
+}
 extern "C" int avec_bn_apply_fwd_mask(int dtype, const void* y, const float* ss, const void* residual, const float* residual_ss, void* out, unsigned char* mask, long long M, int C,
                                       hipStream_t st) {
-  AVEC_CHECK_ARG(y && ss && out && mask && M > 0 && C > 0 && C % 8 == 0 && M * C / 8 < (1ll << 31) && (residual || !residual_ss), "bn_apply_fwd_mask: bad arguments (C %% 8 == 0, M*C < 2^34)");
-  return bn_apply_fwd_impl(dtype, y, ss, residual, residual_ss, 2, out, mask, M, C, st);
+  return avec_bn_apply_fwd_mask_ord(dtype, y, ss, residual, residual_ss, out, mask, M, C, 0, st);
+}
+extern "C" int avec_bn_apply_fwd_ord(int dtype, const void* y, const float* ss, const void* residual, int act, void* out, long long M, int C, int order, hipStream_t st) {
+  AVEC_CHECK_ARG((order == 0 || order == 1) && y && ss && out && M > 0 && C > 0 && C % 4 == 0, "bn_apply_fwd: bad arguments");
+  return bn_apply_fwd_impl(dtype, y, ss, residual, nullptr, act, out, nullptr, M, C, order, st);
 }
 extern "C" int avec_bn_apply_fwd(int dtype, const void* y, const float* ss, const void* residual, int act, void* out, long long M, int C, hipStream_t st) {
-  AVEC_CHECK_ARG(y && ss && out && M > 0 && C > 0 && C % 4 == 0, "bn_apply_fwd: bad arguments");
-  return bn_apply_fwd_impl(dtype, y, ss, residual, nullptr, act, out, nullptr, M, C, st);
+  return avec_bn_apply_fwd_ord(dtype, y, ss, residual, act, out, M, C, 0, st);
 }
 
 template <typename T>
@@ -881,11 +890,14 @@
   colreduce8_atomic<2>(part, dst, m, ws);
 }
 static int bn_bwd_reduce_impl(int dtype, const void* dout, const void* y, const void* out, const unsigned char* mask, const float* ss, int act, float* dstats, long long M, int C,
-                              hipStream_t st) {
+                              int order, hipStream_t st) {
   ColPlan plan;
-  if (mask && bns_ok(dtype, M, C)) {
+  if ((mask || order) && bns_ok(dtype, M, C)) {
     const long long n8 = M * C / 8; const BnsPlan p = bns_plan(1, n8, C, st); plan = p.col;
-    hipLaunchKernelGGL((bn_bwd_reduce8s_kernel<BNS_P, BN_SRC_BITS>), dim3(p.grid), dim3(256), 0, st, (const bf16*)dout, (const bf16*)y, (const bf16*)out, ss, act, dstats, (unsigned)n8, C, p.slice, plan.ws, mask);
+#define BNS_RED(SRC) hipLaunchKernelGGL((bn_bwd_reduce8s_kernel<BNS_P, SRC>), dim3(p.grid), dim3(256), 0, st, (const bf16*)dout, (const bf16*)y, (const bf16*)out, ss, act, dstats, \
+                                        (unsigned)n8, C, p.slice, plan.ws, mask, order)
+    if (mask) BNS_RED(BN_SRC_BITS); else if (act == 2 && out) BNS_RED(BN_SRC_OUT); else BNS_RED(BN_SRC_NONE);
+#undef BNS_RED
   } else if (col8_ok(C)) {
     plan = ColPlan::flat8<2>(M, C, st);
     DISPATCH_T(dtype, hipLaunchKernelGGL(bn_bwd_reduce8_kernel<T>, dim3(plan.nslots), dim3(256), 0, st, (const T*)dout, (const T*)y, (const T*)out, ss, act, dstats, M, C, plan.ws, mask));
@@ -896,13 +908,21 @@
   AVEC_LAUNCH_CHECK();
   return plan.finish({dstats, dstats + C}, C, st);
 }
+extern "C" int avec_bn_bwd_reduce_mask_ord(int dtype, const void* dout, const void* y, const unsigned char* mask, const float* ss, float* dstats, long long M, int C, int order,
+                                           hipStream_t st) {
+  AVEC_CHECK_ARG((order == 0 || order == 1) && dout && y && mask && ss && dstats && M > 0 && col8_ok(C), "bn_bwd_reduce_mask: bad arguments");
+  return bn_bwd_reduce_impl(dtype, dout, y, nullptr, mask, ss, 2, dstats, M, C, order, st);
+}
 extern "C" int avec_bn_bwd_reduce_mask(int dtype, const void* dout, const void* y, const unsigned char* mask, const float* ss, float* dstats, long long M, int C, hipStream_t st) {
-  AVEC_CHECK_ARG(dout && y && mask && ss && dstats && M > 0 && col8_ok(C), "bn_bwd_reduce_mask: bad arguments");
-  return bn_bwd_reduce_impl(dtype, dout, y, nullptr, mask, ss, 2, dstats, M, C, st);
+  return avec_bn_bwd_reduce_mask_ord(dtype, dout, y, mask, ss, dstats, M, C, 0, st);
+}
+extern "C" int avec_bn_bwd_reduce_ord(int dtype, const void* dout, const void* y, const void* out, const float* ss, int act, float* dstats, long long M, int C, int order,
+                                      hipStream_t st) {
+  AVEC_CHECK_ARG((order == 0 || order == 1) && dout && y && ss && dstats && M > 0 && C % 4 == 0, "bn_bwd_reduce: bad arguments");
+  return bn_bwd_reduce_impl(dtype, dout, y, out, nullptr, ss, act, dstats, M, C, order, st);
 }
 extern "C" int avec_bn_bwd_reduce(int dtype, const void* dout, const void* y, const void* out, const float* ss, int act, float* dstats, long long M, int C, hipStream_t st) {
-  AVEC_CHECK_ARG(dout && y && ss && dstats && M > 0 && C % 4 == 0, "bn_bwd_reduce: bad arguments");
-  return bn_bwd_reduce_impl(dtype, dout, y, out, nullptr, ss, act, dstats, M, C, st);
+  return avec_bn_bwd_reduce_ord(dtype, dout, y, out, ss, act, dstats, M, C, 0, st);
 }
 template <typename T>
 __global__ __launch_bounds__(256) void bn_bwd_apply_kernel(const T* __restrict__ dout, const T* __restrict__ y, const T* __restrict__ out, const float* __restrict__ ss,
@@ -948,12 +968,13 @@
   }
 }
 static int bn_bwd_apply_impl(int dtype, const void* dout, const void* y, const void* out, const unsigned char* mask, const float* ss, const float* gamma, const float* dstats,
-                             const float* count_ptr, float count, int act, void* dy, void* dres, float* dgamma, float* dbeta, long long M, int C, hipStream_t st) {
+                             const float* count_ptr, float count, int act, void* dy, void* dres, float* dgamma, float* dbeta, long long M, int C, int order,
+                             hipStream_t st) {
   const long long n8 = M * C / 8;
   if (bns_ok(dtype, M, C)) {
     const BnsPlan p = bns_plan(2, n8, C, st);
 #define BNS_BWD(SRC) hipLaunchKernelGGL((bn_bwd_apply8s_kernel<BNS_P, SRC>), dim3(p.grid), dim3(256), 0, st, (const bf16*)dout, (const bf16*)y, (const bf16*)out, ss, gamma, dstats, \
-                                        count_ptr, count, act, (bf16*)dy, (bf16*)dres, dgamma, dbeta, (unsigned)n8, C, p.slice, mask)
+                                        count_ptr, count, act, (bf16*)dy, (bf16*)dres, dgamma, dbeta, (unsigned)n8, C, p.slice, mask, order)
     if (mask) BNS_BWD(BN_SRC_BITS); else if (act == 2 && out) BNS_BWD(BN_SRC_OUT); else BNS_BWD(BN_SRC_NONE);
 #undef BNS_BWD
   } else if (C % 8 == 0 && n8 < (1ll << 31)) {
@@ -966,15 +987,23 @@
   }
   AVEC_LAUNCH_CHECK(); return 0;
 }
+extern "C" int avec_bn_bwd_apply_mask_ord(int dtype, const void* dout, const void* y, const unsigned char* mask, const float* ss, const float* gamma, const float* dstats,
+                                          const float* count_ptr, float count, void* dy, void* dres, float* dgamma, float* dbeta, long long M, int C, int order, hipStream_t st) {
+  AVEC_CHECK_ARG((order == 0 || order == 1) && dout && y && mask && ss && gamma && dstats && dy && M > 0 && C % 8 == 0 && M * C / 8 < (1ll << 31), "bn_bwd_apply_mask: bad arguments");
+  return bn_bwd_apply_impl(dtype, dout, y, nullptr, mask, ss, gamma, dstats, count_ptr, count, 2, dy, dres, dgamma, dbeta, M, C, order, st);
+}
 extern "C" int avec_bn_bwd_apply_mask(int dtype, const void* dout, const void* y, const unsigned char* mask, const float* ss, const float* gamma, const float* dstats,
                                       const float* count_ptr, float count, void* dy, void* dres, float* dgamma, float* dbeta, long long M, int C, hipStream_t st) {
-  AVEC_CHECK_ARG(dout && y && mask && ss && gamma && dstats && dy && M > 0 && C % 8 == 0 && M * C / 8 < (1ll << 31), "bn_bwd_apply_mask: bad arguments");
-  return bn_bwd_apply_impl(dtype, dout, y, nullptr, mask, ss, gamma, dstats, count_ptr, count, 2, dy, dres, dgamma, dbeta, M, C, st);
+  return avec_bn_bwd_apply_mask_ord(dtype, dout, y, mask, ss, gamma, dstats, count_ptr, count, dy, dres, dgamma, dbeta, M, C, 0, st);
+}
+extern "C" int avec_bn_bwd_apply_ord(int dtype, const void* dout, const void* y, const void* out, const float* ss, const float* gamma, const float* dstats,
+                                     const float* count_ptr, float count, int act, void* dy, void* dres, float* dgamma, float* dbeta, long long M, int C, int order, hipStream_t st) {
+  AVEC_CHECK_ARG((order == 0 || order == 1) && dout && y && ss && gamma && dstats && dy && M > 0 && C % 4 == 0, "bn_bwd_apply: bad arguments");
+  return bn_bwd_apply_impl(dtype, dout, y, out, nullptr, ss, gamma, dstats, count_ptr, count, act, dy, dres, dgamma, dbeta, M, C, order, st);
 }
 extern "C" int avec_bn_bwd_apply(int dtype, const void* dout, const void* y, const void* out, const float* ss, const float* gamma, const float* dstats,
                                  const float* count_ptr, float count, int act, void* dy, void* dres, float* dgamma, float* dbeta, long long M, int C, hipStream_t st) {
-  AVEC_CHECK_ARG(dout && y && ss && gamma && dstats && dy && M > 0 && C % 4 == 0, "bn_bwd_apply: bad arguments");
-  return bn_bwd_apply_impl(dtype, dout, y, out, nullptr, ss, gamma, dstats, count_ptr, count, act, dy, dres, dgamma, dbeta, M, C, st);
+  return avec_bn_bwd_apply_ord(dtype, dout, y, out, ss, gamma, dstats, count_ptr, count, act, dy, dres, dgamma, dbeta, M, C, 0, st);
 }
 extern "C" int avec_bn_slice_mode(int mode) { const int old = bns_mode(); if (mode >= 0 && mode <= 2) bns_mode() = mode; return old; }
 extern "C" int avec_bn_slice_plan(int pass, long long M, int C, int* P, unsigned* grid, unsigned* slice, hipStream_t st) {
diff --git a/avec_amd/csrc/vec.h b/avec_amd/csrc/vec.h
--- a/avec_amd/csrc/vec.h
+++ b/avec_amd/csrc/vec.h
@@ -91,7 +91,7 @@
   Col8 m; m.L = C >> 3; m.R = 256 / m.L; m.r = threadIdx.x / m.L; m.l = threadIdx.x - m.r * m.L; m.active = m.r < m.R; return m;
 }
 template <int NV>
-__device__ __forceinline__ void colreduce8_atomic(float (&part)[NV][8], float* const (&dst)[NV], const Col8& m, const ColWs& ws = ColWs{nullptr}) {
+__device__ __forceinline__ void colreduce8_atomic(float (&part)[NV][8], float* const (&dst)[NV], const Col8& m, const ColWs& ws = ColWs{nullptr}, int slot = -1) {
   __shared__ float red8[NV * 8][256];
 #pragma unroll
   for (int n = 0; n < NV; ++n)
@@ -99,7 +99,7 @@
     for (int e = 0; e < 8; ++e) red8[n * 8 + e][threadIdx.x] = m.active ? part[n][e] : 0.f;
   __syncthreads();
   const int C = m.L * 8;
-  float* mine = ws.partial ? ws_slot(ws, 0, blockIdx.x, gridDim.x, NV * C) : nullptr;
+  float* mine = ws.partial ? ws_slot(ws, 0, slot < 0 ? blockIdx.x : (unsigned)slot, gridDim.x, NV * C) : nullptr;
   for (int o = threadIdx.x; o < NV * 8 * m.L; o += 256) {
     const int q = o / m.L, l = o - q * m.L; float s = 0.f;
     for (int rr = 0; rr < m.R; ++rr) s += red8[q][rr * m.L + l];
diff --git a/avec_amd/nnet/networks.py b/avec_amd/nnet/networks.py
--- a/avec_amd/nnet/networks.py
+++ b/avec_amd/nnet/networks.py
@@ -29,6 +29,7 @@
                                   layers.Linear(dim_blocks[-1], dim_output, weight_init="he_normal", bias_init="zeros")) if include_head else nn.Identity()
 
     def forward_nhwc(self, x):
+        ops.reset_stream_order()
         for i, blk in enumerate(self.blocks):
             x = blk.forward_nhwc(x, chain=i + 1 < len(self.blocks))
         if isinstance(self.head, nn.Identity):
diff --git a/avec_amd/ops.py b/avec_amd/ops.py
--- a/avec_amd/ops.py
+++ b/avec_amd/ops.py
@@ -268,7 +268,7 @@
 
 
 class _BackwardPass:
-    __slots__ = ("task", "queues", "prep", "ln2", "pos", "bn_ready")
+    __slots__ = ("task", "queues", "prep", "ln2", "pos", "bn_ready", "order")
 
     def __init__(self, task):
         self.task = task
@@ -277,6 +277,7 @@
         self.ln2 = {}
         self.pos = {}
         self.bn_ready = {}
+        self.order = 0
 
     def pending(self):
         st = torch.cuda.current_stream()
@@ -298,6 +299,25 @@
         _PASS = _BackwardPass(task)
         torch.autograd.Variable._execution_engine.queue_callback(_flush_at_end)
     return _PASS
+
+
+STREAM_ORDER = True
+_FWD_ORDER = [0]
+
+
+def reset_stream_order(order=0):
+    _FWD_ORDER[0] = order
+
+
+def _take_order():
+    if not STREAM_ORDER:
+        return 0
+    ps = _pass()
+    if ps is not None:
+        o, ps.order = ps.order, ps.order ^ 1
+    else:
+        o, _FWD_ORDER[0] = _FWD_ORDER[0], _FWD_ORDER[0] ^ 1
+    return o
 
 
 def _in_backward():
@@ -977,18 +997,18 @@
         lib.bn_bwd_finalize(pre.stats.data_ptr(), BNState.NREP, st.ss.data_ptr(), dstats.data_ptr(), C, rt.stream())
         act, out, want_dres, mask = ACT_NONE, None, False, None
     elif mask is not None:
-        lib.bn_bwd_reduce_mask(rt.dt(), dout.data_ptr(), y.data_ptr(), mask.data_ptr(), st.ss.data_ptr(), dstats.data_ptr(), M, C, rt.stream())
+        lib.bn_bwd_reduce_mask_ord(rt.dt(), dout.data_ptr(), y.data_ptr(), mask.data_ptr(), st.ss.data_ptr(), dstats.data_ptr(), M, C, _take_order(), rt.stream())
     else:
-        lib.bn_bwd_reduce(rt.dt(), dout.data_ptr(), y.data_ptr(), _p(out), st.ss.data_ptr(), act, dstats.data_ptr(), M, C, rt.stream())
+        lib.bn_bwd_reduce_ord(rt.dt(), dout.data_ptr(), y.data_ptr(), _p(out), st.ss.data_ptr(), act, dstats.data_ptr(), M, C, _take_order(), rt.stream())
     dstats, gw, gb = _bn_sync_grads(bn, dstats, C)
     dy = empty((M, C), adt, dout)
     dres = empty((M, C), adt, dout) if want_dres else None
     if mask is not None:
-        lib.bn_bwd_apply_mask(rt.dt(), dout.data_ptr(), y.data_ptr(), mask.data_ptr(), st.ss.data_ptr(), bn.weight.data_ptr(), dstats.data_ptr(), cptr, float(count),
-                              dy.data_ptr(), _p(dres), _p(gw), _p(gb), M, C, rt.stream())
+        lib.bn_bwd_apply_mask_ord(rt.dt(), dout.data_ptr(), y.data_ptr(), mask.data_ptr(), st.ss.data_ptr(), bn.weight.data_ptr(), dstats.data_ptr(), cptr, float(count),
+                                  dy.data_ptr(), _p(dres), _p(gw), _p(gb), M, C, _take_order(), rt.stream())
     else:
-        lib.bn_bwd_apply(rt.dt(), dout.data_ptr(), y.data_ptr(), _p(out), st.ss.data_ptr(), bn.weight.data_ptr(), dstats.data_ptr(), cptr, float(count), act,
-                         dy.data_ptr(), _p(dres), _p(gw), _p(gb), M, C, rt.stream())
+        lib.bn_bwd_apply_ord(rt.dt(), dout.data_ptr(), y.data_ptr(), _p(out), st.ss.data_ptr(), bn.weight.data_ptr(), dstats.data_ptr(), cptr, float(count), act,
+                             dy.data_ptr(), _p(dres), _p(gw), _p(gb), M, C, _take_order(), rt.stream())
     return dy, (dout if pre is not None else dres)
 
 
@@ -1317,7 +1337,7 @@
     y = empty((M, Cout), rt.act_dtype(), x)
     if _slab_conv(H, W, Cin, Cout, KH, KW, stride):
         ev = KERNEL_TIMER.start()
-        lib.conv3x3_c64(x.data_ptr(), sh.fwd.data_ptr(), y.data_ptr(), None, _p(stats), N, H, W, 0, rt.stream())
+        lib.conv3x3_c64_ord(x.data_ptr(), sh.fwd.data_ptr(), y.data_ptr(), None, _p(stats), N, H, W, 0, _take_order(), rt.stream())
         KERNEL_TIMER.stop(ev, (2, 0), 2.0 * M * Cout * KH * KW * Cin, 2.0 * (N * H * W * Cin + Cout * KH * KW * Cin + M * Cout))
         return y, OH, OW
     gemm_nt(x, sh.fwd, y, M, Cout, KH * KW * Cin, rows=rows_conv(H, W, Cin, KH, KW, stride, pad, OH, OW), mode=ROWS_CONV_FWD, stats=stats,
@@ -1371,9 +1391,9 @@
     if _slab_conv(H, W, Cin, Cout, KH, KW, stride):
         ev = KERNEL_TIMER.start()
         if dx_res_mask is not None:
-            lib.conv3x3_c64_res_masked(dy.data_ptr(), sh.bwd.data_ptr(), dx.data_ptr(), dx_res.data_ptr(), dx_res_mask.data_ptr(), N, H, W, 1, rt.stream())
-        else:
-            lib.conv3x3_c64(dy.data_ptr(), sh.bwd.data_ptr(), dx.data_ptr(), _p(dx_res), None, N, H, W, 1, rt.stream())
+            lib.conv3x3_c64_res_masked_ord(dy.data_ptr(), sh.bwd.data_ptr(), dx.data_ptr(), dx_res.data_ptr(), dx_res_mask.data_ptr(), N, H, W, 1, _take_order(), rt.stream())
+        else:
+            lib.conv3x3_c64_ord(dy.data_ptr(), sh.bwd.data_ptr(), dx.data_ptr(), _p(dx_res), None, N, H, W, 1, _take_order(), rt.stream())
         KERNEL_TIMER.stop(ev, (2, 1), 2.0 * N * H * W * Cin * KH * KW * Cout, 2.0 * (2 * N * H * W * Cin + Cout * KH * KW * Cin + M * Cout))
         return dx
     fuse = bnb if (bnb is not None and BNB_FUSE and rt.act_dtype() == torch.bfloat16 and Cin % 4 == 0) else None
@@ -1409,7 +1429,7 @@
         Mo = N * OH * OW
         c1 = bn_finalize(bn1, st1, Mo, training)
         a1 = empty((Mo, Cout), adt, x)
-        lib.bn_apply_fwd(rt.dt(), y1.data_ptr(), st1.ss.data_ptr(), None, ACT_RELU, a1.data_ptr(), Mo, Cout, rt.stream())
+        lib.bn_apply_fwd_ord(rt.dt(), y1.data_ptr(), st1.ss.data_ptr(), None, ACT_RELU, a1.data_ptr(), Mo, Cout, _take_order(), rt.stream())
         y2, _, _ = conv2d_fwd(a1, conv2.weight, N, OH, OW, Cout, 1, stats=st2.stats if training else None)
         c2 = bn_finalize(bn2, st2, Mo, training)
         has_proj = not isinstance(blk.residual, torch.nn.Identity)
@@ -1422,17 +1442,17 @@
         use_mask = RELU_BITMASK and training and Cout % 8 == 0 and Cout <= 2048 and Mo * Cout // 8 < (1 << 31)
         if has_proj and not use_mask:
             r = empty((Mo, Cout), adt, x)
-            lib.bn_apply_fwd(rt.dt(), yr.data_ptr(), str_.ss.data_ptr(), None, ACT_NONE, r.data_ptr(), Mo, Cout, rt.stream())
+            lib.bn_apply_fwd_ord(rt.dt(), yr.data_ptr(), str_.ss.data_ptr(), None, ACT_NONE, r.data_ptr(), Mo, Cout, _take_order(), rt.stream())
         elif not has_proj:
             r = x
         out = empty((Mo, Cout), adt, x)
         ctx.relu_mask = None
         if use_mask:
             ctx.relu_mask = torch.empty(Mo * Cout // 8, dtype=torch.uint8, device=x.device)
-            lib.bn_apply_fwd_mask(rt.dt(), y2.data_ptr(), st2.ss.data_ptr(), (yr if has_proj else r).data_ptr(), str_.ss.data_ptr() if has_proj else None, out.data_ptr(),
-                                  ctx.relu_mask.data_ptr(), Mo, Cout, rt.stream())
-        else:
-            lib.bn_apply_fwd(rt.dt(), y2.data_ptr(), st2.ss.data_ptr(), r.data_ptr(), ACT_RELU, out.data_ptr(), Mo, Cout, rt.stream())
+            lib.bn_apply_fwd_mask_ord(rt.dt(), y2.data_ptr(), st2.ss.data_ptr(), (yr if has_proj else r).data_ptr(), str_.ss.data_ptr() if has_proj else None, out.data_ptr(),
+                                      ctx.relu_mask.data_ptr(), Mo, Cout, _take_order(), rt.stream())
+        else:
+            lib.bn_apply_fwd_ord(rt.dt(), y2.data_ptr(), st2.ss.data_ptr(), r.data_ptr(), ACT_RELU, out.data_ptr(), Mo, Cout, _take_order(), rt.stream())
         ctx.saved = (x, y1, a1, y2, yr, out, st1, st2, str_, c1, c2, cr, blk, training, N, H, W, Cin, Cout, OH, OW, stride, has_proj)
         ctx.chain = bool(chain and training and BNB_FUSE and rt.act_dtype() == torch.bfloat16)
         if ctx.chain:
@@ -1514,11 +1534,12 @@
             PH, PW = (OH - 1) // 2 + 1, (OW - 1) // 2 + 1
             zp = torch.empty((B * T, PH, PW, C), dtype=torch.bfloat16, device=v.device)
             idx = torch.empty((B * T, PH, PW, C), dtype=torch.uint8, device=v.device)
+            reset_stream_order(1)
             lib.stem3p_fwd(vb.data_ptr(), w8.data_ptr(), _p(conv.bias), bn.weight.data_ptr(), zp.data_ptr(), idx.data_ptr(), st.stats.data_ptr() if training else None,
                            B, T, H, W, rt.stream())
             cp = bn_finalize(bn, st, M, training)
             out = torch.empty_like(zp)
-            lib.bn_apply_fwd(rt.dt(), zp.data_ptr(), st.ss.data_ptr(), None, ACT_RELU, out.data_ptr(), B * T * PH * PW, C, rt.stream())
+            lib.bn_apply_fwd_ord(rt.dt(), zp.data_ptr(), st.ss.data_ptr(), None, ACT_RELU, out.data_ptr(), B * T * PH * PW, C, _take_order(), rt.stream())
             ctx.saved = (v, None, idx, st, cp, conv, bn, ("p", vb, w8, zp, PH, PW), B, T, OH, OW, C, M, K, training, None)
             return out
         if STEM3D_DIRECT and rt.compute_dtype() == "bf16" and C == 64 and K == 245 and lib.raw("avec_stem3d_supported")(B, T, H, W):
diff --git a/include/avec_hip.h b/include/avec_hip.h
--- a/include/avec_hip.h
+++ b/include/avec_hip.h
@@ -133,6 +133,16 @@
 int avec_bn_bwd_reduce_mask(int dtype, const void* dout, const void* y, const unsigned char* mask, const float* ss, float* dstats, long long M, int C, hipStream_t stream);
 int avec_bn_bwd_apply_mask(int dtype, const void* dout, const void* y, const unsigned char* mask, const float* ss, const float* gamma, const float* dstats,
                            const float* count_ptr, float count, void* dy, void* dres, float* dgamma, float* dbeta, long long M, int C, hipStream_t stream);
+int avec_bn_apply_fwd_ord(int dtype, const void* y, const float* ss, const void* residual, int act, void* out, long long M, int C, int order, hipStream_t stream);
+int avec_bn_apply_fwd_mask_ord(int dtype, const void* y, const float* ss, const void* residual, const float* residual_ss, void* out, unsigned char* mask, long long M, int C,
+                               int order, hipStream_t stream);
+int avec_bn_bwd_reduce_ord(int dtype, const void* dout, const void* y, const void* out, const float* ss, int act, float* dstats, long long M, int C, int order, hipStream_t stream);
+int avec_bn_bwd_reduce_mask_ord(int dtype, const void* dout, const void* y, const unsigned char* mask, const float* ss, float* dstats, long long M, int C, int order,
+                                hipStream_t stream);
+int avec_bn_bwd_apply_ord(int dtype, const void* dout, const void* y, const void* out, const float* ss, const float* gamma, const float* dstats,
+                          const float* count_ptr, float count, int act, void* dy, void* dres, float* dgamma, float* dbeta, long long M, int C, int order, hipStream_t stream);
+int avec_bn_bwd_apply_mask_ord(int dtype, const void* dout, const void* y, const unsigned char* mask, const float* ss, const float* gamma, const float* dstats,
+                               const float* count_ptr, float count, void* dy, void* dres, float* dgamma, float* dbeta, long long M, int C, int order, hipStream_t stream);
 int avec_softmax_fwd(int dtype, const float* logits, void* probs, long long M, int V, hipStream_t stream);
 int avec_softmax_bwd(int dtype, const void* dprobs, const float* logits, float* dlogits, const float* dadd, long long M, int V, hipStream_t stream);
 int avec_cast_rows(int dtype, const float* src, long long ld_src, void* dst, long long ld_dst, long long M, int N, hipStream_t stream);
@@ -255,6 +265,9 @@
 int avec_conv3x3_c64_supported(int H, int W, int Cin, int Cout, int KH, int KW, int stride);
 int avec_conv3x3_c64(const void* x, const void* w, void* y, const void* res, float* stats, long long images, int H, int W, int flip, hipStream_t stream);
 int avec_conv3x3_c64_res_masked(const void* x, const void* w, void* y, const void* res, const unsigned char* res_mask, long long images, int H, int W, int flip, hipStream_t stream);
+int avec_conv3x3_c64_ord(const void* x, const void* w, void* y, const void* res, float* stats, long long images, int H, int W, int flip, int order, hipStream_t stream);
+int avec_conv3x3_c64_res_masked_ord(const void* x, const void* w, void* y, const void* res, const unsigned char* res_mask, long long images, int H, int W, int flip, int order,
+                                    hipStream_t stream);
 int avec_wgrad3x3_c64(const void* x, const void* dy, float* dw, long long images, int H, int W, hipStream_t stream);
 int avec_wgrad3x3_c128_supported(int H, int W, int Cin, int Cout, int KH, int KW, int stride);
 int avec_wgrad3x3_c128(const void* x, const void* dy, float* dw, long long images, int C, int H, int W, hipStream_t stream);
```

New measurement: 1953 (median of 6 runs). Within noise of the previous version (+0.5%).
